# WilliamVenner/squad-mortar-helper

Measured on AMD Instinct MI355X. Metric: map frames/sec (1920x1080 full CV pipeline), whole job, higher is better.
Workload: dtype u8/f32

## Files before the change

### squad-mortar-helper_amd/batch.py

```python
import ctypes as C

import numpy as np

from . import _lib as L

STAGE_NAMES = ("button", "map_pass", "brq_pass", "lsd", "scale_ratio")


def make_anchors(per_frame):
    arr = (L.Anchors * len(per_frame))()
    for i, (start_y, scales) in enumerate(per_frame):
        arr[i].n = min(len(scales), L.MAX_SCALES)
        arr[i].scales_start_y = start_y
        for j, (m, x, y) in enumerate(scales[:L.MAX_SCALES]):
            arr[i].scales[j][0], arr[i].scales[j][1], arr[i].scales[j][2] = m, x, y
    return arr


def results_to_dicts(recs):
    out = []
    for r in recs:
        n = r.n_lines
        out.append(dict(
            map_open=int(r.map_open), n_lines=int(n),
# ... 93 lines not shown
            except L.VisionError as e:
                e.records = recs if rc == L.E_STATE else None
                raise
        return recs

    def set_firing(self, heightmap=None, fit_to_minimap=True, viewport=None):
        opt = L.firing_options(fit_to_minimap, viewport)
        L.check(self._lib.smhv_batch_set_firing(self._b, heightmap._hm if heightmap is not None else None, C.byref(opt)))

    def read_firing(self, first=0, n=None):
        n = self.max_frames - first if n is None else n
        out = (L.FiringResult * n)()
        L.check(self._lib.smhv_batch_read_firing(self._b, first, n, out))
        raw = np.frombuffer(out, np.uint8).reshape(n, C.sizeof(L.FiringResult))
        n_lines = raw[:, :4].copy().view(np.uint32).reshape(n)
        lines = raw[:, 8:].copy().view(L.firing_dtype()).reshape(n, L.MAX_LINES)
        return n_lines, lines

    def firing_ptr(self):
        d = C.c_void_p()
        L.check(self._lib.smhv_batch_firing_ptr(self._b, C.byref(d)))
        return d.value or 0

    def read_overlay(self, frame):
        return self.read_image(L.IMAGE_HEIGHTMAP_OVERLAY, frame)

    def overlay_ptr(self):
        d = C.c_void_p()
        L.check(self._lib.smhv_batch_overlay_ptr(self._b, C.byref(d)))
        return d.value or 0

    def render(self, viewport, out_w, out_h, first=0, n=None, heightmap=None, markers=False, fit_to_minimap=True, background=(0, 0, 0, 255),
               stream=None, options=None, layers=None):
        from .render import render_options
        n = self.max_frames - first if n is None else n
        opt = options if options is not None else render_options(viewport, out_w, out_h, heightmap is not None, markers, fit_to_minimap, background)
        if layers is not None:
            ly, keep = layers.struct()
            L.check(self._lib.smhv_batch_render_layers(self._b, first, n, heightmap._hm if heightmap is not None else None, C.byref(opt), C.byref(ly), stream))
            del keep
            return
        L.check(self._lib.smhv_batch_render(self._b, first, n, heightmap._hm if heightmap is not None else None, C.byref(opt), stream))

    def render_size(self):
        w, h = C.c_uint32(), C.c_uint32()
        L.check(self._lib.smhv_batch_render_size(self._b, C.byref(w), C.byref(h)))
        return int(w.value), int(h.value)

    def read_render(self, frame):
        w, h = self.render_size()
        out = np.empty((h, w, 4), np.uint8)
        L.check(self._lib.smhv_batch_read_render(self._b, frame, out.ctypes.data))
        return out

    def render_ptr(self):
        d, st = C.c_void_p(), C.c_uint64()
        L.check(self._lib.smhv_batch_render_ptr(self._b, C.byref(d), C.byref(st)))
        return d.value or 0, int(st.value)

    def render_labels(self, options, labels, first=0, n=None, heightmap=None, stream=None):
        n = self.max_frames - first if n is None else n
        lo, keep = labels.struct()
        L.check(self._lib.smhv_batch_render_labels(self._b, first, n, heightmap._hm if heightmap is not None else None, C.byref(options), C.byref(lo), stream))
        del keep

    def read_labels(self, first=0, n=None):
        n = self.max_frames - first if n is None else n
        out = (L.LabelResult * n)()
        L.check(self._lib.smhv_batch_read_labels(self._b, first, n, out))
        return out

    def labels_ptr(self):
        d = C.c_void_p()
        L.check(self._lib.smhv_batch_labels_ptr(self._b, C.byref(d)))
        return d.value or 0

    def feed(self, feed, first=0, n=None, snapshot=False, stream=0):
        n = self.max_frames - first if n is None else n
        L.check(self._lib.smhv_batch_feed(self._b, feed._f, first, n, L.FEED_SNAPSHOT if snapshot else 0, C.c_void_p(stream)))

    def read_image(self, which, frame):
        x, y, w, h = self.roi
        if which in (L.IMAGE_UI_MAP, L.IMAGE_HEIGHTMAP_OVERLAY):
            out = np.empty((h, w, 4), np.uint8)
        elif which == L.VIEW_LSD_INPUT:
            out = np.empty((h, w), np.uint8)
        else:
            out = np.empty((h // 2, w // 2), np.uint8)
        L.check(self._lib.smhv_batch_read_image(self._b, which, frame, out.ctypes.data))
        return out


class Pipeline:

    def __init__(self, vision, frame_w, frame_h, max_frames, depth=4, search=None, **options):
        self._lib = L.load()
        self._vision = vision
        p = C.c_void_p()
        opt = L.PipelineOptions()
        opt.size = C.sizeof(L.PipelineOptions)
        opt.search = {None: L.SEARCH_AUTO, "auto": L.SEARCH_AUTO, "batch": L.SEARCH_BATCH, "frame": L.SEARCH_FRAME}[search]
        for k, v in options.items():
            if k not in ("streams", "idle_close_us", "occupancy_policy", "late_helpers", "service_workgroups", "flags", "remote_after", "remote_tickets", "remote_last", "room_for_others"):
                raise TypeError("Pipeline: unknown option %r" % k)
            setattr(opt, k, int(v))
        L.check(self._lib.smhv_pipeline_create_ex(vision._ctx, frame_w, frame_h, max_frames, depth, C.byref(opt), C.byref(p)))
        self._p = p
        self.depth = depth
        self.slots = []
        for i in range(depth):
            b = C.c_void_p()
            L.check(self._lib.smhv_pipeline_slot(self._p, i, C.byref(b), None))
            self.slots.append(FrameBatch(vision, frame_w, frame_h, max_frames, _handle=b))

    def stream_of(self, slot):
        st = C.c_void_p()
        L.check(self._lib.smhv_pipeline_slot(self._p, slot, None, C.byref(st)))
        return st.value or 0

    def hold(self, slot, stream):
        L.check(self._lib.smhv_pipeline_hold(self._p, slot, C.c_void_p(stream)))

    def submit(self, frames_ptr, n, stages=L.STAGE_ALL, grayscale=True, max_gap=15, anchors=None, after_stream=0):
        if anchors is not None and len(anchors) < n:
            raise ValueError("anchors holds %d entries, the submission covers %d frames" % (len(anchors), n))
        a = C.cast(anchors, C.c_void_p) if anchors is not None else None
        slot = C.c_uint32(0)
        L.check(self._lib.smhv_pipeline_submit(self._p, C.c_void_p(frames_ptr), n, stages, int(bool(grayscale)), max_gap, a, C.c_void_p(after_stream), C.byref(slot)))
        return int(slot.value)

    def set_firing(self, heightmap=None, fit_to_minimap=True, viewport=None):
        opt = L.firing_options(fit_to_minimap, viewport)
        L.check(self._lib.smhv_pipeline_set_firing(self._p, heightmap._hm if heightmap is not None else None, C.byref(opt)))

    def search_stats(self):
        out = (C.c_uint64 * 32)()
        L.check(self._lib.smhv_debug_pipeline_stats(self._p, out))
        if not out[0]:
            return None
        keys = ("launches", "frames", "waves", "busy_cycles", "resident_cycles", "waves_per_launch", "submissions")
        d = dict(zip(keys, [int(v) for v in out[1:8]]))
        d["cycles_per_frame_by_phase"] = dict(zip(("acquire", "search", "record", "release"), [int(v) / max(d["frames"], 1) for v in out[8:12]]))
        d["help_cycles_per_frame"] = int(out[12]) / max(d["frames"], 1)
        d["remote_help"] = {"requests": int(out[16]), "helpers_attached": int(out[17]), "candidates_cast": int(out[18]), "tickets_left": int(out[19]) - (1 << 64) if int(out[19]) >= (1 << 63) else int(out[19])}
        d["cycles_per_frame"] = d["busy_cycles"] / max(d["frames"], 1)
        d["busy_fraction"] = d["busy_cycles"] / max(d["resident_cycles"], 1)
        d["remote_help"].update({"polls": int(out[23]), "polls_empty": int(out[24]), "claims_lost": int(out[25]), "exits_idle": int(out[26]), "exits_closed": int(out[27]),
                                 "cycles_attached_per_helper": int(out[28]) / max(int(out[17]), 1), "cast_fraction_of_attached": int(out[29]) / max(int(out[28]), 1)})
        d["timeline_ms"] = {"frame_wait": int(out[20]) / max(d["frames"], 1) / 1e5, "submission_search": int(out[21]) / max(d["submissions"], 1) / 1e5,
                            "last_frame_at_work": int(out[22]) / max(d["submissions"], 1) / 1e5}
        d["adaptive"] = bool(int(out[13]) & 2)
        d["settled"] = bool(int(out[13]) & 4) or not d["adaptive"]
        d["mode"] = "frame-granular" if int(out[13]) & 1 else "batch-granular"
        d["measured_frames_per_s"] = {"frame-granular": int(out[14]), "batch-granular": int(out[15])}
        return d

    def peek(self):
        out = (C.c_uint64 * 16)()
        L.check(self._lib.smhv_debug_pipeline_peek(self._p, out))
        keys = ("submissions", "alive_epoch", "launches", "last_seq", "avail", "head", "reserved", "closing_epoch", "completed", "busy")
        d = dict(zip(keys, [int(v) for v in out[:10]]))
        d["avail"] = d["avail"] - (1 << 64) if d["avail"] >= (1 << 63) else d["avail"]
        d["slots"] = [(int(v) >> 32, int(v) & 0xFFFFFFFF) for v in out[10:14]]
        d["service_workgroups"], d["waves_per_workgroup"] = int(out[14]) >> 32, int(out[14]) & 0xFFFFFFFF
        d["lds_words_per_wave"], d["lds_bytes_dynamic"] = int(out[15]) >> 32, int(out[15]) & 0xFFFFFFFF
        return d

    def wait(self, slot=None):
        if slot is None:
            L.check(self._lib.smhv_pipeline_wait_all(self._p))
        else:
            L.check(self._lib.smhv_pipeline_wait(self._p, slot))

    def close(self):
        if self._p:
            for b in self.slots:
                b.close()
            self._lib.smhv_pipeline_destroy(self._p)
            self._p = None

    def __del__(self):
        try:
            self.close()
        except Exception:
            pass
```

### squad-mortar-helper_amd/csrc/smh_kernels.h

```cpp
#pragma once
#include <hip/hip_runtime.h>
#include <stdint.h>

#include "../../include/smh_vision_hip.h"
#include "../../include/smh_vision_hip_debug.h"

namespace smh {

struct Geom {
	uint32_t W, H;
	uint32_t rx, ry, rw, rh;
	uint32_t bx, by, bw, bh;
	uint32_t qx, qy, qw, qh;
	uint32_t m_ax, m_xoff, m_quads, m_block;
	uint32_t q_ax, q_xoff, q_quads, q_block;
	uint64_t frame_bytes;
	uint64_t ui_pitch, ui_stride;
	uint64_t mask_pitch, mask_stride;
	uint32_t bits_pitch_w; uint64_t bits_stride_w;
	uint64_t ocr_pitch, ocr_stride;
};

struct FrameAux {
	uint32_t open;
	uint32_t red;
	uint32_t n_mask_px;
	uint32_t y_min, y_max, w_min, w_max;
	uint32_t tiles;
};

struct LsdCoop {
	uint32_t req_tail;
	uint32_t req_head;
	uint32_t done;
	uint32_t helpers;
	uint32_t remaining;
	uint32_t mode1;
	uint32_t stat_groups, stat_hits, stat_casts;
	uint32_t pad[7];
};
struct LsdCtl {
	uint32_t started[3];
	uint32_t finished[3];
	uint32_t pad[10];
};
struct LsdCacheEntry {
	unsigned long long tag;
	unsigned long long best;
	float ex, ey;
	uint32_t steps, pad;
};
#define SMH_LSD_REQ_CAP 64u
#define SMH_LSD_CACHE_SLOTS 512u
struct LsdCoopBufs {
	LsdCtl *ctl;
	LsdCoop *coop;
	uint32_t *req;
	LsdCacheEntry *cache;
	uint32_t epoch;
};

struct BatchError {
	uint32_t count;
	uint32_t frame, status;
	uint32_t info[8];
	uint32_t pad[5];
};

#define SMH_FARM_RING 4u
#define SMH_REC_ON 0x80000000u
#define SMH_LSD_LATE_HELP 1u
struct FarmEntry {
	unsigned long long post;
	unsigned long long best;
	unsigned long long end;
	unsigned long long start;
	unsigned long long done;
	unsigned long long pad[3];
};
struct FarmFrame {
	unsigned long long attached;
	unsigned long long owner_done;
	unsigned long long want;
	unsigned long long claimed;
	unsigned long long pad[4];
	FarmEntry ring[SMH_FARM_RING];
};

struct Buffers {
	BatchError *err;
	FarmFrame *farm;
	uint32_t rec_stages;
	uint32_t *rec_bars;
	uint32_t lsd_flags, lsd_late_kc;
	const uint8_t *frames;
	uint8_t *ui, *mask, *ocr, *scales;
	uint32_t *bits;
	uint32_t *tiled;
	uint8_t *occ;
	FrameAux *aux;
	smhv_frame_result *results;
	const smhv_anchors *anchors;
	const uint32_t *cull_tab;
	const float *ray_off;
	LsdCoopBufs co;
	const struct FiringRun *firing;
};
struct FiringRun {
	const uint16_t *hm;
	smhv_firing_result *out;
	uint32_t hm_w, hm_h;
	float b0x, b0y;
	double zscale;
	uint32_t flags;
	float sw, sh, tx, ty;
	uint32_t pad;
};
static_assert(sizeof(FiringRun) == 64, "one 64-byte block per run");
struct OverlayRun {
	const uint8_t *ui;
	uint8_t *out;
	const FrameAux *aux;
	const smhv_frame_result *res;
	const uint16_t *hm;
	const uint32_t *lut;
	uint32_t hm_w, hm_h;
	float b0x, b0y;
	uint32_t flags;
};
#define SMH_RND_MAX_LINES 256u
struct RenderRun {
	const uint8_t *ui;
	uint8_t *out;
	const FrameAux *aux;
	const smhv_frame_result *res;
	const smhv_line *lines;
	const uint16_t *hm;
	const uint32_t *lut;
	const uint16_t *lut16;
	uint64_t out_stride;
	uint32_t hm_w, hm_h;
	float b0x, b0y;
	uint32_t flags;
	uint32_t n_lines;
	uint32_t out_w, out_h;
	float ql, qt, qr, qb;
	float sw, sh, tx, ty;
	uint32_t bg;
	uint32_t lds_texels;
	uint32_t n_frames;
};
#define SMH_RND_MAX_ITEMS (SMH_RND_MAX_LINES + SMHV_RENDER_MAX_PRIMS + 1u)
#define SMH_RND_SRC_UI 0u
#define SMH_RND_SRC_GRAY 1u
#define SMH_RND_SRC_RGBA 2u
#define SMH_RND_SRC_PREPROCESS 3u
#define SMH_RND_SRC_CROPPED 4u
struct RenderLayersRun {
	const smhv_render_prim *prims;
	const uint8_t *src;
	uint64_t src_pitch, src_stride;
	uint32_t src_xoff;
	uint32_t src_mode;
	uint32_t src_w, src_h;
	uint32_t n_below, n_fg;
	uint32_t flags;
	uint32_t pad;
};
#define SMH_LBL_SLOTS (SMHV_LABEL_MAX_EXTRA + SMHV_MAX_LINES)
struct LabelCull { float mx, my, rad; uint32_t live; };
struct LabelRun {
	FiringRun fr;
	const FrameAux *aux;
	const smhv_frame_result *res;
	const smhv_label_line *extra;
	const smhv_line *lines;
	smhv_label_result *out;
	LabelCull *cull;
	uint8_t *img;
	uint64_t img_stride;
	double mpx;
	uint32_t out_w, out_h;
	uint32_t n_extra, n_lines;
	uint32_t detected;
	uint32_t scale;
	uint32_t per_call;
	uint32_t has_mpx;
};
__host__ __device__ inline uint32_t tiled_rows(const Geom &g) { return (g.rh + 7u) >> 3; }
__host__ __device__ inline uint64_t tiled_stride_w(const Geom &g) { return (uint64_t)tiled_rows(g) * g.bits_pitch_w * 8u; }
__host__ __device__ inline uint32_t occ_pitch(const Geom &g) { return ((g.m_block >> 6) + 3u) & ~3u; }
__host__ __device__ inline uint64_t occ_stride(const Geom &g) { return (uint64_t)tiled_rows(g) * occ_pitch(g); }

#define SMH_RAY_OFF_BATCHES 168u

#define SMH_SECTOR_R 52
#define SMH_SECTOR_DIM (2 * SMH_SECTOR_R + 1)
#define SMH_SECTOR_ENTRIES (SMH_SECTOR_DIM * SMH_SECTOR_DIM)
#define SMH_CULL_CELLS (SMH_SECTOR_DIM * 4)
#define SMH_CULL_TAB_WORDS (SMH_CULL_CELLS + (SMH_SECTOR_ENTRIES + 3) / 4)

#define SVC_MAX_SLOTS 32u
struct SvcSlot {
	Buffers b;
	uint32_t n;
	uint32_t seq;
	uint32_t done;
	uint32_t pad;
	unsigned long long t_pub;
};
#define SVC_REMOTE_RING 12u
#define SVC_REMOTE_OPEN 0x80000000ull
struct SvcRemoteEntry {
	unsigned long long post;
	unsigned long long claim;
	uint32_t res_a[4];
	uint32_t res_b[4];
	unsigned long long pad[2];
};
struct SvcRemote {
	unsigned long long state;
	unsigned long long info;
	unsigned long long pad[6];
	SvcRemoteEntry ring[SVC_REMOTE_RING];
};
#define SVC_HELP_RING 256u
struct SvcCtl {
	int32_t avail;
	uint32_t closing;
	int32_t help_avail;
	uint32_t help_head, help_reserve;
	uint32_t stat_remote;
	uint32_t head;
	uint32_t reserve;
	uint32_t completed;
	uint32_t busy;
	uint32_t stat_items, stat_waves;
	unsigned long long stat_busy, stat_life;
	unsigned long long stat_phase[4];
	unsigned long long stat_help;
	uint32_t stat_requests, stat_attached;
	unsigned long long stat_t_wait, stat_t_sub, stat_t_last;
	uint32_t stat_h_polls, stat_h_empty, stat_h_lost, stat_h_idle_exit, stat_h_closed_exit, stat_h_pad;
	unsigned long long stat_h_cycles, stat_h_cast_cycles;
	unsigned long long help_ring[SVC_HELP_RING];
};
struct SvcHost {
	unsigned long long state;
	uint32_t launches;
	uint32_t pad0;
	uint32_t done_seq[SVC_MAX_SLOTS];
	uint32_t pad[12];
};
struct SvcParams {
	SvcCtl *ctl;
	unsigned long long *ring;
	SvcSlot *slots;
	SvcHost *host;
	const uint32_t *cull_tab;
	const float *ray_off;
	float max_gap;
	uint32_t tile_cap, list_cap;
	uint32_t part_words;
	uint32_t ring_log2;
	uint32_t epoch;
	uint32_t idle_short, idle_long;
	uint32_t flags;
	SvcRemote *remote;
	uint32_t *remote_store;
	uint32_t remote_store_words;
	uint32_t remote_after;
	uint32_t remote_tickets;
	uint32_t remote_last_div;
	uint32_t compact;
};
uint32_t svc_waves_for(const Geom &g, uint32_t tile_limit, uint32_t *part_words, uint32_t *tile_cap, uint32_t *list_cap, uint32_t *lds_bytes, uint32_t *compact = nullptr);
uint32_t svc_store_words_for(const Geom &g, uint32_t tile_cap, uint32_t compact);
hipError_t svc_probe_host_atomics(SvcHost *h, SvcHost *d_h, bool *ok);
hipError_t launch_svc_publish(SvcCtl *ctl, unsigned long long *ring, SvcSlot *slots, uint32_t slot, const Buffers &b, uint32_t n, uint32_t seq, uint32_t ring_log2, hipStream_t s);
hipError_t launch_lsd_service(const Geom &g, const SvcParams &p, uint32_t workgroups, uint32_t waves, uint32_t lds_bytes, hipStream_t s);

enum : uint32_t { MAP_UI = 1u, MAP_MASK = 2u, MAP_PRIO = 0x100u, MAP_BAND_MAJOR = 0x200u };
enum : uint32_t { BRQ_OCR = 1u, BRQ_SCALES = 2u };

hipError_t launch_button(const Geom &g, const Buffers &b, uint32_t n, int force_open, hipStream_t s);
hipError_t launch_map_pass(const Geom &g, const Buffers &b, uint32_t n, uint32_t flags, int grayscale, hipStream_t s, bool tiles_wanted = false, bool overlapped = false);
struct LaunchTuning {
	uint32_t map_lds_total;
	uint32_t map_grid_cap;
	uint32_t lsd_tile_limit;
	uint32_t map_prio;
	uint32_t map_deep;
	uint32_t map_overlapped;
};
uint32_t map_brq_lds_bytes(const Geom &g);
uint32_t lsd_tile_lds_bytes(const Geom &g, uint32_t tile_limit);
hipError_t launch_map_brq_pass(const Geom &g, const Buffers &b, uint32_t n, uint32_t flags, uint32_t qflags, int grayscale, uint32_t fixed_start_y, int use_anchor_start, hipStream_t s,
                               const LaunchTuning *tune = nullptr);
hipError_t launch_pattern_copy(const Geom &g, const Buffers &b, uint32_t n, uint32_t rows_in_flight, hipStream_t s);
void map_band_rows(uint32_t rh, uint32_t n, int fused, uint32_t *rows, int *tiles);
hipError_t launch_brq_pass(const Geom &g, const Buffers &b, uint32_t n, uint32_t flags, uint32_t fixed_start_y, int use_anchor_start, hipStream_t s);
struct LsdFork { hipStream_t s1, s2; hipEvent_t fork, join1, join2; };
bool lsd_rows_only(const Geom &g);
hipError_t launch_lsd(const Geom &g, const Buffers &b, uint32_t n, float max_gap, int mode, float px, float py, hipStream_t s, const LsdFork *fk, uint32_t tile_bs = 0,
                      bool prefer_classic = false, uint32_t tile_limit = 0, bool *record_fused = nullptr);
size_t lsd_coop_ctl_bytes(uint32_t n);
hipError_t launch_scale_ratio(const Geom &g, const Buffers &b, uint32_t n, uint32_t *d_bars, hipStream_t s);
hipError_t launch_find_minimap(const Geom &g, const Buffers &b, uint32_t n, hipStream_t s);
hipError_t launch_finalize(const Geom &g, const Buffers &b, uint32_t n, uint32_t stages, hipStream_t s);
hipError_t launch_scales_finalize(const Geom &g, const Buffers &b, uint32_t n, uint32_t stages, uint32_t *d_bars, hipStream_t s);
hipError_t launch_firing_lines(const FiringRun &r, const smhv_line *lines, uint32_t n, uint32_t has_mpx, double mpx, uint32_t has_minimap,
                               const uint32_t minimap[4], smhv_firing *out, hipStream_t s);
hipError_t launch_heightmap_color_map(const uint16_t *hm, uint64_t n, uint32_t *mm, uint32_t *rgba, hipStream_t s);
#define SMH_HM_LUT_ENTRIES 65536u
hipError_t launch_heightmap_lut(const uint16_t *hm, uint64_t n, uint32_t *mm, uint32_t *lut, hipStream_t s);
hipError_t launch_hm_overlay(const Geom &g, const OverlayRun &r, uint32_t n, hipStream_t s);
hipError_t launch_render_map(const Geom &g, const RenderRun &r, uint32_t n, hipStream_t s);
hipError_t launch_render_map_layers(const Geom &g, const RenderRun &r, const RenderLayersRun &y, uint32_t n, hipStream_t s);
hipError_t launch_heightmap_lut16(const uint32_t *lut, uint16_t *lut16, uint32_t *vr, hipStream_t s);
#define SMH_HM_LUT_WORDS (SMH_HM_LUT_ENTRIES + 4u + SMH_HM_LUT_ENTRIES / 2u)
hipError_t launch_labels(const LabelRun &r, uint32_t n, hipStream_t s);
void render_set_form(uint32_t form);
uint32_t render_rule(const Geom &g, const RenderRun &r, uint32_t *texels, float *ratio);
float render_switch_ratio();
hipError_t launch_debug_view(const Geom &g, const Buffers &b, uint32_t frame, int which, int isolated, uint8_t *d_rgba, hipStream_t s);
hipError_t launch_marker_table(uint32_t *d_bits, hipStream_t s);
hipError_t launch_pack_rows(const void *d_src, uint32_t src_pitch_bytes, void *d_dst, uint32_t row_bytes, uint32_t rows, hipStream_t s);
hipError_t launch_side_probe(uint32_t *d_out, uint32_t workgroups, uint32_t spin, hipStream_t s);
hipError_t launch_build_sector_table(unsigned long long *d_tab, uint32_t T, hipStream_t s);
hipError_t launch_build_ray_offsets(float *d_off, hipStream_t s);
size_t lsd_lds_bytes();
void lsd_set_classic(bool on);
void lsd_set_tile_cap(uint32_t cap);
void lsd_set_threads(uint32_t threads);
void lsd_set_spin_limit(uint32_t polls);
hipError_t set_ray_table(const float *dx, const float *dy);
#define SMH_CRC_BS 1024
hipError_t launch_to_bgra(const void *d_src, void *d_bgra, uint64_t n_px, uint32_t layout, hipStream_t s);
hipError_t launch_unpack_rows(const void *d_pack, void *d_frame, uint32_t pitch_px, uint32_t roi_x, uint32_t roi_y, uint32_t roi_w, uint32_t roi_h, uint32_t btn_x,
                              uint32_t btn_y, uint32_t btn_w, uint32_t btn_h, hipStream_t s);
hipError_t launch_crc32(const void *d_msg, uint64_t n_dwords, uint32_t wgs, uint32_t rounds, uint32_t x_skip, const uint32_t *d_x_local,
                        const uint32_t *d_x_wg, uint32_t *d_acc, hipStream_t s);
uint32_t crc32_xpow(uint64_t n);
uint32_t crc32_mul(uint32_t a, uint32_t b);

struct FeedMap { uint64_t dst; uint32_t frame, pad; };
struct FeedRun {
	const uint8_t *ui;
	const smhv_frame_result *res;
	uint64_t ui_stride, ui_pitch;
	uint32_t w, h, xoff, quads;
	uint32_t n, first, flags;
	uint32_t len_term;
	uint32_t rows_per_wave;
	uint64_t capacity;
	uint32_t *raw;
	const uint32_t *tab;
	uint32_t *state;
	smhv_feed_header *header;
	smhv_feed_entry *entries;
	uint8_t *bytes;
	FeedMap *maps;
};
#define SMH_FEED_MAX_ROWS 16384u
hipError_t launch_feed_tables(uint32_t *d_tab, uint32_t w, uint32_t h, uint32_t xoff, uint32_t quads, hipStream_t s);
uint32_t feed_rows_per_wave(uint32_t h, uint32_t n);
void feed_set_rows(uint32_t rows);
hipError_t launch_feed(const FeedRun &r, hipStream_t s);

}
```

### squad-mortar-helper_amd/csrc/smh_lsd.hip

```cpp
#include <algorithm>
#include <atomic>
#include <cstdlib>
#include <cstring>

#include "smh_device.h"
#include "smh_proximity.h"
#include "smh_record.inc"

namespace smh {

struct RayDir { uint32_t dx, dy; };
__device__ RayDir g_ray_table[SMH_LSD_RAYS] = {
#include "ray_table.inc"
};

#ifndef LSD_BS
#define LSD_BS 1024
#endif
#define LSD_NW (LSD_BS / 64)
#ifndef LSD_C
#define LSD_C 8u
#endif
#ifndef LSD_C_RESET
#define LSD_C_RESET 2u
// ... 1126 lines not shown
				if (hit) m |= 1ull << u;
			}
		}
	}
	tab[i] = m;
}

size_t lsd_lds_bytes() { return LSD_DYN_LDS_BYTES; }

static std::atomic<bool> &lsd_classic_flag() {
	static std::atomic<bool> flag{false};
	return flag;
}
void lsd_set_classic(bool on) { lsd_classic_flag().store(on, std::memory_order_relaxed); }
static std::atomic<uint32_t> g_tile_cap_override{0};
void lsd_set_tile_cap(uint32_t cap) { g_tile_cap_override.store(cap, std::memory_order_relaxed); }
static std::atomic<uint32_t> g_bs_override{0};
void lsd_set_threads(uint32_t threads) { g_bs_override.store(threads, std::memory_order_relaxed); }
static std::atomic<uint32_t> g_spin_limit{W_SPIN_LIMIT_DEFAULT};
void lsd_set_spin_limit(uint32_t polls) { g_spin_limit.store(polls ? polls : W_SPIN_LIMIT_DEFAULT, std::memory_order_relaxed); }

bool lsd_rows_only(const Geom &g) { return (g.rh + 2u) * LSD_ROWS_PITCH(g.bits_pitch_w) + 4u <= LSD_WIN_WORDS_CAP; }

static uint32_t lsd_tile_static_lds() {
	static const uint32_t v = [] { hipFuncAttributes a; return hipFuncGetAttributes(&a, (const void *)k_lsd_tile) == hipSuccess ? (uint32_t)a.sharedSizeBytes : 17408u; }();
	return v;
}
static uint32_t lsd_tile_cap_of(const Geom &g, uint32_t tile_limit) {
	const uint32_t cap_o = g_tile_cap_override.load(std::memory_order_relaxed);
	uint32_t cap = tile_cap_for(g);
	if (tile_limit) cap = std::min(cap, tile_limit);
	if (cap_o) cap = std::min(cap_o, tile_cap_for(g));
	return cap;
}
uint32_t lsd_tile_lds_bytes(const Geom &g, uint32_t tile_limit) {
	return lsd_tile_static_lds() + (tile_mask_words(g.rw, g.rh, lsd_tile_cap_of(g, tile_limit)) + 2u * tile_list_cap_for(g) + W_NWIN * W_WIN_STRIDE) * 4u;
}

hipError_t launch_lsd(const Geom &g, const Buffers &b, uint32_t n, float max_gap, int mode, float px, float py, hipStream_t s, const LsdFork *fk, uint32_t tile_bs, bool prefer_classic,
                      uint32_t tile_limit, bool *record_fused) {
	if (record_fused) *record_fused = false;
	const unsigned lds_full = LSD_DYN_LDS_BYTES;
	static std::atomic<uint64_t> attr_devices{0};
	int dev = 0;
	hipError_t e0 = hipGetDevice(&dev);
	if (e0 != hipSuccess) return e0;
	if (dev >= 64 || !((attr_devices.load(std::memory_order_acquire) >> dev) & 1ull)) {
		hipError_t e = hipSuccess;
		const void *fns[] = {(const void *)k_lsd<LSD_MODE_ROWS, false>, (const void *)k_lsd<LSD_MODE_XWIN, false>, (const void *)k_lsd<LSD_MODE_GLOBAL, false>,
		                     (const void *)k_lsd<LSD_MODE_ROWS, true>, (const void *)k_lsd<LSD_MODE_XWIN, true>, (const void *)k_lsd<LSD_MODE_GLOBAL, true>};
		for (const void *fn : fns) if (e == hipSuccess) e = hipFuncSetAttribute(fn, hipFuncAttributeMaxDynamicSharedMemorySize, (int)lds_full);
		if (e == hipSuccess) e = hipFuncSetAttribute((const void *)k_lsd_tile, hipFuncAttributeMaxDynamicSharedMemorySize, (int)LSD_TILE_DYN_LDS_MAX);
		if (e != hipSuccess) return e;
		if (dev < 64) attr_devices.fetch_or(1ull << dev, std::memory_order_release);
	}
	const bool rows_only = mode == 0 && lsd_rows_only(g);
	const bool coop = mode == 0 && b.co.ctl != nullptr;
	if (mode == 0 && !coop && !prefer_classic && !lsd_classic_flag().load(std::memory_order_relaxed)) {
		const uint32_t bs_o = g_bs_override.load(std::memory_order_relaxed);
		const uint32_t bs = std::max<uint32_t>(128u, bs_o ? bs_o : (tile_bs ? std::min<uint32_t>(tile_bs, LSD_TILE_BS) : 512u));
		const uint32_t cap = lsd_tile_cap_of(g, tile_limit);
		const unsigned t_lds = std::min<unsigned>((tile_mask_words(g.rw, g.rh, cap) + 2u * tile_list_cap_for(g) + W_NWIN * W_WIN_STRIDE) * 4u, LSD_TILE_DYN_LDS_MAX);
		if (record_fused) *record_fused = (b.rec_stages & SMH_REC_ON) != 0u;
		hipLaunchKernelGGL(k_lsd_tile, dim3(n), dim3(bs), t_lds, s, g, b, max_gap, cap, g_spin_limit.load(std::memory_order_relaxed), tile_list_cap_for(g), n);
		return hipGetLastError();
	}
	if (coop) {
		hipError_t e = hipMemsetAsync(b.co.ctl, 0, lsd_coop_ctl_bytes(n), s);
		if (e != hipSuccess) return e;
	}
	uint32_t extra = 0;
	if (coop && rows_only) {
		static std::atomic<int> n_cus{0};
		int cus = n_cus.load(std::memory_order_relaxed);
		if (cus == 0) {
			if (hipDeviceGetAttribute(&cus, hipDeviceAttributeMultiprocessorCount, dev) != hipSuccess || cus <= 0) cus = 256;
			n_cus.store(cus, std::memory_order_relaxed);
		}
		if (n < (uint32_t)cus) extra = std::min((uint32_t)cus - n, 4u * n);
	}
	hipStream_t s1 = s, s2 = s;
	if (!rows_only && fk) {
		hipError_t e = hipEventRecord(fk->fork, s);
		if (e == hipSuccess) e = hipStreamWaitEvent(fk->s1, fk->fork, 0);
		if (e == hipSuccess) e = hipStreamWaitEvent(fk->s2, fk->fork, 0);
		if (e != hipSuccess) return e;
		s1 = fk->s1; s2 = fk->s2;
	}
	if (record_fused && mode == 0) *record_fused = (b.rec_stages & SMH_REC_ON) != 0u;
	if (coop) hipLaunchKernelGGL((k_lsd<LSD_MODE_ROWS, true>), dim3(n + extra), dim3(LSD_BS), lds_full, s, g, b, max_gap, mode, px, py, n);
	else hipLaunchKernelGGL((k_lsd<LSD_MODE_ROWS, false>), dim3(n), dim3(LSD_BS), lds_full, s, g, b, max_gap, mode, px, py, n);
	if (!rows_only) {
		if (coop) hipLaunchKernelGGL((k_lsd<LSD_MODE_XWIN, true>), dim3(n), dim3(LSD_BS), lds_full, s1, g, b, max_gap, mode, px, py, n);
		else hipLaunchKernelGGL((k_lsd<LSD_MODE_XWIN, false>), dim3(n), dim3(LSD_BS), lds_full, s1, g, b, max_gap, mode, px, py, n);
		if (coop) hipLaunchKernelGGL((k_lsd<LSD_MODE_GLOBAL, true>), dim3(n), dim3(LSD_BS), lds_full, s2, g, b, max_gap, mode, px, py, n);
		else hipLaunchKernelGGL((k_lsd<LSD_MODE_GLOBAL, false>), dim3(n), dim3(LSD_BS), lds_full, s2, g, b, max_gap, mode, px, py, n);
		if (fk) {
			hipError_t e = hipEventRecord(fk->join1, s1);
			if (e == hipSuccess) e = hipEventRecord(fk->join2, s2);
			if (e == hipSuccess) e = hipStreamWaitEvent(s, fk->join1, 0);
			if (e == hipSuccess) e = hipStreamWaitEvent(s, fk->join2, 0);
			if (e != hipSuccess) return e;
		}
	}
	return hipGetLastError();
}

static uint32_t lsd_service_static_lds() {
	static const uint32_t v = [] { hipFuncAttributes a; return hipFuncGetAttributes(&a, (const void *)k_lsd_service) == hipSuccess ? (uint32_t)a.sharedSizeBytes : SMH_CULL_TAB_WORDS * 4u; }();
	return v;
}
uint32_t svc_waves_for(const Geom &g, uint32_t tile_limit, uint32_t *part_words, uint32_t *tile_cap, uint32_t *list_cap, uint32_t *lds_bytes, uint32_t *compact) {
	const uint32_t cap = lsd_tile_cap_of(g, tile_limit);
	const uint32_t lds_cu = 160u * 1024u, beside = 2u * ((map_brq_lds_bytes(g) + 1023u) & ~1023u) + 1024u;
	uint32_t best_w = 0, best_part = 0, best_lc = 0, best_c = 0;
	for (uint32_t c = 0; c < 2u; ++c) {
		const uint32_t lc = c ? W_LIST_CAP_MAX / 2u : tile_list_cap_for(g);
		const uint32_t part = (SVC_WS_WORDS + (c ? tilec_mask_words(g.rw, g.rh, cap) : tile_mask_words(g.rw, g.rh, cap)) + 2u * lc + W_WIN_STRIDE + 3u) & ~3u;
		uint32_t w = SVC_MAX_WAVES;
		while (w > 0u && lsd_service_static_lds() + w * part * 4u + beside > lds_cu) --w;
		if (w > best_w) { best_w = w; best_part = part; best_lc = lc; best_c = c; }
	}
	if (part_words) *part_words = best_part;
	if (tile_cap) *tile_cap = cap;
	if (list_cap) *list_cap = best_lc;
	if (lds_bytes) *lds_bytes = best_w * best_part * 4u;
	if (compact) *compact = best_c;
	return best_w;
}

uint32_t svc_store_words_for(const Geom &g, uint32_t tile_cap, uint32_t compact) { return ((compact ? tilec_mask_words(g.rw, g.rh, tile_cap) : tile_mask_words(g.rw, g.rh, tile_cap)) + 7u) & ~3u; }

hipError_t svc_probe_host_atomics(SvcHost *h, SvcHost *d_h, bool *ok) {
	*ok = false;
	uint32_t *d_ok = nullptr;
	hipError_t e = hipMalloc((void **)&d_ok, sizeof(uint32_t));
	if (e != hipSuccess) return e;
	const unsigned long long expect = 0x0123456789ABCDEFull, desired = 0xFEDCBA9876543210ull;
	unsigned long long *w = (unsigned long long *)&h->pad[0];
	__atomic_store_n(w, expect, __ATOMIC_RELEASE);
	__atomic_store_n(&h->pad[2], 0u, __ATOMIC_RELEASE);
	e = hipMemset(d_ok, 0, sizeof(uint32_t));
	uint32_t dev_ok = 0;
	if (e == hipSuccess) { hipLaunchKernelGGL(k_svc_probe, dim3(1), dim3(1), 0, nullptr, d_h, expect, desired, d_ok); e = hipGetLastError(); }
	if (e == hipSuccess) e = hipMemcpy(&dev_ok, d_ok, sizeof dev_ok, hipMemcpyDeviceToHost);
	(void)hipFree(d_ok);
	if (e != hipSuccess) return e;
	*ok = dev_ok == 1u && __atomic_load_n(w, __ATOMIC_ACQUIRE) == desired && __atomic_load_n(&h->pad[2], __ATOMIC_ACQUIRE) == 0x600Du;
	__atomic_store_n(w, 0ull, __ATOMIC_RELEASE);
	__atomic_store_n(&h->pad[2], 0u, __ATOMIC_RELEASE);
	return hipSuccess;
}

hipError_t launch_svc_publish(SvcCtl *ctl, unsigned long long *ring, SvcSlot *slots, uint32_t slot, const Buffers &b, uint32_t n, uint32_t seq, uint32_t ring_log2, hipStream_t s) {
	hipLaunchKernelGGL(k_svc_publish, dim3(1), dim3(256), 0, s, ctl, ring, slots, slot, b, n, seq, ring_log2);
	return hipGetLastError();
}

hipError_t launch_lsd_service(const Geom &g, const SvcParams &p, uint32_t workgroups, uint32_t waves, uint32_t lds_bytes, hipStream_t s) {
	static std::atomic<uint64_t> attr_devices{0};
	int dev = 0;
	hipError_t e = hipGetDevice(&dev);
	if (e != hipSuccess) return e;
	if (dev >= 64 || !((attr_devices.load(std::memory_order_acquire) >> dev) & 1ull)) {
		e = hipFuncSetAttribute((const void *)k_lsd_service, hipFuncAttributeMaxDynamicSharedMemorySize, 160 * 1024 - (int)lsd_service_static_lds());
		if (e == hipSuccess) e = hipFuncSetAttribute((const void *)k_lsd_service_c, hipFuncAttributeMaxDynamicSharedMemorySize, 160 * 1024 - (int)lsd_service_static_lds());
		if (e != hipSuccess) return e;
		if (dev < 64) attr_devices.fetch_or(1ull << dev, std::memory_order_release);
	}
	if (p.compact) hipLaunchKernelGGL(k_lsd_service_c, dim3(workgroups), dim3(64u * waves), lds_bytes, s, g, p);
	else hipLaunchKernelGGL(k_lsd_service, dim3(workgroups), dim3(64u * waves), lds_bytes, s, g, p);
	return hipGetLastError();
}

size_t lsd_coop_ctl_bytes(uint32_t n) { return sizeof(LsdCtl) + sizeof(LsdCoop) * (size_t)n; }

hipError_t set_ray_table(const float *dx, const float *dy) {
	static RayDir host[SMH_LSD_RAYS];
	for (int i = 0; i < SMH_LSD_RAYS; ++i) { memcpy(&host[i].dx, &dx[i], 4); memcpy(&host[i].dy, &dy[i], 4); }
	return hipMemcpyToSymbol(HIP_SYMBOL(g_ray_table), host, sizeof host, 0, hipMemcpyHostToDevice);
}

__global__ void k_build_ray_offsets(float *off) {
	const uint32_t i = blockIdx.x * blockDim.x + threadIdx.x;
	if (i >= SMH_LSD_RAYS) return;
	const float dx = __uint_as_float(g_ray_table[i].dx), dy = __uint_as_float(g_ray_table[i].dy);
	float xo = 0.0f, yo = 0.0f;
	float2 *o = (float2 *)off + (size_t)i * (SMH_RAY_OFF_BATCHES + 1u);
	for (uint32_t j = 0; j <= SMH_RAY_OFF_BATCHES; ++j) {
		o[j] = make_float2(xo, yo);
		for (int k = 0; k < 32; ++k) { xo += dx; yo += dy; }
	}
}

hipError_t launch_build_ray_offsets(float *d_off, hipStream_t s) {
	hipLaunchKernelGGL(k_build_ray_offsets, dim3((SMH_LSD_RAYS + 63) / 64), dim3(64), 0, s, d_off);
	return hipGetLastError();
}

hipError_t launch_build_sector_table(unsigned long long *d_tab, uint32_t T, hipStream_t s) {
	static_assert(LSD_GROUPS == LSD_GROUPS_HOST && LSD_GROUPS <= 64, "sector masks are 64-bit");
	hipLaunchKernelGGL(k_build_sector_table, dim3((SMH_SECTOR_ENTRIES + 255) / 256), dim3(256), 0, s, d_tab, T);
	return hipGetLastError();
}

}
```

### squad-mortar-helper_amd/csrc/smh_lsd_seq.inc

```

template <int MODE>
__device__ __forceinline__ uint32_t seq_build_list(const Win &m, WShared &ws, uint32_t *list, uint32_t *survw, uint32_t list_cap, uint32_t wy0, uint32_t wrows, uint32_t wwords, uint32_t wi_min,
                                                   uint32_t WT, uint32_t *wi_next) {
	const uint32_t lane = threadIdx.x & 63u;
	uint32_t o = 0, next = WT;
	auto append = [&](uint32_t w, uint32_t wi) {
		const unsigned long long nz = __ballot(w != 0u);
		if (!nz) return;
		const uint32_t pos = o + (uint32_t)__popcll(nz & ((1ull << lane) - 1ull));
		if (w != 0u && pos < list_cap) { list[pos] = wi; survw[pos] = w; ws.stag[pos] = 0; }
		const uint32_t cnt = (uint32_t)__popcll(nz);
		if (o + cnt > list_cap) {
			unsigned long long rest = nz;
			for (uint32_t k = o; k < list_cap; ++k) rest &= rest - 1ull;
			next = (uint32_t)__builtin_amdgcn_readlane((int)wi, (int)__builtin_ctzll(rest));
			o = list_cap;
		} else o += cnt;
	};
	if constexpr (MODE == LSD_MODE_TILE || MODE == LSD_MODE_TILEC) {
		auto tile_at = [&](uint32_t ty, uint32_t c) -> uint32_t {
			if constexpr (MODE == LSD_MODE_TILEC) return tilec_number(m, (int)c, (int)ty);
			else return (uint32_t)m.t_idx[__mul24((int)ty, (int)m.t_pitch) + (int)c];
		};
		const bool two = wwords <= 32u;
// ... 296 lines not shown
		const uint32_t wi = list[e], r = wi / wwords, c = wi - r * wwords;
		fpy = (float)(wy0 + r); fpx0 = (float)(xorg + (int)(c * 32u));
		const uint32_t tag = ws.stag[e];
		if (w && tag < n_lines) {
			for (uint32_t l = tag; l < n_lines && w; ++l) {
				ProxLine L;
				L.x0 = ws.lines[l][0]; L.y0 = ws.lines[l][1]; L.x1 = ws.lines[l][2]; L.y1 = ws.lines[l][3];
				L.a = ws.prox_a[l]; L.dxl = ws.prox_d[l][0]; L.dyl = ws.prox_d[l][1];
				L.degenerate = L.dxl == 0.0 && L.dyl == 0.0;
				w = prox_filter_word(w, fpx0, fpy, L);
			}
			survw[e] = w;
			ws.stag[e] = (unsigned char)n_lines;
		}
	}
	return w;
}

__device__ __forceinline__ void desk_post_remote(WShared &ws, uint32_t slot, uint32_t qx, uint32_t qy, uint32_t &st, uint32_t &spx, uint32_t &spy) {
	const uint32_t k = uniform_u32(ws.rem_k) + 1u;
	if (opaque_lane() == slot) {
		ws.rob[slot].px = qx; ws.rob[slot].py = qy; ws.rob[slot].lines_seen = k; ws.rob[slot].state = H_RPOSTED;
		ws.rem_k = k;
		g_st64(&rem_of(ws)->ring[slot - SEQ_HELP_SLOTS].post, ((unsigned long long)k << 32) | ((qy & 0xFFFFu) << 16) | (qx & 0xFFFFu));
		st = H_RPOSTED; spx = qx; spy = qy;
	}
	RDBG(0, 1ull);
	wave_lds_sync();
}
__device__ __forceinline__ void desk_refresh(WShared &ws, const uint32_t *list, uint32_t *survw, uint32_t wy0, uint32_t wwords, int xorg, uint32_t cap_local, uint32_t cap_remote, uint32_t &post_seq,
                                             uint32_t &cur_e, int &cur_bit, uint32_t &ahead) {
	const uint32_t lane = opaque_lane();
	const uint32_t n_lines = W_LD(&ws.n_lines), end = ws.disp_end, first = W_LD(&ws.disp_e);
	const uint32_t want = 1u + cap_local + cap_remote;
	cur_e = end; cur_bit = -1;
	uint32_t mpx = 0xFFFFFFFFu, mpy = 0xFFFFFFFFu, np = 0;
	for (uint32_t e0 = first & ~63u; e0 < end && np < want; e0 += 64u) {
		float fpx0, fpy;
		const uint32_t w = disp_entry(ws, list, survw, e0 + lane, first, end, n_lines, wy0, wwords, xorg, fpx0, fpy);
		unsigned long long any = __ballot(w != 0u);
		while (any && np < want) {
			const uint32_t src = (uint32_t)__builtin_ctzll(any);
			any &= any - 1ull;
			uint32_t ww = (uint32_t)__builtin_amdgcn_readlane((int)w, (int)src);
			const int bx = (int)bcast_f(fpx0, src);
			const uint32_t by = (uint32_t)bcast_f(fpy, src);
			while (ww && np < want) {
				const uint32_t bit = (uint32_t)__builtin_ctz(ww);
				ww &= ww - 1u;
				if (lane == np) { mpx = (uint32_t)(bx + (int)bit); mpy = by; }
				++np;
				if (np == want) { cur_e = e0 + src; cur_bit = (int)bit; }
			}
		}
	}
	ahead = np;
	uint32_t st = H_FREE, spx = 0, spy = 0, sk = 0;
	if (lane < SEQ_DESK_ENTRIES) { st = W_LD_ACQ(&ws.rob[lane].state); spx = ws.rob[lane].px; spy = ws.rob[lane].py; sk = ws.rob[lane].lines_seen; }
	bool listed = false;
	for (uint32_t k = 0; k < np; ++k) {
		const uint32_t qx = (uint32_t)__builtin_amdgcn_readlane((int)mpx, (int)k), qy = (uint32_t)__builtin_amdgcn_readlane((int)mpy, (int)k);
		listed = listed || (spx == qx && spy == qy);
	}
	if (lane < SEQ_HELP_SLOTS && !listed) {
		if (st == (uint32_t)H_DONE) { W_ST(&ws.rob[lane].state, (uint32_t)H_FREE); st = H_FREE; }
		else if (st == (uint32_t)H_POSTED) {
			uint32_t expect = H_POSTED;
			if (__hip_atomic_compare_exchange_strong(&ws.rob[lane].state, &expect, (uint32_t)H_FREE, __ATOMIC_ACQ_REL, __ATOMIC_RELAXED, __HIP_MEMORY_SCOPE_WORKGROUP)) st = H_FREE;
			else st = H_TAKEN;
		}
	}
	if (lane >= SEQ_HELP_SLOTS && lane < SEQ_DESK_ENTRIES && !listed) {
		if (st == (uint32_t)H_DONE) { ws.rob[lane].state = H_FREE; st = H_FREE; }
		else if (st == (uint32_t)H_RPOSTED) {
			const unsigned long long old = __hip_atomic_fetch_max(&rem_of(ws)->ring[lane - SEQ_HELP_SLOTS].claim, (unsigned long long)sk, __ATOMIC_RELAXED, __HIP_MEMORY_SCOPE_AGENT);
			st = (uint32_t)old < sk ? (uint32_t)H_FREE : (uint32_t)H_RZOMBIE;
			ws.rob[lane].state = st;
#ifdef SMH_LSD_WDEBUG
			atomicAdd(&ws.rdbg[st == (uint32_t)H_FREE ? 1 : 2], 1ull);
#endif
		}
	}
	wave_lds_sync();
	for (uint32_t k = 1; k < np; ++k) {
		const uint32_t qx = (uint32_t)__builtin_amdgcn_readlane((int)mpx, (int)k), qy = (uint32_t)__builtin_amdgcn_readlane((int)mpy, (int)k);
		const bool live = lane < SEQ_DESK_ENTRIES && st != (uint32_t)H_FREE && st != (uint32_t)H_RZOMBIE;
		if (__ballot(live && spx == qx && spy == qy) != 0ull) continue;
		const unsigned long long free_l = __ballot(lane < SEQ_HELP_SLOTS && st == (uint32_t)H_FREE);
		const unsigned long long free_r = __ballot(lane >= SEQ_HELP_SLOTS && lane < SEQ_DESK_ENTRIES && st == (uint32_t)H_FREE);
		const uint32_t busy_l = SEQ_HELP_SLOTS - (uint32_t)__popcll(free_l);
		const uint32_t busy_r = (uint32_t)__popcll(__ballot(lane >= SEQ_HELP_SLOTS && live));
		if (busy_l < cap_local && free_l) {
			const uint32_t slot = (uint32_t)__builtin_ctzll(free_l);
			if (lane == slot) {
				ws.rob[slot].px = qx; ws.rob[slot].py = qy; ws.rob[slot].lines_seen = post_seq;
				W_ST_REL(&ws.rob[slot].state, (uint32_t)H_POSTED);
				st = H_POSTED; spx = qx; spy = qy;
			}
			++post_seq;
		} else if (busy_r < cap_remote && free_r) desk_post_remote(ws, (uint32_t)__builtin_ctzll(free_r), qx, qy, st, spx, spy);
		else break;
	}
}

__device__ __forceinline__ void desk_post_more(WShared &ws, const uint32_t *list, uint32_t *survw, uint32_t wy0, uint32_t wwords, int xorg, uint32_t cap_local, uint32_t cap_remote, uint32_t &post_seq,
                                               uint32_t &cur_e, int &cur_bit, uint32_t &ahead) {
	const uint32_t lane = opaque_lane();
	uint32_t st = H_DONE;
	if (lane < SEQ_DESK_ENTRIES) st = W_LD_ACQ(&ws.rob[lane].state);
	unsigned long long free_l = __ballot(lane < SEQ_HELP_SLOTS && st == (uint32_t)H_FREE);
	unsigned long long free_r = __ballot(lane >= SEQ_HELP_SLOTS && lane < SEQ_DESK_ENTRIES && st == (uint32_t)H_FREE);
	uint32_t busy_l = SEQ_HELP_SLOTS - (uint32_t)__popcll(free_l);
	uint32_t busy_r = (uint32_t)__popcll(__ballot(lane >= SEQ_HELP_SLOTS && lane < SEQ_DESK_ENTRIES && (st == (uint32_t)H_RPOSTED || st == (uint32_t)H_DONE)));
	if (cap_remote && busy_r < cap_remote && !free_r && __ballot(lane >= SEQ_HELP_SLOTS && lane < SEQ_DESK_ENTRIES && st == (uint32_t)H_RZOMBIE)) {
		remote_harvest(ws);
		if (lane < SEQ_DESK_ENTRIES) st = W_LD_ACQ(&ws.rob[lane].state);
		free_r = __ballot(lane >= SEQ_HELP_SLOTS && lane < SEQ_DESK_ENTRIES && st == (uint32_t)H_FREE);
	}
	bool room_l = busy_l < cap_local && free_l, room_r = busy_r < cap_remote && free_r;
	if (!room_l && !room_r) return;
	const uint32_t n_lines = W_LD(&ws.n_lines), end = ws.disp_end, first = W_LD(&ws.disp_e);
	while ((room_l || room_r) && cur_e < end) {
		const uint32_t e0 = cur_e & ~63u;
		float fpx0, fpy;
		uint32_t w = disp_entry(ws, list, survw, e0 + lane, first, end, n_lines, wy0, wwords, xorg, fpx0, fpy);
		if (e0 + lane < cur_e) w = 0u;
		else if (e0 + lane == cur_e && cur_bit >= 0) w = cur_bit >= 31 ? 0u : (w & ~((2u << (uint32_t)cur_bit) - 1u));
		const unsigned long long any = __ballot(w != 0u);
		if (!any) { cur_e = e0 + 64u; cur_bit = -1; continue; }
		const uint32_t src = (uint32_t)__builtin_ctzll(any);
		const uint32_t ww = (uint32_t)__builtin_amdgcn_readlane((int)w, (int)src);
		const uint32_t bit = (uint32_t)__builtin_ctz(ww);
		const uint32_t ppx = (uint32_t)((int)bcast_f(fpx0, src) + (int)bit), ppy = (uint32_t)bcast_f(fpy, src);
		cur_e = e0 + src; cur_bit = (int)bit;
		if (ahead++ == 0u) continue;
		if (room_l) {
			const uint32_t slot = (uint32_t)__builtin_ctzll(free_l);
			free_l &= free_l - 1ull;
			if (lane == slot) {
				ws.rob[slot].px = ppx; ws.rob[slot].py = ppy; ws.rob[slot].lines_seen = post_seq;
				W_ST_REL(&ws.rob[slot].state, (uint32_t)H_POSTED);
			}
			++post_seq; ++busy_l;
		} else {
			uint32_t d0 = 0, d1 = 0, d2 = 0;
			desk_post_remote(ws, (uint32_t)__builtin_ctzll(free_r), ppx, ppy, d0, d1, d2);
			free_r &= free_r - 1ull;
			++busy_r;
		}
		room_l = busy_l < cap_local && free_l; room_r = busy_r < cap_remote && free_r;
	}
}

template <int MODE, bool WAVE = false, bool TEAM = false>
__device__ void lsd_frame_seq(const Geom &g, const Buffers &b, uint32_t f, float max_gap, const FrameAux &aux, uint32_t *smem, WShared &ws, const uint32_t *cull_tab, const RayDir *dirs,
                              uint32_t win_cap, uint32_t list_cap, const FrameView *tile_view = nullptr) {
	static_assert(!TEAM || (WAVE && (MODE == LSD_MODE_TILE || MODE == LSD_MODE_TILEC)), "helpers read the owner's tile store in LDS");
	const uint32_t lane = threadIdx.x & 63u;
	FrameView v;
	if constexpr (MODE == LSD_MODE_TILE || MODE == LSD_MODE_TILEC) v = *tile_view;
	else frame_setup<MODE, WAVE>(g, b, f, aux, smem, v);
	const Win &m = v.m;
	uint32_t *list = smem + win_cap, *survw = list + list_cap, *wwin = survw + list_cap;
	const uint32_t wy0 = v.wy0, wrows = v.wrows, wwords = v.wwords;
	const int xorg = v.xorg;
	const uint32_t WT = wrows * wwords;
	const bool cull = b.cull_tab != nullptr && max_gap > 0.0f && max_gap <= 49.0f;
	if (lane == 0) { ws.n_lines = 0u; ws.rounds = 0u; ws.steps = 0ull; }
	if (TEAM && lane < SEQ_DESK_ENTRIES) ws.rob[lane].state = H_FREE;
	if (TEAM && lane == 0) { ws.rem_open = 0u; ws.rem_nr = 0u; }
#ifdef SMH_LSD_WDEBUG
	if (lane < 8u) ws.dbg[lane] = 0u;
	if (lane < 10u) ws.rdbg[lane] = 0ull;
	if (lane == 0) ws.prof[0] = 0ull;
#endif
	const bool remote_ok = TEAM && ws.rem_r != 0ull;
	bool rem_open = false;
	uint32_t rem_nr = 0, rem_asked = 0;
	uint32_t rounds = 0, n_lines = 0, post_seq = 0;
	uint32_t seg_start = 0, cur_e = 0, ahead = 0;
	int cur_bit = -1;
	bool done = false, want = false, desk_valid = false;
#ifdef SMH_LSD_WDEBUG
	unsigned long long sprof[8] = {0, 0, 0, 0, 0, 0, 0, 0}, slast = __builtin_amdgcn_s_memtime(), uprof[12] = {0, 0, 0, 0, 0, 0, 0, 0, 0, 0, 0, 0};
	uint32_t n_units = 0, n_taken = 0;
#define SPROF(i) do { const unsigned long long _n = __builtin_amdgcn_s_memtime(); sprof[i] += _n - slast; slast = _n; } while (0)
#else
#define SPROF(i)
#endif
	while (!done) {
		uint32_t segnext;
		const uint32_t n_list = seq_build_list<MODE>(m, ws, list, survw, list_cap, wy0, wrows, wwords, seg_start, WT, &segnext);
		if (lane == 0) { ws.disp_e = 0u; ws.disp_end = n_list; }
		desk_valid = false;
		__builtin_amdgcn_fence(__ATOMIC_RELEASE, "workgroup");
		__builtin_amdgcn_wave_barrier();
		__builtin_amdgcn_fence(__ATOMIC_ACQUIRE, "workgroup");
		SPROF(0);
		while (true) {
			uint32_t px = 0, py = 0;
			if (!wave_dispatch(ws, list, survw, wy0, wwords, xorg, px, py)) break;
			__builtin_amdgcn_fence(__ATOMIC_RELEASE, "workgroup");
			__builtin_amdgcn_wave_barrier();
			SPROF(1);
			float xs = 0.0f, ys = 0.0f, ex0 = 0.0f, ey0 = 0.0f;
			unsigned long long wkey = 0ull;
			uint32_t st_sum = 0u;
			++rounds;
			if (ahead) --ahead;
			bool have = false;
#ifdef SMH_LSD_WDEBUG
			const unsigned long long t_tk = __builtin_amdgcn_s_memtime();
#endif
			if (TEAM && want) have = desk_take(ws, px, py, xs, ys, wkey, ex0, ey0, st_sum);
#ifdef SMH_LSD_WDEBUG
			if (rem_open) RDBG(7, __builtin_amdgcn_s_memtime() - t_tk);
#endif
#ifdef SMH_LSD_WDEBUG
			if (have) ++n_taken;
			if (!have) seq_cast_candidate<MODE>(m, wwin, cull_tab, cull, dirs, b.ray_off, max_gap, px, py, xs, ys, wkey, ex0, ey0, st_sum, sprof, slast, uprof, n_units);
#else
			if (!have) seq_cast_candidate<MODE>(m, wwin, cull_tab, cull, dirs, b.ray_off, max_gap, px, py, xs, ys, wkey, ex0, ey0, st_sum);
#endif
			if (lane == 0) ws.steps += st_sum;
			if (wkey != 0ull && __uint_as_float((uint32_t)(wkey >> 32)) > SMH_LSD_ACCEPT_LEN_SQ) {
				float ex, ey;
				get_centre(m, ex0, ey0, ex, ey);
				if (lane == 0) {
					ws.lines[n_lines][0] = xs; ws.lines[n_lines][1] = ys; ws.lines[n_lines][2] = ex; ws.lines[n_lines][3] = ey;
					const ProxLine pl = prox_line(xs, ys, ex, ey);
					ws.prox_a[n_lines] = pl.a; ws.prox_d[n_lines][0] = pl.dxl; ws.prox_d[n_lines][1] = pl.dyl;
					W_ST_REL(&ws.n_lines, n_lines + 1u);
				}
				++n_lines;
				desk_valid = false;
				__builtin_amdgcn_fence(__ATOMIC_RELEASE, "workgroup");
				__builtin_amdgcn_wave_barrier();
				__builtin_amdgcn_fence(__ATOMIC_ACQUIRE, "workgroup");
				if (n_lines == SMH_LSD_MAX_LINES) { done = true; break; }
			}
			if (TEAM) {
				if (!want && rounds >= SEQ_HELP_AFTER) {
					want = true;
					if (lane == 0) W_ST_REL(&ws.want_set, 1u);
				}
				if (want) {
					if (remote_ok && (rounds & (rem_open ? 7u : 1u)) == 0u) {
						if (rem_open) {
							rem_nr = remote_helpers(ws);
							const uint32_t want_h = uniform_u32(ws.rem_tickets);
							if (rem_nr * 2u < want_h && rounds - rem_asked >= 8u) {
								if ((ws.rem_flags & 1u) || (int32_t)uniform_u32((uint32_t)__hip_atomic_load(&rem_ctl_of(ws)->avail, __ATOMIC_RELAXED, __HIP_MEMORY_SCOPE_AGENT)) <= 0)
									(void)remote_issue_tickets(ws, rem_ctl_of(ws), uniform_u32(ws.rem_gen), want_h - rem_nr);
								rem_asked = rounds;
							}
						}
						else if (rounds >= uniform_u32(ws.rem_after) && ws.disp_end - min(W_LD(&ws.disp_e), ws.disp_end) >= SEQ_REMOTE_MIN_LEFT) {
							const uint32_t *dp = (const uint32_t *)(uintptr_t)(((unsigned long long)uniform_u32((uint32_t)(ws.rem_done >> 32)) << 32) | uniform_u32((uint32_t)ws.rem_done));
							const uint32_t n_sub = uniform_u32(ws.rem_n), fin = uniform_u32(__hip_atomic_load(dp, __ATOMIC_RELAXED, __HIP_MEMORY_SCOPE_AGENT));
							const bool free_waves = (ws.rem_flags & 1u) || (int32_t)uniform_u32((uint32_t)__hip_atomic_load(&rem_ctl_of(ws)->avail, __ATOMIC_RELAXED, __HIP_MEMORY_SCOPE_AGENT)) <= 0;
							if (free_waves && (n_sub - min(fin, n_sub)) * uniform_u32(ws.rem_last_div) <= n_sub) rem_asked = rounds;
#ifdef SMH_LSD_WDEBUG
							if (rem_asked == rounds && lane == 0) { ws.dbg[3] += 1u; if (ws.dbg[4] == 0u) ws.dbg[4] = rounds; }
#endif
							if (rem_asked == rounds)
								rem_open = remote_open<MODE == LSD_MODE_TILEC>((uint32_t)(uintptr_t)(const LdsByte *)&ws, (uint32_t)(uintptr_t)(const LdsByte *)smem, MODE == LSD_MODE_TILEC ? tilec_idx_words(g.rw, g.rh) : tile_idx_words(g.rw, g.rh));
						}
					}
					const uint32_t nh = uniform_u32(W_LD(&ws.late));
					const uint32_t cap_l = min(nh, SEQ_HELP_SLOTS - 1u), cap_r = rem_open ? min(2u + 2u * rem_nr, SVC_REMOTE_RING) : 0u;
					if (!cap_l && !cap_r) desk_valid = false;
					else if (!desk_valid) {
#ifdef SMH_LSD_WDEBUG
						const unsigned long long t_r = __builtin_amdgcn_s_memtime();
#endif
						desk_refresh(ws, list, survw, wy0, wwords, xorg, cap_l, cap_r, post_seq, cur_e, cur_bit, ahead);
						desk_valid = true;
#ifdef SMH_LSD_WDEBUG
						if (rem_open) { RDBG(3, 1ull); RDBG(5, __builtin_amdgcn_s_memtime() - t_r); }
#endif
					} else {
#ifdef SMH_LSD_WDEBUG
						const unsigned long long t_r = __builtin_amdgcn_s_memtime();
#endif
						desk_post_more(ws, list, survw, wy0, wwords, xorg, cap_l, cap_r, post_seq, cur_e, cur_bit, ahead);
#ifdef SMH_LSD_WDEBUG
						if (rem_open) RDBG(6, __builtin_amdgcn_s_memtime() - t_r);
#endif
					}
#ifdef SMH_LSD_WDEBUG
					if (rem_open) { RDBG(8, 1ull); if (lane == 0 && ws.rdbg[9] == 0ull) ws.rdbg[9] = __builtin_amdgcn_s_memtime(); }
#endif
				}
			}
			SPROF(4);
		}
		if (segnext >= WT) break;
		seg_start = segnext;
	}
	if (TEAM) {
		if (lane == 0) W_ST_REL(&ws.want_set, 0u);
		if (rem_open) remote_close(ws);
		while (uniform_u32(W_LD_ACQ(&ws.late)) != 0u) __builtin_amdgcn_s_sleep(2);
	}
	smhv_frame_result *res = &b.results[f];
	if (lane < n_lines) {
		res->lines[lane].x0 = ws.lines[lane][0]; res->lines[lane].y0 = ws.lines[lane][1];
		res->lines[lane].x1 = ws.lines[lane][2]; res->lines[lane].y1 = ws.lines[lane][3];
	}
	if (lane == 0) { res->n_lines = n_lines; res->rounds = rounds; res->ray_steps = ws.steps; res->status = SMHV_FRAME_OK; }
#ifdef SMH_LSD_WDEBUG
	if (lane == 0) {
		for (int k = 0; k < 5; ++k) res->meters[20 + k] = (double)sprof[k];
		for (int k = 0; k < 3; ++k) res->meters[25 + k] = (double)uprof[8 + k];
		res->meters[30] = (double)uprof[0]; res->meters[31] = (double)uprof[1];
		res->meters[28] = (double)n_units;
		res->meters[29] = (double)n_taken;
		res->length_px[22] = (double)ws.dbg[0]; res->length_px[23] = (double)ws.dbg[1]; res->length_px[24] = (double)ws.dbg[2]; res->length_px[25] = (double)ws.prof[0];
		res->length_px[26] = (double)ws.dbg[3]; res->length_px[27] = (double)ws.dbg[4];
		for (int k = 0; k < 9; ++k) res->angle[16 + k] = (float)ws.rdbg[k];
		res->angle[25] = ws.rdbg[9] ? (float)(__builtin_amdgcn_s_memtime() - ws.rdbg[9]) : 0.0f;
	}
#endif
}
```

### squad-mortar-helper_amd/csrc/smh_lsd_wave.inc

```

#ifndef W_WAVES_PER_EU
#define W_WAVES_PER_EU 4
#endif
#ifndef W_A_BATCHES
#define W_A_BATCHES LSD_A_BATCHES
#endif
#ifndef W_NWIN
#define W_NWIN 4u
#endif
#define W_ROB 16u
#define W_LIST_CAP_MAX 1024u
#define W_WIN_R 67
#define W_WIN_ROWS (2 * W_WIN_R + 1)
#define W_WIN_STRIDE (W_WIN_ROWS * LSD_W2_PITCH + 2u)
#ifndef W_SPEC_MAX
#define W_SPEC_MAX 8u
#endif
static_assert(W_SPEC_MAX + SMH_FARM_RING <= W_ROB && W_NWIN <= W_SPEC_MAX && W_NWIN + SMH_FARM_RING <= W_ROB && (W_ROB & (W_ROB - 1u)) == 0u && W_NWIN <= 32u, "reorder buffer: every local (one window each) and remote (one ring entry each) candidate in flight has a slot");
static_assert(2 * W_WIN_R + 1 + 31 <= 32 * LSD_W2_PITCH, "a window row holds the neighbourhood from a word boundary on");
static_assert(W_WIN_R >= 32 * (int)W_A_BATCHES + 3 && W_WIN_R >= SMH_SECTOR_R + 3, "the window covers the first batches and the culling annulus");
#ifndef W_SPEC_MIN
#define W_SPEC_MIN 2u
#endif
#ifndef W_SPEC_GROW
#define W_SPEC_GROW(s) ((s) * 2u)
#endif
#define W_SPIN_LIMIT_DEFAULT 4000000u

struct WSlot {
	uint32_t px, py;
	uint32_t lines_seen;
	uint32_t state;
	float ptx, pty;
	unsigned long long todo;
	unsigned long long live;
	unsigned long long best;
	float ex, ey;
	uint32_t block;
	uint32_t pending;
	uint32_t steps;
	uint32_t win;
	unsigned long long tag;
#ifdef SMH_LSD_WDEBUG
	unsigned long long t_disp, t_setup, t_done;
#endif
};
enum { W_FREE = 0, W_SETUP = 1, W_CASTING = 2, W_DONE = 3, W_REMOTE = 4 };

struct WShared {
	WSlot rob[W_ROB];
	uint32_t lock;
	uint32_t head, tail;
	uint32_t spec;
	uint32_t disp_e, disp_end;
	uint32_t n_lines, rounds, frame_done;
	unsigned long long steps;
	float lines[SMH_LSD_MAX_LINES][4];
	float prox_a[SMH_LSD_MAX_LINES];
	double prox_d[SMH_LSD_MAX_LINES][2];
	unsigned char stag[W_LIST_CAP_MAX];
	uint32_t scan[LSD_NW];
	uint32_t segnext;
	uint32_t ntiles;
	uint32_t stuck;
	uint32_t win_free;
	uint32_t farm_on, farm_posted, farm_retired, pad0;
	uint32_t late, want_set, want_tick, pick;
	unsigned long long t0, late_cycles;
	unsigned long long rem_r, rem_store, rem_ctl;
	uint32_t rem_after, rem_tickets, rem_owner, rem_cap;
	uint32_t rem_open, rem_gen, rem_k, rem_nr;
	unsigned long long rem_done;
	uint32_t rem_n, rem_last_div;
	uint32_t rem_flags, rem_pad;
#ifdef SMH_LSD_WDEBUG
	uint32_t dbg[8];
	unsigned long long rdbg[10];
	uint32_t why[4];
	unsigned long long prof[12];
	unsigned long long lat[8];
#endif
};
#ifdef SMH_LSD_WDEBUG
#define WDBG(i, v) do { if ((threadIdx.x & 63u) == 0) atomicAdd(&ws.dbg[i], (v)); } while (0)
#define WPROF(i) do { const unsigned long long _n = __builtin_amdgcn_s_memtime(); wprof[i] += _n - wlast; wlast = _n; } while (0)
#else
#define WDBG(i, v)
#define WPROF(i)
#endif

#define W_LD(p) __hip_atomic_load((p), __ATOMIC_RELAXED, __HIP_MEMORY_SCOPE_WORKGROUP)
#define W_LD_ACQ(p) __hip_atomic_load((p), __ATOMIC_ACQUIRE, __HIP_MEMORY_SCOPE_WORKGROUP)
#define W_ST(p, v) __hip_atomic_store((p), (v), __ATOMIC_RELAXED, __HIP_MEMORY_SCOPE_WORKGROUP)
#define W_ST_REL(p, v) __hip_atomic_store((p), (v), __ATOMIC_RELEASE, __HIP_MEMORY_SCOPE_WORKGROUP)

__device__ __forceinline__ float bcast_f(float v, uint32_t src) { return __uint_as_float((uint32_t)__builtin_amdgcn_readlane((int)__float_as_uint(v), (int)src)); }
__device__ __forceinline__ uint32_t uniform_u32(uint32_t v) { return (uint32_t)__builtin_amdgcn_readfirstlane((int)v); }

__device__ __forceinline__ const LdsByte *window_base(const uint32_t *wwin, uint32_t px, uint32_t py) {
	const int x0 = ((int)px - W_WIN_R) & ~31, y0 = (int)py - W_WIN_R;
	return (const LdsByte *)(const LdsWord *)wwin - (__mul24(y0, (int)(4u * LSD_W2_PITCH)) + ((x0 >> 5) << 2));
}
__device__ __forceinline__ uint32_t opaque_lane() { uint32_t l = threadIdx.x & 63u; asm volatile("" : "+v"(l)); return l; }
template <bool COMPACT = false>
__device__ __forceinline__ void cand_setup(const Win &m, uint32_t *wwin, const uint32_t *cull_tab, bool cull, uint32_t px, uint32_t py, float &xs, float &ys, unsigned long long &live
#ifdef SMH_LSD_WDEBUG
                                           , unsigned long long *cprof = nullptr
#endif
                                           ) {
	const uint32_t lane = opaque_lane();
#ifdef SMH_LSD_WDEBUG
	const unsigned long long c_t0 = __builtin_amdgcn_s_memtime();
#endif
	{
		const int wq0 = (((int)px - W_WIN_R) & ~31) >> 5, y0 = (int)py - W_WIN_R;
		constexpr uint32_t NIT = (W_WIN_ROWS * LSD_W2_PITCH + 63u) / 64u;
		if (m.tiled) {
#pragma unroll
			for (uint32_t k = 0; k < NIT; ++k) {
				const uint32_t i = lane + 64u * k;
				if (i < W_WIN_ROWS * LSD_W2_PITCH) wwin[i] = 0u;
			}
			const int ty0 = y0 >> 3, ty1 = (y0 + (int)W_WIN_ROWS - 1) >> 3;
			const uint32_t nslots = (uint32_t)(ty1 - ty0 + 1) * LSD_W2_PITCH;
			static_assert(((W_WIN_ROWS + 14u) / 8u + 1u) * LSD_W2_PITCH <= 128u, "two tile slots per lane cover the window");
			uint32_t tv[2];
#pragma unroll
			for (uint32_t rnd = 0; rnd < 2u; ++rnd) {
				const uint32_t sidx = lane + 64u * rnd, tr = sidx / LSD_W2_PITCH, tc = sidx - tr * LSD_W2_PITCH;
				const int ty = ty0 + (int)tr, wq = wq0 + (int)tc;
				const bool ok = sidx < nslots && ty >= 0 && (uint32_t)(ty << 3) < m.h && (uint32_t)(wq + 2) < m.t_pitch;
				if constexpr (COMPACT) tv[rnd] = ok ? tilec_number(m, wq, ty) : 0u;
				else tv[rnd] = ok ? (uint32_t)m.t_idx[__mul24(ty, (int)m.t_pitch) + wq] : 0u;
			}
			const uint32_t grp = lane >> 3, row = lane & 7u;
#pragma unroll
			for (uint32_t rnd = 0; rnd < 2u; ++rnd) {
				unsigned long long todo = __ballot(tv[rnd] != 0u);
				while (todo) {
					uint32_t src = 64u;
#pragma unroll
					for (uint32_t k = 0; k < 8u; ++k) {
						const uint32_t p = todo ? (uint32_t)__builtin_ctzll(todo) : 64u;
						todo &= todo - 1ull;
						if (grp == k) src = p;
					}
					const uint32_t tt = (uint32_t)__shfl((int)tv[rnd], (int)(src & 63u));
					const uint32_t sidx = src + 64u * rnd, tr = sidx / LSD_W2_PITCH, tc = sidx - tr * LSD_W2_PITCH;
					const int rr = ((ty0 + (int)tr) << 3) + (int)row - y0;
					if (src < 64u && rr >= 0 && rr < (int)W_WIN_ROWS) wwin[(uint32_t)rr * LSD_W2_PITCH + tc] = (uint32_t)m.t_tiles[(tt << 3) + row];
				}
			}
		} else {
#pragma unroll 1
			for (uint32_t i = lane; i < W_WIN_ROWS * LSD_W2_PITCH; i += 64u) {
				const uint32_t r = i / LSD_W2_PITCH, c = i - r * LSD_W2_PITCH;
				const int b0 = ((wq0 + (int)c) << 5) + m.xbias;
				wwin[i] = __builtin_amdgcn_alignbit(win_word(m, (b0 >> 5) + 1, y0 + (int)r), win_word(m, b0 >> 5, y0 + (int)r), (uint32_t)b0 & 31u);
			}
		}
		if (lane < 2u) wwin[W_WIN_ROWS * LSD_W2_PITCH + lane] = 0u;
		__builtin_amdgcn_fence(__ATOMIC_RELEASE, "workgroup");
		__builtin_amdgcn_wave_barrier();
	}
#ifdef SMH_LSD_WDEBUG
	if (cprof) cprof[0] += __builtin_amdgcn_s_memtime() - c_t0;
#endif
	Win mw = m;
	mw.w2 = window_base(wwin, px, py);
	{
		const uint32_t l = lane & 31u, dir = l >> 3, k = l & 7u;
		const float cx = (float)px, cy = (float)py, fk = (float)k;
		bool cond = k < 5u;
		if (dir == 0u) cond = cond && (cx - fk > 0.0f);
		else if (dir == 1u) cond = cond && (cx + fk < (float)(m.w - 1u));
		else if (dir == 2u) cond = cond && (cy - fk > 0.0f);
		else cond = cond && (cy + fk < (float)(m.h - 1u));
		if (cond) {
			const int k_ = (int)k;
			const int xi = (int)px + (dir == 0u ? -k_ : (dir == 1u ? k_ : 0)), yi = (int)py + (dir == 2u ? -k_ : (dir == 3u ? k_ : 0));
			cond = win2_bit(mw, xi, yi) != 0u;
		}
		const uint32_t bits = (uint32_t)__ballot(cond);
		const float nl = (float)__builtin_ctz(~(bits & 0xFFu)), nr = (float)__builtin_ctz(~((bits >> 8) & 0xFFu));
		const float nu = (float)__builtin_ctz(~((bits >> 16) & 0xFFu)), nd = (float)__builtin_ctz(~((bits >> 24) & 0xFFu));
		xs = ((cx - nl) + (cx + nr)) / 2.0f;
		ys = ((cy - nu) + (cy + nd)) / 2.0f;
	}
	live = (1ull << LSD_GROUPS) - 1ull;
#ifdef SMH_LSD_WDEBUG
	const unsigned long long c_t1 = __builtin_amdgcn_s_memtime();
	struct CullTimer { unsigned long long *p, t; __device__ ~CullTimer() { if (p) p[1] += __builtin_amdgcn_s_memtime() - t; } } c_timer{cprof, c_t1};
#endif
	if (cull) {
		unsigned long long acc = 0ull;
		const int fx = (int)floorf(xs), fy = (int)floorf(ys);
		constexpr int ROUNDS = (SMH_CULL_CELLS + 63) / 64;
		uint32_t hits[ROUNDS];
#pragma unroll
		for (int it = 0; it < ROUNDS; ++it) {
			const uint32_t cell = lane + 64u * (uint32_t)it;
			const int yi = fy + (int)(cell >> 2) - SMH_SECTOR_R;
			uint32_t hit = 0;
			if (cell < SMH_CULL_CELLS) {
				const int b0 = fx - SMH_SECTOR_R + (int)((cell & 3u) << 5);
				const uint32_t lo = win2_word(mw, b0 >> 5, yi), hi = win2_word(mw, (b0 >> 5) + 1, yi);
				hit = __builtin_amdgcn_alignbit(hi, lo, (uint32_t)b0 & 31u) & cull_tab[cell];
			}
			hits[it] = hit;
		}
#pragma unroll
		for (int it = 0; it < ROUNDS; ++it) {
			uint32_t hit = hits[it];
			if (hit) {
				const uint32_t cell = lane + 64u * (uint32_t)it;
				const uint8_t *codes = (const uint8_t *)(cull_tab + SMH_CULL_CELLS) + (cell >> 2) * SMH_SECTOR_DIM + ((cell & 3u) << 5);
				while (hit) {
					const uint32_t code = codes[__builtin_ctz(hit)];
					hit &= hit - 1u;
					acc |= code == 0xFFu ? ~0ull : ((2ull << (code >> 6)) - 1ull) << (code & 63u);
				}
			}
		}
		acc = wave_or64(acc);
		live = (acc | (acc >> LSD_GROUPS)) & ((1ull << LSD_GROUPS) - 1ull);
	}
}
// ... 1239 lines not shown
```

### squad-mortar-helper_amd/csrc/smh_record.inc

```
#pragma once
#include "smh_device.h"
#include "smh_firing.h"

namespace smh {

__device__ inline bool find_scale_width(const uint8_t *img, size_t pitch, uint32_t w, uint32_t h, uint32_t meters, uint32_t x, uint32_t y, double *ratio,
                                 uint32_t bar[3]) {
	const uint32_t lane = threadIdx.x & 63u;
	if (y < SMH_MIN_SCALE_VERTICAL_BAR_HEIGHT || x >= w) return false;
	const double t = (20.0 / 640.0) * (double)w;
	const uint32_t max_off = (uint32_t)floor(t + 0.5);
	const uint32_t y_end = min(h, y + max_off);
	auto first_tick = [&](uint32_t yy, uint32_t count, auto col) -> uint32_t {
		for (uint32_t base = 0; base < count; base += 256u) {
			uint8_t v[4][SMH_MIN_SCALE_VERTICAL_BAR_HEIGHT];
#pragma unroll
			for (uint32_t c = 0; c < 4u; ++c) {
				const uint32_t i = base + c * 64u + lane, xx = col(min(i, count - 1u));
#pragma unroll
				for (uint32_t k = 0; k < SMH_MIN_SCALE_VERTICAL_BAR_HEIGHT; ++k) v[c][k] = img[(size_t)min(yy + k, h - 1u) * pitch + xx];
			}
#pragma unroll
			for (uint32_t c = 0; c < 4u; ++c) {
				const uint32_t i = base + c * 64u + lane;
				uint32_t bad = 0;
#pragma unroll
				for (uint32_t k = 0; k < SMH_MIN_SCALE_VERTICAL_BAR_HEIGHT; ++k) bad |= (yy + k >= h || v[c][k] != 0) ? 1u : 0u;
				const uint64_t hit = __ballot(i < count && bad == 0u);
				if (hit) return base + c * 64u + (uint32_t)__builtin_ctzll(hit);
			}
		}
		return count;
	};
	for (uint32_t y0 = y; y0 < y_end; y0 += 64u) {
		const uint32_t yl = y0 + lane;
		uint64_t rows = __ballot(yl < y_end && img[(size_t)min(yl, h - 1u) * pitch + x] == 0);
		while (rows) {
			const uint32_t yy = y0 + (uint32_t)__builtin_ctzll(rows);
			rows &= rows - 1ull;
			const uint32_t ri = first_tick(yy, w - x, [&](uint32_t i) { return x + i; });
			uint32_t right = ri < w - x ? x + ri : 0u;
			if (right == 0) continue;
			right -= 1;
			const uint32_t li = x ? first_tick(yy, x, [&](uint32_t i) { return x - 1u - i; }) : 0u;
			uint32_t left = li < x ? x - 1u - li : 0u;
			if (left == 0) continue;
			left += 1;
			const uint32_t width = right - left;
			if (width < SMH_MIN_SCALE_WIDTH) continue;
			bar[0] = left; bar[1] = yy; bar[2] = right;
			*ratio = (double)meters / (double)width;
			return true;
		}
	}
	return false;
}

__device__ __forceinline__ void scale_ratio_body(const Geom &g, const Buffers &b, uint32_t f, uint32_t *bars) {
	const uint32_t wave = threadIdx.x >> 6, lane = threadIdx.x & 63u, nwaves = blockDim.x >> 6;
	__shared__ double s_ratio[SMHV_MAX_SCALES];
	__shared__ uint32_t s_ok[SMHV_MAX_SCALES];
	smhv_frame_result *res = &b.results[f];
	const bool open = b.aux[f].open != 0;
	const smhv_anchors an = b.anchors[f];
	const uint32_t n = open ? min(an.n, (uint32_t)SMHV_MAX_SCALES) : 0u;
	const bool valid = an.scales_start_y <= g.qh;
	for (uint32_t k = wave; k < SMHV_MAX_SCALES; k += nwaves) {
		double r = 0.0;
		uint32_t bar[3] = {0, 0, 0};
		bool ok = false;
		if (k < n && valid) {
			const uint8_t *img = b.scales + (size_t)f * g.ocr_stride + g.q_xoff;
			ok = find_scale_width(img, g.ocr_pitch, g.qw, g.qh, an.scales[k][0], an.scales[k][1], an.scales[k][2], &r, bar);
		}
		if (lane == 0) {
			s_ratio[k] = r; s_ok[k] = ok ? 1u : 0u;
			if (bars) {
				uint32_t *o = bars + ((size_t)f * SMHV_MAX_SCALES + k) * 4;
				o[0] = bar[0]; o[1] = bar[1]; o[2] = bar[2]; o[3] = ok ? 1u : 0u;
			}
		}
	}
	__syncthreads();
	if (threadIdx.x == 0) {
		double sum = 0.0; uint32_t k = 0;
		for (uint32_t i = 0; i < SMHV_MAX_SCALES; ++i)
			if (s_ok[i]) { sum = k ? sum + s_ratio[i] : s_ratio[i]; ++k; }
		res->has_mpx = k ? 1u : 0u;
		res->mpx = k == 0 ? 0.0 : (k == 1 ? sum : sum / (double)k);
	}
}

__device__ __forceinline__ void finalize_body(const Geom &g, const Buffers &b, uint32_t f, uint32_t stages, uint32_t l) {
	smhv_frame_result *res = &b.results[f];
	const FrameAux aux = b.aux[f];
	const bool open = aux.open != 0;
	const bool markers = (stages & SMHV_STAGE_MARKERS) != 0;
	const uint32_t n = (open && markers) ? res->n_lines : 0u;
	const bool has_mpx = open && (stages & SMHV_STAGE_SCALES) && res->has_mpx;
	const double mpx = has_mpx ? res->mpx : 0.0;
	if (l < SMHV_MAX_LINES) {
		double len = 0.0, met = 0.0;
		float ang = 0.0f;
		smhv_line ln = {0.0f, 0.0f, 0.0f, 0.0f};
		if (l < n) {
			ln = res->lines[l];
			const double ax = (double)ln.x0 - (double)ln.x1, ay = (double)ln.y0 - (double)ln.y1;
			len = sqrt(ax * ax + ay * ay);
			met = has_mpx ? len * mpx : 0.0;
			ang = atan2f(ln.y0 - ln.y1, ln.x0 - ln.x1);
		}
		res->lines[l] = ln;
#ifdef SMH_LSD_PROFILE
		if (l < 20)
#endif
		res->length_px[l] = len;
#ifdef SMH_LSD_PROFILE
		if (l < 16)
#endif
		res->angle[l] = ang;
#ifdef SMH_LSD_PROFILE
		if (l < 20)
#endif
		res->meters[l] = met;
	}
	if (l == 0) {
		res->map_open = open ? 1u : 0u;
		res->n_lines = n;
		res->mpx = mpx; res->has_mpx = has_mpx ? 1u : 0u;
		res->n_mask_px = (open && markers) ? aux.n_mask_px : 0u;
		res->red_pixels = aux.red;
		if (!(open && markers)) { res->rounds = 0; res->ray_steps = 0; }
		if (!(stages & SMHV_STAGE_MINIMAP)) { res->has_minimap = 0; res->minimap[0] = 0; res->minimap[1] = 0; res->minimap[2] = 0; res->minimap[3] = 0; }
		if (!(open && markers)) res->status = SMHV_FRAME_OK;
	}
}

__device__ __forceinline__ void finalize_body(const Geom &g, const Buffers &b, uint32_t f, uint32_t stages) { finalize_body(g, b, f, stages, threadIdx.x); }

__device__ __forceinline__ void firing_after_finalize(const Buffers *bp, uint32_t f, uint32_t lane) {
	__builtin_amdgcn_fence(__ATOMIC_RELEASE, "workgroup");
	__builtin_amdgcn_wave_barrier();
	__builtin_amdgcn_fence(__ATOMIC_ACQUIRE, "workgroup");
	firing_frame_tail(bp, f, lane);
}

__device__ __attribute__((noinline)) void frame_record_tail(const Geom *gp, const Buffers *bp, uint32_t f) {
	const Geom &g = *gp;
	const Buffers &b = *bp;
	const uint32_t stages = b.rec_stages & ~SMH_REC_ON;
	if (stages & SMHV_STAGE_SCALES) {
		scale_ratio_body(g, b, f, b.rec_bars);
		__syncthreads();
	}
	if (threadIdx.x < 64) {
		finalize_body(g, b, f, stages);
		if (stages & SMHV_STAGE_FIRING) firing_after_finalize(bp, f, threadIdx.x);
	}
}

__device__ __attribute__((noinline)) void frame_record_tail_wave(const Geom *gp, const Buffers *bp, uint32_t f) {
	const Geom &g = *gp;
	const Buffers &b = *bp;
	const uint32_t stages = b.rec_stages & ~SMH_REC_ON;
	const uint32_t lane = threadIdx.x & 63u;
	smhv_frame_result *res = &b.results[f];
	if (stages & SMHV_STAGE_SCALES) {
		const bool open = b.aux[f].open != 0;
		const smhv_anchors an = b.anchors[f];
		const uint32_t n = open ? min(an.n, (uint32_t)SMHV_MAX_SCALES) : 0u;
		const bool valid = an.scales_start_y <= g.qh;
		double sum = 0.0;
		uint32_t cnt = 0;
		for (uint32_t k = 0; k < SMHV_MAX_SCALES; ++k) {
			double r = 0.0;
			uint32_t bar[3] = {0, 0, 0};
			bool ok = false;
			if (k < n && valid) {
				const uint8_t *img = b.scales + (size_t)f * g.ocr_stride + g.q_xoff;
				ok = find_scale_width(img, g.ocr_pitch, g.qw, g.qh, an.scales[k][0], an.scales[k][1], an.scales[k][2], &r, bar);
			}
			if (lane == 0 && b.rec_bars) {
				uint32_t *o = b.rec_bars + ((size_t)f * SMHV_MAX_SCALES + k) * 4;
				o[0] = bar[0]; o[1] = bar[1]; o[2] = bar[2]; o[3] = ok ? 1u : 0u;
			}
			if (ok) { sum = cnt ? sum + r : r; ++cnt; }
		}
		if (lane == 0) {
			res->has_mpx = cnt ? 1u : 0u;
			res->mpx = cnt == 0 ? 0.0 : (cnt == 1 ? sum : sum / (double)cnt);
		}
	}
	__builtin_amdgcn_fence(__ATOMIC_RELEASE, "workgroup");
	__builtin_amdgcn_wave_barrier();
	__builtin_amdgcn_fence(__ATOMIC_ACQUIRE, "workgroup");
	finalize_body(g, b, f, stages, lane);
	if (stages & SMHV_STAGE_FIRING) firing_after_finalize(bp, f, lane);
}

}
```

### squad-mortar-helper_amd/csrc/smh_runtime.cpp

```cpp
#include <hip/hip_runtime.h>

#include <atomic>
#include <condition_variable>
#include <deque>
#include <thread>
#include <cmath>
#include <cstdarg>
#include <cstdio>
#include <cstdlib>
#include <cstring>
#include <ctime>
#include <sched.h>
#include <pthread.h>
#include <cctype>
#include <mutex>
#include <vector>
#include <new>
#include <string>

#include "smh_consts.h"
#include "smh_kernels.h"

using namespace smh;

// ... 599 lines not shown
	o->ocr_pitch = g.ocr_pitch; o->ocr_stride = g.ocr_stride; o->ocr_offset = g.q_xoff;
	o->scales_pitch = g.ocr_pitch; o->scales_stride = g.ocr_stride; o->scales_offset = g.q_xoff;
	o->bits_pitch_words = g.bits_pitch_w; o->bits_stride = g.bits_stride_w * 4; o->bits_xoff = g.m_xoff;
	return SMHV_OK;
}

extern "C" SMHV_API int smhv_batch_enable_timing(smhv_batch *b, int enable) {
	if (!b) return fail(SMHV_E_INVALID, "null batch");
	if (enable && !b->ev) {
		HIPCHK(hipSetDevice(b->ctx->device));
		b->ev = new hipEvent_t[smhv_batch::TIMING_RING][smhv_batch::TIMING_EVENTS]();
		for (int r = 0; r < smhv_batch::TIMING_RING; ++r)
			for (int i = 0; i < smhv_batch::TIMING_EVENTS; ++i) HIPCHK(hipEventCreate(&b->ev[r][i]));
	}
	b->timing = enable != 0;
	b->timed_runs = 0;
	return SMHV_OK;
}

static void hm_release(smhv_heightmap *hm) {
	if (!hm || hm->refs.fetch_sub(1, std::memory_order_acq_rel) != 1) return;
	(void)hipSetDevice(hm->ctx->device);
	(void)hipDeviceSynchronize();
	if (hm->d) (void)hipFree(hm->d);
	if (uint32_t *l = hm->d_lut.load(std::memory_order_acquire)) (void)hipFree(l);
	ctx_release(hm->ctx);
	delete hm;
}

static smhv_firing_options firing_opts(const smhv_firing_options *opt) {
	smhv_firing_options o{};
	o.size = sizeof o;
	if (opt) { o.flags = opt->flags; o.viewport_scale[0] = opt->viewport_scale[0]; o.viewport_scale[1] = opt->viewport_scale[1];
	           o.viewport_top_left[0] = opt->viewport_top_left[0]; o.viewport_top_left[1] = opt->viewport_top_left[1]; }
	if (o.viewport_scale[0] == 0.0f) o.viewport_scale[0] = 1.0f;
	if (o.viewport_scale[1] == 0.0f) o.viewport_scale[1] = 1.0f;
	return o;
}

static void firing_run_params(const smhv_heightmap *hm, const smhv_firing_options *o, FiringRun *r) {
	memset(r, 0, sizeof *r);
	if (hm) {
		r->hm = hm->d; r->hm_w = hm->w; r->hm_h = hm->h;
		r->b0x = (float)hm->bounds[0]; r->b0y = (float)hm->bounds[1];
		r->zscale = (double)hm->scale[2] / 0.1953125;
	}
	r->flags = o->flags;
	r->sw = o->viewport_scale[0] == 0.0f ? 1.0f : o->viewport_scale[0];
	r->sh = o->viewport_scale[1] == 0.0f ? 1.0f : o->viewport_scale[1];
	r->tx = o->viewport_top_left[0]; r->ty = o->viewport_top_left[1];
}

static void firing_bind(smhv_batch *b, smhv_heightmap *hm, const smhv_firing_options *opt) {
	b->fire_opt = firing_opts(opt);
	if (b->fire_hm == hm) return;
	hm_retain(hm);
	smhv_heightmap *old = b->fire_hm;
	b->fire_hm = hm;
	hm_release(old);
}

static int check_firing_options(const smhv_firing_options *opt) {
	if (opt && opt->size != 0u && opt->size < sizeof(smhv_firing_options)) return fail(SMHV_E_INVALID, "smhv_firing_options.size %u < %zu", opt->size, sizeof(smhv_firing_options));
	if (opt && (opt->flags & ~SMHV_FIRING_BOUNDS_OFFSET)) return fail(SMHV_E_INVALID, "unknown firing flags 0x%x", opt->flags);
	return SMHV_OK;
}

static int firing_upload(smhv_batch *b, hipStream_t sb) {
	if (!b->d_firing) {
		hipError_t e = hipMalloc((void **)&b->d_firing, sizeof(smhv_firing_result) * (size_t)b->max_frames);
		if (e == hipSuccess) e = hipMalloc((void **)&b->d_fire_run, sizeof(FiringRun));
		if (e == hipSuccess) e = hipMemset(b->d_firing, 0, sizeof(smhv_firing_result) * (size_t)b->max_frames);
		if (e != hipSuccess) {
			if (b->d_firing) (void)hipFree(b->d_firing);
			if (b->d_fire_run) (void)hipFree(b->d_fire_run);
			b->d_firing = nullptr; b->d_fire_run = nullptr;
			return fail(SMHV_E_HIP, "firing slab: %s", hipGetErrorString(e));
		}
	}
	smhv_batch::FireStage *st = nullptr;
	for (auto &a : b->fire_stage)
		if (hipEventQuery(a.done) == hipSuccess) { st = &a; break; }
	if (!st) {
		smhv_batch::FireStage a;
		hipError_t e = hipHostMalloc((void **)&a.h, sizeof(FiringRun));
		if (e == hipSuccess) e = hipEventCreateWithFlags(&a.done, hipEventDisableTiming);
		if (e != hipSuccess) { if (a.h) (void)hipHostFree(a.h); return fail(SMHV_E_HIP, "firing staging: %s", hipGetErrorString(e)); }
		b->fire_stage.push_back(a);
		st = &b->fire_stage.back();
	}
	firing_run_params(b->fire_hm, &b->fire_opt, st->h);
	st->h->out = b->d_firing;
	HIPCHK(hipMemcpyAsync(b->d_fire_run, st->h, sizeof(FiringRun), hipMemcpyHostToDevice, sb));
	HIPCHK(hipEventRecord(st->done, sb));
	return SMHV_OK;
}

static int hm_lut(const smhv_heightmap *hm, const uint32_t **lut) {
	uint32_t *l = hm->d_lut.load(std::memory_order_acquire);
	if (!l) {
		std::lock_guard<std::mutex> lk(hm->lut_mu);
		l = hm->d_lut.load(std::memory_order_relaxed);
		if (!l) {
			HIPCHK(hipSetDevice(hm->ctx->device));
			hipStream_t s = nullptr;
			hipError_t e = hipMalloc((void **)&l, sizeof(uint32_t) * SMH_HM_LUT_WORDS);
			if (e == hipSuccess) e = hipStreamCreateWithFlags(&s, hipStreamNonBlocking);
			if (e == hipSuccess) e = launch_heightmap_lut(hm->d, (uint64_t)hm->w * hm->h, l + SMH_HM_LUT_ENTRIES, l, s);
			if (e == hipSuccess) e = launch_heightmap_lut16(l, (uint16_t *)(l + SMH_HM_LUT_ENTRIES + 4u), l + SMH_HM_LUT_ENTRIES + 2u, s);
			if (e == hipSuccess) e = hipStreamSynchronize(s);
			if (s) (void)hipStreamDestroy(s);
			if (e != hipSuccess) {
				if (l) (void)hipFree(l);
				return fail(SMHV_E_HIP, "heightmap overlay colour table: %s", hipGetErrorString(e));
			}
			hm->d_lut.store(l, std::memory_order_release);
		}
	}
	*lut = l;
	return SMHV_OK;
}

static int overlay_prepare(smhv_batch *b, const smhv_heightmap *hm, uint32_t flags, const smhv_frame_result *res, hipStream_t s, OverlayRun *r) {
	const uint32_t *lut = nullptr;
	int rc = hm_lut(hm, &lut);
	if (rc) return rc;
	if (!b->d_overlay) {
		const size_t bytes = b->g.ui_stride * (size_t)b->max_frames;
		hipError_t e = hipMalloc((void **)&b->d_overlay, bytes);
		if (e == hipSuccess) e = hipMemsetAsync(b->d_overlay, 0, bytes, s);
		if (e != hipSuccess) {
			if (b->d_overlay) (void)hipFree(b->d_overlay);
			b->d_overlay = nullptr;
			return fail(SMHV_E_HIP, "overlay slab: %s", hipGetErrorString(e));
		}
	}
	memset(r, 0, sizeof *r);
	r->ui = b->d_ui; r->out = b->d_overlay; r->aux = b->d_aux; r->res = res;
	r->hm = hm->d; r->lut = lut; r->hm_w = hm->w; r->hm_h = hm->h;
	r->b0x = (float)hm->bounds[0]; r->b0y = (float)hm->bounds[1];
	r->flags = flags;
	return SMHV_OK;
}

static int check_overlay_stages(uint32_t stages, const smhv_heightmap *hm) {
	if (!(stages & SMHV_STAGE_HEIGHTMAP_OVERLAY)) return SMHV_OK;
	if ((stages & (SMHV_STAGE_UI_MAP | SMHV_STAGE_MINIMAP)) != (SMHV_STAGE_UI_MAP | SMHV_STAGE_MINIMAP))
		return fail(SMHV_E_INVALID, "SMHV_STAGE_HEIGHTMAP_OVERLAY needs SMHV_STAGE_UI_MAP and SMHV_STAGE_MINIMAP");
	if (!hm) return fail(SMHV_E_INVALID, "SMHV_STAGE_HEIGHTMAP_OVERLAY needs a heightmap (smhv_batch_set_firing / smhv_pipeline_set_firing)");
	return SMHV_OK;
}

struct SvcPublish { SvcCtl *ctl; unsigned long long *ring; SvcSlot *slots; uint32_t slot, seq, ring_log2; const uint32_t *cull_tab; bool have_cull; hipStream_t s_pro; hipEvent_t ev_pro;
                    bool *published; };
static int batch_run_impl(smhv_batch *b, const void *d_frames, uint32_t n, uint32_t stages, int grayscale, uint32_t max_gap,
                          const smhv_anchors *anchors, hipStream_t s, hipStream_t sl, const SvcPublish *svc = nullptr) {
	if (!b || !d_frames || n == 0 || n > b->max_frames) return fail(SMHV_E_INVALID, "bad arguments (n=%u, capacity %u)", n, b ? b->max_frames : 0);
	CTX_OPEN(b->ctx);
	if ((stages & (SMHV_STAGE_ALL | SMHV_STAGE_MINIMAP)) == 0) return fail(SMHV_E_INVALID, "no stage selected");
	if ((stages & SMHV_STAGE_FIRING) && !(stages & SMHV_STAGE_MARKERS)) return fail(SMHV_E_INVALID, "SMHV_STAGE_FIRING needs SMHV_STAGE_MARKERS");
	{ int rc = check_overlay_stages(stages, b->fire_hm); if (rc) return rc; }
	stages &= SMHV_STAGE_ALL | SMHV_STAGE_MINIMAP | SMHV_STAGE_EXACT_STATS | SMHV_STAGE_LSD_HELPERS | SMHV_STAGE_FIRING | SMHV_STAGE_HEIGHTMAP_OVERLAY;
	HIPCHK(hipSetDevice(b->ctx->device));
	const Geom &g = b->g;
	Buffers bf = make_buffers(b, (const uint8_t *)d_frames, 0);
	OverlayRun orun{};
	if (stages & SMHV_STAGE_HEIGHTMAP_OVERLAY) {
		int rc = overlay_prepare(b, b->fire_hm, b->fire_opt.flags, bf.results, s, &orun);
		if (rc) return rc;
	}
	if ((bf.co.epoch & 0xFFFFu) == 0u && b->d_farm) HIPCHK(hipMemsetAsync(b->d_farm, 0, sizeof(FarmFrame) * (size_t)b->max_frames, s));
	if (stages & SMHV_STAGE_LSD_HELPERS) bf.co.ctl = (LsdCtl *)b->d_lsd_ctl;
	if (svc && svc->have_cull) bf.cull_tab = svc->cull_tab;
	else if ((stages & SMHV_STAGE_MARKERS) && !(stages & SMHV_STAGE_EXACT_STATS)) {
		int rc = sector_table_for(b->ctx, max_gap, s, &bf);
		if (rc) return rc;
	}
	const bool scales = (stages & SMHV_STAGE_SCALES) && anchors;
	const hipStream_t sb = (svc && svc->s_pro) ? svc->s_pro : s;
	if (scales) {
		smhv_batch::AnchorStage *st = nullptr;
		for (auto &a : b->anchor_stage)
			if (hipEventQuery(a.done) == hipSuccess) { st = &a; break; }
		if (!st) {
			smhv_batch::AnchorStage a;
			hipError_t e = hipHostMalloc((void **)&a.h, sizeof(smhv_anchors) * b->max_frames);
			if (e == hipSuccess) e = hipEventCreateWithFlags(&a.done, hipEventDisableTiming);
			if (e != hipSuccess) { if (a.h) (void)hipHostFree(a.h); return fail(SMHV_E_HIP, "anchor staging: %s", hipGetErrorString(e)); }
			b->anchor_stage.push_back(a);
			st = &b->anchor_stage.back();
		}
		memcpy(st->h, anchors, sizeof(smhv_anchors) * n);
		HIPCHK(hipMemcpyAsync(b->d_anchors, st->h, sizeof(smhv_anchors) * n, hipMemcpyHostToDevice, sb));
		HIPCHK(hipEventRecord(st->done, sb));
	}
	if (stages & SMHV_STAGE_FIRING) {
		int rc = firing_upload(b, sb);
		if (rc) return rc;
		bf.firing = b->d_fire_run;
	}
	const bool t = b->timing;
	hipEvent_t *ev = t ? b->ev[b->timed_runs % smhv_batch::TIMING_RING] : nullptr;
#define STAGE_BEGIN(i, st) do { if (t) HIPCHK(hipEventRecord(ev[2 * (i)], (st))); } while (0)
#define STAGE_END(i, st) do { if (t) HIPCHK(hipEventRecord(ev[2 * (i) + 1], (st))); } while (0)
	STAGE_BEGIN(0, sb);
	HIPCHK(launch_button(g, bf, n, 0, sb));
	STAGE_END(0, sb);
	if (sb != s) {
		HIPCHK(hipEventRecord(svc->ev_pro, sb));
		HIPCHK(hipStreamWaitEvent(s, svc->ev_pro, 0));
	}
	uint32_t mflags = 0, qflags = 0;
	if (stages & SMHV_STAGE_MARKERS) mflags |= MAP_MASK;
	if (stages & SMHV_STAGE_UI_MAP) mflags |= MAP_UI;
	if (stages & SMHV_STAGE_OCR) qflags |= BRQ_OCR;
	if (scales) qflags |= BRQ_SCALES;
	if (b->probe) HIPCHK(hipEventRecord(b->ev_probe[0], s));
	STAGE_BEGIN(1, s);
	if (mflags && qflags) HIPCHK(launch_map_brq_pass(g, bf, n, mflags, qflags, grayscale, 0, 1, s, &b->tune));
	else if (mflags) HIPCHK(launch_map_pass(g, bf, n, mflags, grayscale, s, true, b->tune.map_overlapped != 0u));
	STAGE_END(1, s);
	if (mflags & MAP_UI) { b->ui_written = true; b->ui_gray = grayscale != 0; }
	if (mflags & MAP_MASK) b->mask_written = true;
	if (qflags & BRQ_OCR) b->ocr_written = true;
	if (qflags & BRQ_SCALES) b->scales_written = true;
	STAGE_BEGIN(2, s);
	if (qflags && !mflags) HIPCHK(launch_brq_pass(g, bf, n, qflags, 0, 1, s));
	STAGE_END(2, s);
	if (!svc) HIPCHK(hipEventRecord(b->ev_map_done, s));
	if (b->probe) HIPCHK(hipEventRecord(b->ev_probe[1], s));
	if (sl != s) HIPCHK(hipStreamWaitEvent(sl, b->ev_map_done, 0));
	const bool skip_lsd = g_skip_lsd.load(std::memory_order_relaxed);
	if (svc) {
		if (stages & SMHV_STAGE_MINIMAP) HIPCHK(launch_find_minimap(g, bf, n, s));
		if (stages & SMHV_STAGE_HEIGHTMAP_OVERLAY) HIPCHK(launch_hm_overlay(g, orun, n, s));
		bf.rec_stages = SMH_REC_ON | (scales ? stages : (stages & ~SMHV_STAGE_SCALES));
		bf.rec_bars = b->d_bars;
		STAGE_BEGIN(3, s);
		HIPCHK(launch_svc_publish(svc->ctl, svc->ring, svc->slots, svc->slot, bf, n, svc->seq, svc->ring_log2, s));
		if (svc->published) *svc->published = true;
		STAGE_END(3, s);
		STAGE_BEGIN(4, s);
		STAGE_END(4, s);
		if (t) b->timed_runs++;
		return SMHV_OK;
	}
	STAGE_BEGIN(3, sl);
	const uint32_t late_kc = b->lsd_late_kc;
	if (late_kc > 0u) { bf.lsd_flags |= SMH_LSD_LATE_HELP; bf.lsd_late_kc = late_kc; }
	bool record_fused = false;
	if (!(stages & SMHV_STAGE_MINIMAP)) {
		bf.rec_stages = SMH_REC_ON | (scales ? stages : (stages & ~SMHV_STAGE_SCALES));
		bf.rec_bars = b->d_bars;
	}
	if ((stages & SMHV_STAGE_MARKERS) && !skip_lsd) HIPCHK(launch_lsd(g, bf, n, (float)max_gap, 0, 0.0f, 0.0f, sl, b->lsd_fork.s1 ? &b->lsd_fork : nullptr, b->lsd_bs, b->lsd_prefer_classic,
	                                                      (mflags && qflags) ? b->tune.lsd_tile_limit : 0u,
	                                                      &record_fused));
	STAGE_END(3, sl);
	if (b->probe) { HIPCHK(hipEventRecord(b->ev_probe[2], sl)); b->probe_valid = (stages & SMHV_STAGE_MARKERS) && mflags; }
	if (stages & SMHV_STAGE_MINIMAP) HIPCHK(launch_find_minimap(g, bf, n, sl));
	if (stages & SMHV_STAGE_HEIGHTMAP_OVERLAY) HIPCHK(launch_hm_overlay(g, orun, n, sl));
	STAGE_BEGIN(4, sl);
	if (record_fused) {  }
	else if (scales) HIPCHK(launch_scales_finalize(g, bf, n, stages, b->d_bars, sl));
	else HIPCHK(launch_finalize(g, bf, n, stages & ~SMHV_STAGE_SCALES, sl));
	STAGE_END(4, sl);
#undef STAGE_BEGIN
#undef STAGE_END
	if (t) b->timed_runs++;
	return SMHV_OK;
}

extern "C" SMHV_API int smhv_batch_run(smhv_batch *b, const void *d_frames, uint32_t n, uint32_t stages, int grayscale, uint32_t max_gap,
                                       const smhv_anchors *anchors, void *stream) {
	return batch_run_impl(b, d_frames, n, stages, grayscale, max_gap, anchors, (hipStream_t)stream, (hipStream_t)stream);
}

extern "C" SMHV_API int smhv_debug_pattern_copy(smhv_batch *b, const void *d_frames, uint32_t n, uint32_t rows_in_flight, void *stream) {
	if (!b || !d_frames || n == 0 || n > b->max_frames || (rows_in_flight != 0u && rows_in_flight != 4u && rows_in_flight != 8u && rows_in_flight != 12u))
		return fail(SMHV_E_INVALID, "bad arguments (rows in flight: 0 = 4, 4, 8, 12)");
	CTX_OPEN(b->ctx);
	HIPCHK(hipSetDevice(b->ctx->device));
	const Buffers bf = make_buffers(b, (const uint8_t *)d_frames, 0);
	HIPCHK(launch_pattern_copy(b->g, bf, n, rows_in_flight, (hipStream_t)stream));
	return SMHV_OK;
}

extern "C" SMHV_API int smhv_batch_wait_map_pass(smhv_batch *b, void *stream) {
	if (!b) return fail(SMHV_E_INVALID, "null batch");
	HIPCHK(hipSetDevice(b->ctx->device));
	HIPCHK(hipStreamWaitEvent((hipStream_t)stream, b->ev_map_done, 0));
	return SMHV_OK;
}

extern "C" SMHV_API int smhv_batch_set_scales_stream(smhv_batch *b, void *stream) {
	if (!b) return fail(SMHV_E_INVALID, "null batch");
	(void)stream;
	return SMHV_OK;
}

extern "C" SMHV_API int smhv_batch_stage_ms(smhv_batch *b, float ms[5]) {
	if (!b || !ms) return fail(SMHV_E_INVALID, "bad arguments");
	if (!b->ev || b->timed_runs == 0) return fail(SMHV_E_STATE, "no timed smhv_batch_run since timing was enabled");
	const uint64_t runs = b->timed_runs < (uint64_t)smhv_batch::TIMING_RING ? b->timed_runs : (uint64_t)smhv_batch::TIMING_RING;
	double acc[5] = {0, 0, 0, 0, 0};
	for (uint64_t r = 0; r < runs; ++r) {
		hipEvent_t *ev = b->ev[(b->timed_runs - 1 - r) % smhv_batch::TIMING_RING];
		for (int i = 0; i < 5; ++i) {
			float m = 0;
			HIPCHK(hipEventSynchronize(ev[2 * i + 1]));
			HIPCHK(hipEventElapsedTime(&m, ev[2 * i], ev[2 * i + 1]));
			acc[i] += m;
		}
	}
	for (int i = 0; i < 5; ++i) ms[i] = (float)(acc[i] / (double)runs);
	b->timed_runs = 0;
	return SMHV_OK;
}

extern "C" SMHV_API int smhv_batch_lsd_coop_stats(smhv_batch *b, uint32_t first, uint32_t n, uint32_t *out) {
	if (!b || !out || (uint64_t)first + n > b->max_frames) return fail(SMHV_E_INVALID, "bad arguments");
	HIPCHK(hipSetDevice(b->ctx->device));
	HIPCHK(hipDeviceSynchronize());
	std::vector<LsdCoop> h(n);
	HIPCHK(hipMemcpy(h.data(), b->d_lsd_ctl + sizeof(LsdCtl) + sizeof(LsdCoop) * (size_t)first, sizeof(LsdCoop) * n, hipMemcpyDeviceToHost));
	for (uint32_t i = 0; i < n; ++i) { out[4 * i] = h[i].stat_groups; out[4 * i + 1] = h[i].stat_hits; out[4 * i + 2] = h[i].stat_casts; out[4 * i + 3] = h[i].req_tail; }
	return SMHV_OK;
}

extern "C" SMHV_API int smhv_batch_device_ptrs(smhv_batch *b, void **r, void **ui, void **mask, void **ocr, void **scales, void **bits) {
	if (!b) return fail(SMHV_E_INVALID, "null batch");
	if (r) *r = b->d_results;
	if (ui) *ui = b->d_ui;
	if (mask) *mask = b->d_mask;
	if (ocr) *ocr = b->d_ocr;
	if (scales) *scales = b->d_scales;
	if (bits) *bits = b->d_bits;
	return SMHV_OK;
}

extern "C" SMHV_API int smhv_batch_tile_mask(smhv_batch *b, void **d_tiled, void **d_occ, uint32_t geometry[4]) {
	if (!b) return fail(SMHV_E_INVALID, "null batch");
	if (d_tiled) *d_tiled = b->d_tiled;
	if (d_occ) *d_occ = b->d_occ;
	if (geometry) { geometry[0] = tiled_rows(b->g); geometry[1] = b->g.bits_pitch_w; geometry[2] = occ_pitch(b->g); geometry[3] = b->g.m_xoff; }
	return SMHV_OK;
}

extern "C" SMHV_API int smhv_batch_read_tile_mask(smhv_batch *b, uint32_t frame, uint32_t *tiled, uint8_t *occ, uint32_t *bits, int *written) {
	if (!b || frame >= b->max_frames) return fail(SMHV_E_INVALID, "bad arguments");
	HIPCHK(hipSetDevice(b->ctx->device));
	HIPCHK(hipDeviceSynchronize());
	const Geom &g = b->g;
	if (tiled) HIPCHK(hipMemcpy(tiled, b->d_tiled + (size_t)frame * tiled_stride_w(g), tiled_stride_w(g) * 4, hipMemcpyDeviceToHost));
	if (occ) HIPCHK(hipMemcpy(occ, b->d_occ + (size_t)frame * occ_stride(g), occ_stride(g), hipMemcpyDeviceToHost));
	if (bits) HIPCHK(hipMemcpy(bits, b->d_bits + (size_t)frame * g.bits_stride_w, g.bits_stride_w * 4, hipMemcpyDeviceToHost));
	if (written) {
		FrameAux a;
		HIPCHK(hipMemcpy(&a, b->d_aux + frame, sizeof a, hipMemcpyDeviceToHost));
		*written = a.tiles ? 1 : 0;
	}
	return SMHV_OK;
}

extern "C" SMHV_API int smhv_batch_read_results(smhv_batch *b, uint32_t first, uint32_t n, smhv_frame_result *out) {
	if (!b || !out || (uint64_t)first + n > b->max_frames) return fail(SMHV_E_INVALID, "bad arguments");
	HIPCHK(hipSetDevice(b->ctx->device));
	HIPCHK(hipDeviceSynchronize());
	HIPCHK(hipMemcpy(out, b->d_results + first, sizeof(smhv_frame_result) * n, hipMemcpyDeviceToHost));
	return batch_check_errors(b, "batch_read_results");
}

static int copy_image_d2h(smhv_ctx *c, int slot, uint8_t *dst, const uint8_t *d_rows, size_t pitch, size_t xoff, size_t width, size_t rows, hipStream_t s) {
	const size_t bytes = pitch * rows;
	if (c->h_stage_cap[slot] < bytes) {
		if (c->h_stage[slot]) { (void)hipHostFree(c->h_stage[slot]); c->h_stage[slot] = nullptr; c->h_stage_cap[slot] = 0; }
		HIPCHK(hipHostMalloc((void **)&c->h_stage[slot], bytes, hipHostMallocDefault));
		c->h_stage_cap[slot] = bytes;
	}
	HIPCHK(hipMemcpyAsync(c->h_stage[slot], d_rows, bytes, hipMemcpyDeviceToHost, s));
	HIPCHK(wait_stream(s));
	for (size_t r = 0; r < rows; ++r) memcpy(dst + r * width, c->h_stage[slot] + r * pitch + xoff, width);
	return SMHV_OK;
}

extern "C" SMHV_API int smhv_batch_read_image(smhv_batch *b, int which, uint32_t frame, uint8_t *out) {
	if (!b || !out || frame >= b->max_frames) return fail(SMHV_E_INVALID, "bad arguments");
	CTX_OPEN(b->ctx);
	const Geom &g = b->g;
	HIPCHK(hipSetDevice(b->ctx->device));
	HIPCHK(hipDeviceSynchronize());
	if (which == SMHV_IMAGE_HEIGHTMAP_OVERLAY && !b->d_overlay) return fail(SMHV_E_STATE, "batch_read_image: no run of this batch had SMHV_STAGE_HEIGHTMAP_OVERLAY");
// ... 228 lines not shown
		if (e == hipSuccess) e = hipMalloc((void **)&p->d_svc_ctl, sizeof(SvcCtl));
		if (e == hipSuccess) e = hipMemset(p->d_svc_ctl, 0, sizeof(SvcCtl));
		if (e == hipSuccess) e = hipMalloc((void **)&p->d_svc_ring, sizeof(unsigned long long) << lg);
		if (e == hipSuccess) e = hipMemset(p->d_svc_ring, 0, sizeof(unsigned long long) << lg);
		if (e == hipSuccess) e = hipMalloc((void **)&p->d_svc_slots, sizeof(SvcSlot) * depth);
		if (e == hipSuccess) e = hipMemset(p->d_svc_slots, 0, sizeof(SvcSlot) * depth);
		if (!(opt.flags & (SMHV_PIPE_NO_REMOTE_HELP | SMHV_PIPE_NO_TEAM_HELP)) && (uint64_t)p->svc_wgs * p->svc_waves <= 0xFFFFu) {
			const size_t owners = (size_t)p->svc_wgs * p->svc_waves;
			p->svc_store_words = svc_store_words_for(g0, p->svc_tile_cap, p->svc_compact);
			if (e == hipSuccess) e = hipMalloc((void **)&p->d_svc_remote, sizeof(SvcRemote) * owners);
			if (e == hipSuccess) e = hipMemset(p->d_svc_remote, 0, sizeof(SvcRemote) * owners);
			if (e == hipSuccess) e = hipMalloc((void **)&p->d_svc_store, sizeof(uint32_t) * owners * p->svc_store_words);
		}
	}
	if (e != hipSuccess) { smhv_pipeline_destroy(p); return fail(SMHV_E_HIP, "pipeline streams / events: %s", hipGetErrorString(e)); }
	for (uint32_t i = 0; i < depth; ++i) {
		int rc = smhv_batch_create(c, W, H, max_frames, &p->batch[i]);
		if (rc) { smhv_pipeline_destroy(p); return rc; }
		p->batch[i]->lsd_bs = depth >= 2 ? 512u : 1024u;
		p->batch[i]->lsd_prefer_classic = depth == 2 && lsd_rows_only(p->batch[i]->g);
		if (p->svc && !p->adaptive) {
			p->batch[i]->tune.map_prio = (opt.flags & SMHV_PIPE_NO_STREAM_PRIORITY) ? 0u : 1u;
			p->batch[i]->tune.map_deep = (opt.flags & SMHV_PIPE_THREE_LOAD_SETS) ? 1u : 0u;
			p->batch[i]->tune.map_overlapped = 1u;
		} else if (depth >= 3) {
			if (opt.occupancy_policy != 2u) p->tuning = pipeline_tuning(p->batch[i]->g);
			p->batch[i]->tune = p->tuning;
			p->batch[i]->tune.map_overlapped = 1u;
			if (opt.late_helpers == 1u) p->batch[i]->lsd_late_kc = 20u;
			if (opt.occupancy_policy == 0u) {
				p->adapt = true;
				hipError_t e2 = hipSuccess;
				for (int k = 0; k < 3 && e2 == hipSuccess; ++k) e2 = hipEventCreate(&p->batch[i]->ev_probe[k]);
				if (e2 != hipSuccess) { smhv_pipeline_destroy(p); return fail(SMHV_E_HIP, "pipeline probe events: %s", hipGetErrorString(e2)); }
				p->batch[i]->probe = true;
			}
		}
	}
	*out = p;
	return SMHV_OK;
}

extern "C" SMHV_API int smhv_pipeline_create(smhv_ctx *c, uint32_t W, uint32_t H, uint32_t max_frames, uint32_t depth, smhv_pipeline **out) {
	return pipeline_create_impl(c, W, H, max_frames, depth, nullptr, out);
}

extern "C" SMHV_API int smhv_pipeline_create_ex(smhv_ctx *c, uint32_t W, uint32_t H, uint32_t max_frames, uint32_t depth, const smhv_pipeline_options *opt, smhv_pipeline **out) {
	return pipeline_create_impl(c, W, H, max_frames, depth, opt, out);
}

static inline bool svc_alive(smhv_pipeline *p) { return (uint32_t)__atomic_load_n(&p->h_svc->state, __ATOMIC_ACQUIRE) != 0u; }

static int svc_launch(smhv_pipeline *p, uint32_t slot) {
	SvcParams sp;
	sp.ctl = p->d_svc_ctl; sp.ring = p->d_svc_ring; sp.slots = p->d_svc_slots; sp.host = p->d_svc_host;
	sp.cull_tab = p->svc_cull; sp.ray_off = p->ctx->d_ray_off; sp.max_gap = (float)p->svc_max_gap;
	sp.tile_cap = p->svc_tile_cap; sp.list_cap = p->svc_list_cap; sp.part_words = p->svc_part_words; sp.ring_log2 = p->svc_ring_log2;
	sp.epoch = ++p->svc_epoch;
	if (sp.epoch == 0u) sp.epoch = ++p->svc_epoch;
	sp.idle_short = p->opt.idle_close_us ? p->opt.idle_close_us * 2u : 100u;
	sp.flags = (p->opt.flags & SMHV_PIPE_NO_TEAM_HELP) ? 8u : 0u;
	sp.idle_long = 50000u;
	if (p->opt.flags & SMHV_PIPE_HELP_FIRST) sp.flags |= 16u;
	if (p->opt.flags & SMHV_PIPE_WALK_BIT_ROWS) sp.flags |= 32u;

	sp.remote = p->d_svc_remote; sp.remote_store = p->d_svc_store; sp.remote_store_words = p->svc_store_words;
	sp.remote_after = p->opt.remote_after ? p->opt.remote_after : 24u;
	sp.remote_tickets = std::min<uint32_t>(p->opt.remote_tickets ? p->opt.remote_tickets : 3u, 16u);
	sp.remote_last_div = p->opt.remote_last ? p->opt.remote_last : 6u;
	sp.compact = p->svc_compact;
	__atomic_fetch_or(&p->h_svc->state, (unsigned long long)sp.epoch, __ATOMIC_ACQ_REL);
	hipError_t e = hipStreamWaitEvent(p->s_search, p->ev_pub[slot], 0);
	if (e == hipSuccess) e = launch_lsd_service(p->batch[slot]->g, sp, p->svc_wgs, p->svc_waves, p->svc_lds, p->s_search);
	if (e != hipSuccess) {
		__atomic_fetch_and(&p->h_svc->state, 0xFFFFFFFF00000000ull, __ATOMIC_ACQ_REL);
		return fail(SMHV_E_HIP, "launching the line-search service: %s", hipGetErrorString(e));
	}
	p->h_svc->launches++;
	return SMHV_OK;
}

static int svc_wait_slot(smhv_pipeline *p, uint32_t slot) {
	const uint32_t target = p->seq[slot];
	if (target == 0u) return SMHV_OK;
	volatile uint32_t *flag = &p->h_svc->done_seq[slot];
	uint64_t spins = 0;
	struct timespec t0;
	clock_gettime(CLOCK_MONOTONIC, &t0);
	auto reached = [flag, target]() { return (int32_t)(__atomic_load_n(flag, __ATOMIC_ACQUIRE) - target) >= 0; };
	while (!reached()) {
		if (!svc_alive(p)) {
			if (reached()) break;
			int rc = svc_launch(p, slot);
			if (rc) return rc;
		}
		if (++spins < 4000u) { __builtin_ia32_pause(); continue; }
		struct timespec ts = {0, 20000};
		nanosleep(&ts, nullptr);
		if ((spins & 1023u) == 0u) {
			struct timespec t1;
			clock_gettime(CLOCK_MONOTONIC, &t1);
			if (t1.tv_sec - t0.tv_sec > 60) {
				const unsigned long long st = __atomic_load_n(&p->h_svc->state, __ATOMIC_ACQUIRE);
				return fail(SMHV_E_STATE, "pipeline_wait: slot %u (sequence %u, last completed %u) did not complete within 60 s: line-search service stalled "
				            "(submissions %u, launch alive %u, launches %u)", slot, target, *flag, (uint32_t)(st >> 32), (uint32_t)st, p->h_svc->launches);
			}
		}
	}
	return SMHV_OK;
}

static int svc_submit(smhv_pipeline *p, uint32_t slot, const void *d_frames, uint32_t n, uint32_t stages, int grayscale, uint32_t max_gap,
                      const smhv_anchors *anchors, void *after_stream, uint32_t *slot_out) {
	smhv_batch *b = p->batch[slot];
	if (!d_frames || n == 0 || n > b->max_frames) return fail(SMHV_E_INVALID, "bad arguments (n=%u, capacity %u)", n, b->max_frames);
	int rc = slot_wait(p, slot);
	if (rc) return rc;
	if (batch_check_errors(b, "pipeline_submit (the slot's previous submission, never waited for)") != SMHV_OK) logf(p->ctx, 2, "%s", t_last_error.c_str());
	hipStream_t st = p->svc_stream[p->submitted % p->svc_streams];
	if (p->adaptive) { b->tune = LaunchTuning{0u, 0u, 0u, (p->opt.flags & SMHV_PIPE_NO_STREAM_PRIORITY) ? 0u : 1u, (p->opt.flags & SMHV_PIPE_THREE_LOAD_SETS) ? 1u : 0u, 1u}; b->probe = false; b->lsd_late_kc = 0u; }
	Buffers probe{};
	const bool want_cull = (stages & SMHV_STAGE_MARKERS) && !(stages & SMHV_STAGE_EXACT_STATS);
	if (want_cull) { rc = sector_table_for(p->ctx, max_gap, st, &probe); if (rc) return rc; }
	if (!p->svc_key_valid || p->svc_cull != probe.cull_tab || p->svc_max_gap != max_gap) {
		for (uint32_t i = 0; i < p->depth; ++i) { rc = svc_wait_slot(p, i); if (rc) return rc; }
		struct timespec td0;
		clock_gettime(CLOCK_MONOTONIC, &td0);
		for (uint64_t spins = 0; svc_alive(p); ++spins) {
			struct timespec ts = {0, 20000}, td1;
			nanosleep(&ts, nullptr);
			if ((spins & 1023u) == 1023u) {
				clock_gettime(CLOCK_MONOTONIC, &td1);
				if (td1.tv_sec - td0.tv_sec > 60) {
					const unsigned long long stw = __atomic_load_n(&p->h_svc->state, __ATOMIC_ACQUIRE);
					return fail(SMHV_E_STATE, "pipeline_submit: the line-search service did not close within 60 s of its last submission (another gap threshold needs a new launch; "
					            "submissions %u, launch alive %u, launches %u)", (uint32_t)(stw >> 32), (uint32_t)stw, p->h_svc->launches);
				}
			}
		}
		p->svc_key_valid = true; p->svc_cull = probe.cull_tab; p->svc_max_gap = max_gap;
	}
	const hipStream_t s_first = p->s_pro ? p->s_pro : st;
	if (after_stream) {
		HIPCHK(hipEventRecord(p->ev_after, (hipStream_t)after_stream));
		HIPCHK(hipStreamWaitEvent(s_first, p->ev_after, 0));
	}
	if (p->held[slot]) {
		HIPCHK(hipStreamWaitEvent(s_first, p->hold[slot], 0));
		p->held[slot] = 0;
	}
	uint32_t seq = ++p->seq_counter;
	if (seq == 0u) seq = ++p->seq_counter;
	bool published = false;
	SvcPublish pub{p->d_svc_ctl, p->d_svc_ring, p->d_svc_slots, slot, seq, p->svc_ring_log2, probe.cull_tab, true, p->s_pro, p->ev_pro[slot], &published};
	__atomic_fetch_add(&p->h_svc->state, 1ull << 32, __ATOMIC_ACQ_REL);
	rc = batch_run_impl(b, d_frames, n, stages, grayscale, max_gap, anchors, st, st, &pub);
	if (rc && !published) {
		__atomic_fetch_sub(&p->h_svc->state, 1ull << 32, __ATOMIC_ACQ_REL);
		return rc;
	}
	const int rc_late = rc;
	p->seq[slot] = seq;
	p->slot_st[slot] = st;
	p->last_sl[slot] = st;
	p->slot_frame[slot] = 1;
	if (!svc_alive(p)) {
		HIPCHK(hipEventRecord(p->ev_pub[slot], st));
		rc = svc_launch(p, slot);
		if (rc) return rc;
	}
	p->submitted++;
	if (slot_out) *slot_out = slot;
	return rc_late;
}


#define SMH_MODE_RECHECK 16384u
static inline bool same_shape(uint32_t n_a, uint32_t st_a, uint32_t gap_a, uint32_t n_b, uint32_t st_b, uint32_t gap_b) {
	if (st_a != st_b || gap_a != gap_b) return false;
	const uint64_t lo = std::min(n_a, n_b), hi = std::max(n_a, n_b);
	return hi * 4u <= lo * 5u;
}
#define SMH_MODE_REMEASURE_CAP 4u
static int mode_control(smhv_pipeline *p, uint32_t n, uint32_t stages, uint32_t max_gap) {
	smhv_pipeline::ModeCtl &m = p->mc;
	const uint32_t W = 8u * p->depth;
	auto begin = [&m]() { m.count = 0; m.frames = 0; m.window_mixed = false; clock_gettime(CLOCK_MONOTONIC, &m.t0); };
	auto rate = [&m]() {
		struct timespec t1;
		clock_gettime(CLOCK_MONOTONIC, &t1);
		const double dt = (double)(t1.tv_sec - m.t0.tv_sec) + 1e-9 * (double)(t1.tv_nsec - m.t0.tv_nsec);
		return dt > 0.0 ? (double)m.frames / dt : 0.0;
	};
	const bool same = m.key_n == 0u || same_shape(n, stages, max_gap, m.key_n, m.key_stages, m.key_gap);
	if (m.key_n == 0u) { m.key_n = n; m.key_stages = stages; m.key_gap = max_gap; }
	if (m.phase == 4) {
		if (same) m.cand_count = 0;
		else {
			if (m.cand_count && same_shape(n, stages, max_gap, m.cand_n, m.cand_stages, m.cand_gap)) m.cand_count++;
			else { m.cand_n = n; m.cand_stages = stages; m.cand_gap = max_gap; m.cand_count = 1; }
			if (m.cand_count >= p->depth && m.remeasured < SMH_MODE_REMEASURE_CAP) {
				m.key_n = m.cand_n; m.key_stages = m.cand_stages; m.key_gap = m.cand_gap;
				m.cand_count = 0; m.remeasured++;
				m.phase = 0; m.count = 0;
			}
		}
	} else if (!same) m.window_mixed = true;
	int rc = SMHV_OK;
	switch (m.phase) {
	case 0:
		if (m.count >= 2u * p->depth) { m.phase = 1; begin(); }
		break;
	case 1:
		if (m.count >= W) {
			if (m.window_mixed) { m.key_n = n; m.key_stages = stages; m.key_gap = max_gap; begin(); break; }
			m.rate[p->mode_frame ? 1 : 0] = rate(); p->mode_frame = !p->mode_frame; m.phase = 2; m.count = 0;
		}
		break;
	case 2:
		if (m.count >= 6u * p->depth) { m.phase = 3; begin(); }
		break;
	case 3:
		if (m.count >= W) {
			if (m.window_mixed) { m.key_n = n; m.key_stages = stages; m.key_gap = max_gap; begin(); break; }
			m.rate[p->mode_frame ? 1 : 0] = rate();
			p->mode_frame = !(m.rate[0] > 1.03 * m.rate[1]);
			m.decisions++;
			m.phase = 4; m.count = 0; m.settle = SMH_MODE_RECHECK;
			logf(p->ctx, 3, "pipeline: frame-granular search %.0f frames/s, batch-granular %.0f -> %s", m.rate[1], m.rate[0], p->mode_frame ? "frame-granular" : "batch-granular");
		}
		break;
	default:
		if (m.count >= m.settle) { m.phase = 1; m.remeasured = 0; begin(); }
		break;
	}
	return rc;
}

extern "C" SMHV_API int smhv_pipeline_submit(smhv_pipeline *p, const void *d_frames, uint32_t n, uint32_t stages, int grayscale, uint32_t max_gap,
                                             const smhv_anchors *anchors, void *after_stream, uint32_t *slot_out) {
	if (!p) return fail(SMHV_E_INVALID, "null pipeline");
	CTX_OPEN(p->ctx);
	HIPCHK(hipSetDevice(p->ctx->device));
	const uint32_t slot = (uint32_t)(p->submitted % p->depth);
	if (stages & SMHV_STAGE_HEIGHTMAP_OVERLAY) {
		int rc = check_overlay_stages(stages, p->fire_hm);
		const uint32_t *lut = nullptr;
		if (!rc) rc = hm_lut(p->fire_hm, &lut);
		if (rc) return rc;
	}
	if (stages & (SMHV_STAGE_FIRING | SMHV_STAGE_HEIGHTMAP_OVERLAY)) firing_bind(p->batch[slot], p->fire_hm, &p->fire_opt);
	if (p->adaptive) { int rc = mode_control(p, n, stages, max_gap); if (rc) return rc; }
	if (p->svc && p->mode_frame) {
		int rc = svc_submit(p, slot, d_frames, n, stages, grayscale, max_gap, anchors, after_stream, slot_out);
		if (!rc && p->adaptive) { p->mc.count++; p->mc.frames += n; }
		return rc;
	}
	{ int rc = slot_wait(p, slot); if (rc) return rc; }
	if (batch_check_errors(p->batch[slot], "pipeline_submit (the slot's previous submission, never waited for)") != SMHV_OK)
		logf(p->ctx, 2, "%s", t_last_error.c_str());
	if (p->adapt) {
		smhv_batch *bb = p->batch[slot];
		if (bb->probe_valid) {
			float map_ms = 0.0f, lsd_ms = 0.0f;
			if (hipEventElapsedTime(&map_ms, bb->ev_probe[0], bb->ev_probe[1]) == hipSuccess &&
			    hipEventElapsedTime(&lsd_ms, bb->ev_probe[1], bb->ev_probe[2]) == hipSuccess && map_ms > 0.0f) {
				const float ratio = lsd_ms / map_ms;
				p->ratio_ema = p->ratio_ema == 0.0f ? ratio : 0.75f * p->ratio_ema + 0.25f * ratio;
				if (p->tune_on && p->ratio_ema > SMH_ADAPT_OFF) p->tune_on = false;
				else if (!p->tune_on && p->ratio_ema < SMH_ADAPT_ON) p->tune_on = true;
			}
			bb->probe_valid = false;
		}
		bb->tune = p->tune_on ? p->tuning : LaunchTuning{0u, 0u, 0u, 0u, 0u, 0u};
		bb->tune.map_overlapped = 1u;
		bb->lsd_late_kc = p->opt.late_helpers == 2u ? 0u : (p->opt.late_helpers == 1u ? 20u : (p->tune_on ? 0u : SMH_LATE_KC_SEARCH_BOUND));
		bb->probe = (p->submitted / p->depth) % 4u == 0u || (p->adaptive && p->mc.phase != 4u);
	}
	if (p->adaptive && !p->adapt) {
		p->batch[slot]->tune = p->tuning;
		p->batch[slot]->tune.map_overlapped = 1u;
		p->batch[slot]->lsd_late_kc = p->opt.late_helpers == 1u ? 20u : 0u;
	}
	hipStream_t st, sl;
	{
		st = sl = p->stream[slot];
		bool idle = true;
		for (uint32_t i = 0; i < p->depth && idle; ++i) idle = hipEventQuery(p->done[i]) == hipSuccess;
		if (idle) p->round_start = p->submitted;
		const uint64_t k = p->submitted - p->round_start;
		if (k > 0 && k < p->depth) {
			const uint32_t prev = (uint32_t)((p->submitted - 1) % p->depth);
			HIPCHK(hipStreamWaitEvent(st, p->batch[prev]->ev_map_done, 0));
		}
	}
	if (after_stream) {
		HIPCHK(hipEventRecord(p->ev_after, (hipStream_t)after_stream));
		HIPCHK(hipStreamWaitEvent(st, p->ev_after, 0));
	}
	if (p->held[slot]) {
		HIPCHK(hipStreamWaitEvent(st, p->hold[slot], 0));
		p->held[slot] = 0;
	}
	if (p->depth == 1 && lsd_rows_only(p->batch[slot]->g)) stages |= SMHV_STAGE_LSD_HELPERS;
	int rc = batch_run_impl(p->batch[slot], d_frames, n, stages, grayscale, max_gap, anchors, st, sl);
	if (rc) return rc;
	HIPCHK(hipEventRecord(p->done[slot], sl));
	p->last_sl[slot] = sl;
	p->slot_frame[slot] = 0;
	p->submitted++;
	if (p->adaptive) { p->mc.count++; p->mc.frames += n; }
	if (slot_out) *slot_out = slot;
	return SMHV_OK;
}

extern "C" SMHV_API int smhv_pipeline_wait(smhv_pipeline *p, uint32_t slot) {
	if (!p || slot >= p->depth) return fail(SMHV_E_INVALID, "pipeline_wait: bad arguments");
	HIPCHK(hipSetDevice(p->ctx->device));
	{ int rc = slot_wait(p, slot); if (rc) return rc; }
	return batch_check_errors(p->batch[slot], "pipeline_wait");
}

extern "C" SMHV_API int smhv_pipeline_wait_all(smhv_pipeline *p) {
	if (!p) return fail(SMHV_E_INVALID, "null pipeline");
	HIPCHK(hipSetDevice(p->ctx->device));
	for (uint32_t i = 0; i < p->depth; ++i) { int r = slot_wait(p, i); if (r) return r; }
	int rc = SMHV_OK;
	for (uint32_t i = 0; i < p->depth; ++i) {
		std::string keep = t_last_error;
		const int r = batch_check_errors(p->batch[i], "pipeline_wait_all");
		if (r && !rc) rc = r;
		else if (r) t_last_error = keep;
	}
	return rc;
}

extern "C" SMHV_API int smhv_debug_pipeline_stats(smhv_pipeline *p, uint64_t out[32]) {
	if (!p || !out) return fail(SMHV_E_INVALID, "bad arguments");
	memset(out, 0, sizeof(uint64_t) * 32);
	if (!p->svc) return SMHV_OK;
	HIPCHK(hipSetDevice(p->ctx->device));
	HIPCHK(hipDeviceSynchronize());
	SvcCtl c;
	HIPCHK(hipMemcpy(&c, p->d_svc_ctl, sizeof c, hipMemcpyDeviceToHost));
	out[0] = 1u; out[1] = p->h_svc->launches; out[2] = c.stat_items; out[3] = c.stat_waves; out[4] = c.stat_busy; out[5] = c.stat_life;
	out[6] = (uint64_t)p->svc_wgs * p->svc_waves; out[7] = c.completed;
	for (int k = 0; k < 4; ++k) out[8 + k] = c.stat_phase[k];
	out[12] = c.stat_help;
	out[16] = c.stat_requests; out[17] = c.stat_attached; out[18] = c.stat_remote; out[19] = (uint64_t)(int64_t)c.help_avail;
	out[20] = c.stat_t_wait; out[21] = c.stat_t_sub; out[22] = c.stat_t_last;
	out[23] = c.stat_h_polls; out[24] = c.stat_h_empty; out[25] = c.stat_h_lost; out[26] = c.stat_h_idle_exit; out[27] = c.stat_h_closed_exit; out[28] = c.stat_h_cycles; out[29] = c.stat_h_cast_cycles;
	out[13] = (p->adaptive ? 2u : 0u) | (p->mode_frame ? 1u : 0u) | (p->mc.phase == 4u ? 4u : 0u); out[14] = (uint64_t)p->mc.rate[1]; out[15] = (uint64_t)p->mc.rate[0];
	return SMHV_OK;
}

extern "C" SMHV_API int smhv_debug_pipeline_peek(smhv_pipeline *p, uint64_t out[16]) {
	if (!p || !out) return fail(SMHV_E_INVALID, "bad arguments");
	memset(out, 0, sizeof(uint64_t) * 16);
	if (!p->svc) return SMHV_OK;
	HIPCHK(hipSetDevice(p->ctx->device));
	const unsigned long long st = __atomic_load_n(&p->h_svc->state, __ATOMIC_ACQUIRE);
	out[0] = st >> 32; out[1] = (uint32_t)st; out[2] = p->h_svc->launches; out[3] = p->seq_counter;
	out[14] = ((uint64_t)p->svc_wgs << 32) | p->svc_waves; out[15] = ((uint64_t)p->svc_part_words << 32) | p->svc_lds;
	std::lock_guard<std::mutex> lk(p->peek_mu);
	if (!p->s_peek) HIPCHK(hipStreamCreateWithFlags(&p->s_peek, hipStreamNonBlocking));
	if (!p->h_peek) HIPCHK(hipHostMalloc((void **)&p->h_peek, sizeof(SvcCtl)));
	SvcCtl *h_ctl = p->h_peek;
	HIPCHK(hipMemcpyAsync(h_ctl, p->d_svc_ctl, sizeof(SvcCtl), hipMemcpyDeviceToHost, p->s_peek));
	HIPCHK(hipStreamSynchronize(p->s_peek));
	out[4] = (uint64_t)(int64_t)h_ctl->avail; out[5] = h_ctl->head; out[6] = h_ctl->reserve; out[7] = h_ctl->closing; out[8] = h_ctl->completed; out[9] = h_ctl->busy;
	for (uint32_t i = 0; i < 4 && i < p->depth; ++i) out[10 + i] = ((uint64_t)p->seq[i] << 32) | __atomic_load_n(&p->h_svc->done_seq[i], __ATOMIC_ACQUIRE);
	return SMHV_OK;
}

extern "C" SMHV_API int smhv_pipeline_hold(smhv_pipeline *p, uint32_t slot, void *stream) {
	if (!p || slot >= p->depth) return fail(SMHV_E_INVALID, "pipeline_hold: bad arguments");
	HIPCHK(hipSetDevice(p->ctx->device));
	HIPCHK(hipEventRecord(p->hold[slot], (hipStream_t)stream));
	p->held[slot] = 1;
	return SMHV_OK;
}

extern "C" SMHV_API int smhv_pipeline_slot(smhv_pipeline *p, uint32_t slot, smhv_batch **batch, void **stream) {
	if (!p || slot >= p->depth) return fail(SMHV_E_INVALID, "pipeline_slot: bad arguments");
	if (batch) *batch = p->batch[slot];
	if (stream && p->svc && (p->slot_frame[slot] || p->stream.empty())) {
		HIPCHK(hipSetDevice(p->ctx->device));
		int rc = svc_wait_slot(p, slot);
		if (rc) return rc;
		*stream = (void *)(p->slot_st[slot] ? p->slot_st[slot] : p->svc_stream[0]);
		return SMHV_OK;
	}
	if (stream) *stream = (void *)(p->last_sl[slot] ? p->last_sl[slot] : p->stream[slot]);
	return SMHV_OK;
}

static int ensure_frame_buffers(smhv_ctx *c, uint32_t w, uint32_t h) {
	if (c->fb && c->W == w && c->H == h) return SMHV_OK;
	std::lock_guard<std::mutex> lk(c->mu);
	Geom g;
	int rc = compute_geom(w, h, &g);
	if (rc) return rc;
	HIPCHK(hipDeviceSynchronize());
	if (c->fb) { smhv_batch_destroy(c->fb); c->fb = nullptr; }
	if (c->h_ocr) { (void)hipHostFree(c->h_ocr); c->h_ocr = nullptr; }
	if (c->h_scales) { (void)hipHostFree(c->h_scales); c->h_scales = nullptr; }
	rc = smhv_batch_create(c, w, h, 1, &c->fb);
	if (rc) return rc;
	HIPCHK(hipHostMalloc((void **)&c->h_ocr, (size_t)g.qw * g.qh));
	HIPCHK(hipHostMalloc((void **)&c->h_scales, (size_t)g.qw * g.qh));
	memset(c->h_scales, 0, (size_t)g.qw * g.qh);
	memset(c->h_ocr, 0, (size_t)g.qw * g.qh);
	c->W = w; c->H = h;
	logf(c, 3, "allocated buffers for %ux%u frames (map ROI %u,%u %ux%u)", w, h, g.rx, g.ry, g.rw, g.rh);
	return SMHV_OK;
}

struct TraitTimer {
	smhv_ctx *c; int idx; struct timespec t0;
	TraitTimer(smhv_ctx *c_, int idx_) : c(c_), idx(idx_) { clock_gettime(CLOCK_MONOTONIC, &t0); }
	~TraitTimer() {
		if (!c) return;
		struct timespec t1;
		clock_gettime(CLOCK_MONOTONIC, &t1);
		c->tt_ns[idx].fetch_add((uint64_t)((t1.tv_sec - t0.tv_sec) * 1000000000ll + (t1.tv_nsec - t0.tv_nsec)), std::memory_order_relaxed);
		c->tt_calls[idx].fetch_add(1u, std::memory_order_relaxed);
	}
};
extern "C" SMHV_API int smhv_trait_times(smhv_ctx *c, uint64_t ns[SMHV_TRAIT_CALLS], uint64_t calls[SMHV_TRAIT_CALLS], int reset) {
	if (!c) return fail(SMHV_E_INVALID, "null context");
	for (int i = 0; i < SMHV_TRAIT_CALLS; ++i) {
		if (ns) ns[i] = c->tt_ns[i].load(std::memory_order_relaxed);
		if (calls) calls[i] = c->tt_calls[i].load(std::memory_order_relaxed);
		if (reset) { c->tt_ns[i].store(0, std::memory_order_relaxed); c->tt_calls[i].store(0, std::memory_order_relaxed); }
	}
	return SMHV_OK;
}

static void reset_frame_state(smhv_ctx *c) {
	c->have_frame = true; c->cropped = false; c->map_open = false; c->isolated = false; c->mask_valid = false; c->minimap_cached = false;
}

extern "C" SMHV_API int smhv_load_frame(smhv_ctx *c, const uint8_t *bgra, uint32_t w, uint32_t h) {
	TraitTimer tt_(c, SMHV_T_LOAD_FRAME);
	if (!c || !bgra || w == 0 || h == 0) return fail(SMHV_E_INVALID, "bad arguments");
	CTX_OPEN(c);
	HIPCHK(hipSetDevice(c->device));
	int rc = ensure_frame_buffers(c, w, h);
	if (rc) return rc;
	const size_t bytes = (size_t)w * h * 4;
	if (c->d_frame_cap < bytes) {
		HIPCHK(hipDeviceSynchronize());
		if (c->d_frame) (void)hipFree(c->d_frame);
		c->d_frame = nullptr; c->d_frame_cap = 0;
		HIPCHK(hipMalloc((void **)&c->d_frame, bytes));
		c->d_frame_cap = bytes;
	}
	const Geom &g = c->fb->g;
	const uint32_t y0 = g.ry < g.by ? g.ry : g.by;
	const uint32_t y1 = (g.ry + g.rh > g.by + g.bh) ? g.ry + g.rh : g.by + g.bh;
	const size_t off = (size_t)y0 * w * 4, len = (size_t)(y1 - y0) * w * 4;
	HIPCHK(hipMemcpyAsync(c->d_frame + off, bgra + off, len, hipMemcpyHostToDevice, c->s_main));
	HIPCHK(wait_stream(c->s_main));
	c->frame_ptr = c->d_frame;
	reset_frame_state(c);
	return SMHV_OK;
}

extern "C" SMHV_API int smhv_load_frame_view(smhv_ctx *c, const uint8_t *parent_bgra, uint32_t parent_w, uint32_t parent_h,
                                              uint32_t x, uint32_t y, uint32_t w, uint32_t h) {
	if (!c || !parent_bgra || w == 0 || h == 0) return fail(SMHV_E_INVALID, "bad arguments");
	if ((uint64_t)x + w > parent_w || (uint64_t)y + h > parent_h)
		return fail(SMHV_E_INVALID, "load_frame_view: the view %ux%u+%u+%u does not lie inside its %ux%u parent", w, h, x, y, parent_w, parent_h);
	if (x == 0 && w == parent_w) return smhv_load_frame(c, parent_bgra + (size_t)y * parent_w * 4, w, h);
	CTX_OPEN(c);
	HIPCHK(hipSetDevice(c->device));
	int rc = ensure_frame_buffers(c, w, h);
	if (rc) return rc;
	const size_t bytes = (size_t)w * h * 4;
	if (c->d_frame_cap < bytes) {
		HIPCHK(hipDeviceSynchronize());
		if (c->d_frame) (void)hipFree(c->d_frame);
		c->d_frame = nullptr; c->d_frame_cap = 0;
		HIPCHK(hipMalloc((void **)&c->d_frame, bytes));
		c->d_frame_cap = bytes;
	}
	const Geom &g = c->fb->g;
	const uint32_t y0 = g.ry < g.by ? g.ry : g.by;
	const uint32_t y1 = (g.ry + g.rh > g.by + g.bh) ? g.ry + g.rh : g.by + g.bh;
	const uint8_t *src = parent_bgra + ((size_t)(y + y0) * parent_w + x) * 4;
	HIPCHK(hipMemcpy2DAsync(c->d_frame + (size_t)y0 * w * 4, (size_t)w * 4, src, (size_t)parent_w * 4, (size_t)w * 4, y1 - y0, hipMemcpyHostToDevice, c->s_main));
	HIPCHK(wait_stream(c->s_main));
	c->frame_ptr = c->d_frame;
	reset_frame_state(c);
	return SMHV_OK;
}

extern "C" SMHV_API int smhv_load_frame_device(smhv_ctx *c, const void *d_bgra, uint32_t w, uint32_t h) {
	TraitTimer tt_(c, SMHV_T_LOAD_FRAME);
	if (!c || !d_bgra || w == 0 || h == 0) return fail(SMHV_E_INVALID, "bad arguments");
	CTX_OPEN(c);
	HIPCHK(hipSetDevice(c->device));
	int rc = ensure_frame_buffers(c, w, h);
	if (rc) return rc;
// ... 1330 lines not shown
```

### squad-mortar-helper_amd/csrc/smh_service.inc

```
#pragma once

struct SvcKernelArgs { Geom g; SvcParams p; };
#ifdef __HIP_DEVICE_COMPILE__
typedef const __attribute__((address_space(4))) SvcSlot *SvcSlotPtr;
typedef const __attribute__((address_space(4))) SvcKernelArgs *SvcKernelArgsPtr;
#else
typedef const SvcSlot *SvcSlotPtr;
typedef const SvcKernelArgs *SvcKernelArgsPtr;
#endif
__device__ __forceinline__ SvcKernelArgsPtr svc_args(const void *ka) {
	const unsigned long long v = (unsigned long long)(uintptr_t)ka;
	const uint32_t lo = (uint32_t)__builtin_amdgcn_readfirstlane((int)(uint32_t)v), hi = (uint32_t)__builtin_amdgcn_readfirstlane((int)(uint32_t)(v >> 32));
	return (SvcKernelArgsPtr)(uintptr_t)(((unsigned long long)hi << 32) | lo);
}

#define SVC_WS_WORDS ((uint32_t)((sizeof(WShared) + 15u) / 16u * 4u))
#define SVC_POLL_SLEEP 64

__device__ __forceinline__ uint32_t svc_ld(const uint32_t *p) { return __hip_atomic_load(p, __ATOMIC_RELAXED, __HIP_MEMORY_SCOPE_AGENT); }

__device__ __forceinline__ uint32_t *lds_ptr(uint32_t byte_off) { return (uint32_t *)(LdsWord *)(uintptr_t)uniform_u32(byte_off); }
__device__ __forceinline__ uint32_t lds_off(const void *p) { return (uint32_t)(uintptr_t)(const LdsByte *)p; }

template <bool COMPACT>
__device__ __attribute__((noinline)) void svc_frame_global(const void *kargs, uint32_t slot, uint32_t f, uint32_t part_off, uint32_t cull_off, uint32_t dirs_off) {
	SvcKernelArgsPtr ka = svc_args(kargs);
	slot = uniform_u32(slot); f = uniform_u32(f);
	uint32_t *part = lds_ptr(part_off);
	const Geom g = ka->g;
	const Buffers b = ((SvcSlotPtr)(ka->p.slots + slot))->b;
	const FrameAux aux = b.aux[f];
	lsd_frame_seq<LSD_MODE_GLOBAL, true>(g, b, f, ka->p.max_gap, aux, part + SVC_WS_WORDS, *(WShared *)part, lds_ptr(cull_off), (const RayDir *)lds_ptr(dirs_off), 0u, ka->p.list_cap);
}

template <bool COMPACT>
__device__ __attribute__((noinline)) unsigned long long svc_frame(const void *kargs, uint32_t slot, uint32_t f, uint32_t part_off, uint32_t cull_off, uint32_t dirs_off) {
	SvcKernelArgsPtr ka = svc_args(kargs);
	slot = uniform_u32(slot); f = uniform_u32(f);
	uint32_t *part = lds_ptr(part_off);
	const Geom g = ka->g;
	const Buffers b = ((SvcSlotPtr)(ka->p.slots + slot))->b;
	const FrameAux aux = b.aux[f];
	WShared &ws = *(WShared *)part;
	uint32_t *smem = part + SVC_WS_WORDS;
	if (!aux.open || aux.n_mask_px == 0) {
		if ((threadIdx.x & 63u) == 0) { b.results[f].n_lines = 0; b.results[f].rounds = 0; b.results[f].ray_steps = 0; b.results[f].status = SMHV_FRAME_OK; }
	} else {
		const uint32_t tile_cap = ka->p.tile_cap;
		if ((threadIdx.x & 63u) == 0) {
			SvcSlot *sl = ka->p.slots + slot;
			ws.rem_done = (unsigned long long)(uintptr_t)&sl->done;
			ws.rem_n = __hip_atomic_load(&sl->n, __ATOMIC_RELAXED, __HIP_MEMORY_SCOPE_AGENT);
		}
		FrameView v;
		bool fits;
		if constexpr (COMPACT) {
			uint32_t rc = 2u;
			if (b.tiled && aux.tiles && !(ka->p.flags & 32u)) rc = frame_setup_tilec_occ(g, b, f, aux, smem, tile_cap, &ws.ntiles, v, smem + tilec_mask_words(g.rw, g.rh, tile_cap), 2u * ka->p.list_cap + W_WIN_STRIDE);
			fits = rc == 2u ? frame_setup_tilec(g, b, f, aux, smem, tile_cap, &ws.ntiles, v) : rc == 0u;
		} else {
			uint32_t rc = 2u;
			if (b.tiled && aux.tiles && !(ka->p.flags & 32u)) rc = frame_setup_tile_occ(g, b, f, aux, smem, tile_cap, &ws.ntiles, v, smem + tile_mask_words(g.rw, g.rh, tile_cap), 2u * ka->p.list_cap + W_WIN_STRIDE);
			fits = rc == 2u ? frame_setup_tile<true>(g, b, f, aux, smem, tile_cap, &ws.ntiles, v) : rc == 0u;
		}
		if (fits) {
			if constexpr (COMPACT) lsd_frame_seq<LSD_MODE_TILEC, true, true>(g, b, f, ka->p.max_gap, aux, smem, ws, lds_ptr(cull_off), (const RayDir *)lds_ptr(dirs_off), tilec_mask_words(g.rw, g.rh, tile_cap), ka->p.list_cap, &v);
			else lsd_frame_seq<LSD_MODE_TILE, true, true>(g, b, f, ka->p.max_gap, aux, smem, ws, lds_ptr(cull_off), (const RayDir *)lds_ptr(dirs_off), tile_mask_words(g.rw, g.rh, tile_cap), ka->p.list_cap, &v);
		} else svc_frame_global<COMPACT>(kargs, slot, f, part_off, cull_off, dirs_off);
	}
	const unsigned long long t_search_end = __builtin_amdgcn_s_memtime();
	if (b.rec_stages & SMH_REC_ON) frame_record_tail_wave(&((const SvcKernelArgs *)kargs)->g, &((const SvcSlot *)(ka->p.slots + slot))->b, f);
	return t_search_end;
}

#define SVC_HELP_IDLE_POLLS 160u
template <bool COMPACT>
__device__ __attribute__((noinline)) void svc_help(const void *kargs, uint32_t owner_off, uint32_t my_off, uint32_t cull_off, uint32_t dirs_off) {
	SvcKernelArgsPtr ka = svc_args(kargs);
	uint32_t *opart = lds_ptr(owner_off), *mpart = lds_ptr(my_off);
	WShared &wo = *(WShared *)opart;
	const uint32_t lane = threadIdx.x & 63u;
	uint32_t ok = 0;
	if (lane == 0 && W_LD_ACQ(&wo.want_set) && W_LD(&wo.late) < SEQ_MAX_HELPERS) {
		const uint32_t prev = __hip_atomic_fetch_add(&wo.late, 1u, __ATOMIC_ACQ_REL, __HIP_MEMORY_SCOPE_WORKGROUP);
		if (prev < SEQ_MAX_HELPERS && W_LD_ACQ(&wo.want_set)) ok = 1u;
		else __hip_atomic_fetch_sub(&wo.late, 1u, __ATOMIC_RELEASE, __HIP_MEMORY_SCOPE_WORKGROUP);
	}
	if (!uniform_u32(ok)) return;
	const uint32_t rw = ka->g.rw, rh = ka->g.rh, tile_cap = ka->p.tile_cap, list_cap = ka->p.list_cap;
	const float max_gap = ka->p.max_gap;
	const bool cull = ka->p.cull_tab != nullptr && max_gap > 0.0f && max_gap <= 49.0f;
	const float *ray_off = ka->p.ray_off;
	Win m;
	if constexpr (COMPACT) tilec_win(m, rw, rh, opart + SVC_WS_WORDS, tile_cap); else tile_win(m, rw, rh, opart + SVC_WS_WORDS, tile_cap);
	uint32_t *wwin = mpart + SVC_WS_WORDS + (COMPACT ? tilec_mask_words(rw, rh, tile_cap) : tile_mask_words(rw, rh, tile_cap)) + 2u * list_cap;
	const uint32_t *cull_tab = lds_ptr(cull_off);
	const RayDir *dirs = (const RayDir *)lds_ptr(dirs_off);
	uint32_t idle = 0;
	while (uniform_u32(W_LD_ACQ(&wo.want_set))) {
		uint32_t key = 0u;
		if (lane < SEQ_HELP_SLOTS && W_LD_ACQ(&wo.rob[lane].state) == (uint32_t)H_POSTED) key = ~((wo.rob[lane].lines_seen << 2) | lane);
		key = wave_max32_dpp(key);
		if (!key) {
			if (++idle > SVC_HELP_IDLE_POLLS) break;
			__builtin_amdgcn_s_sleep(8);
			continue;
		}
		WSlot &sl = wo.rob[~key & 3u];
		uint32_t got = 0;
		if (lane == 0) { uint32_t expect = H_POSTED; got = __hip_atomic_compare_exchange_strong(&sl.state, &expect, (uint32_t)H_TAKEN, __ATOMIC_ACQ_REL, __ATOMIC_RELAXED, __HIP_MEMORY_SCOPE_WORKGROUP) ? 1u : 0u; }
		if (!uniform_u32(got)) continue;
		idle = 0;
		const uint32_t px = uniform_u32(sl.px), py = uniform_u32(sl.py);
		float xs, ys, ex0, ey0;
		unsigned long long wkey;
		uint32_t st_sum;
#ifdef SMH_LSD_WDEBUG
		unsigned long long sprof[8] = {0, 0, 0, 0, 0, 0, 0, 0}, slast = __builtin_amdgcn_s_memtime(), uprof[12] = {0, 0, 0, 0, 0, 0, 0, 0, 0, 0, 0, 0};
		uint32_t n_units = 0;
		seq_cast_candidate<COMPACT ? LSD_MODE_TILEC : LSD_MODE_TILE>(m, wwin, cull_tab, cull, dirs, ray_off, max_gap, px, py, xs, ys, wkey, ex0, ey0, st_sum, sprof, slast, uprof, n_units);
#else
		seq_cast_candidate<COMPACT ? LSD_MODE_TILEC : LSD_MODE_TILE>(m, wwin, cull_tab, cull, dirs, ray_off, max_gap, px, py, xs, ys, wkey, ex0, ey0, st_sum);
#endif
		if (lane == 0) {
			sl.ptx = xs; sl.pty = ys; sl.best = wkey; sl.ex = ex0; sl.ey = ey0; sl.steps = st_sum;
			W_ST_REL(&sl.state, (uint32_t)H_DONE);
		}
	}
	if (lane == 0) __hip_atomic_fetch_sub(&wo.late, 1u, __ATOMIC_RELEASE, __HIP_MEMORY_SCOPE_WORKGROUP);
}

#define SVC_REMOTE_IDLE_POLLS 12u
#define SVC_REMOTE_IDLE_POLLS_FREE 600u
#define SVC_REMOTE_MAX_HELPERS 12u
template <bool COMPACT>
__device__ __attribute__((noinline)) void svc_help_remote(const void *kargs, uint32_t ticket, uint32_t my_off, uint32_t cull_off, uint32_t dirs_off) {
	SvcKernelArgsPtr ka = svc_args(kargs);
	ticket = uniform_u32(ticket);
	const uint32_t owner = ticket & 0xFFFFu, gen16 = ticket >> 16;
	SvcRemote *r = ka->p.remote + owner;
	const uint32_t lane = threadIdx.x & 63u;
	uint32_t ok = 0, gen = 0;
	if (lane == 0) {
		unsigned long long st = g_ld64(&r->state);
		while ((st & SVC_REMOTE_OPEN) && ((uint32_t)(st >> 32) & 0xFFFFu) == gen16 && ((uint32_t)st & 0x7FFFFFFFu) < SVC_REMOTE_MAX_HELPERS) {
			if (__hip_atomic_compare_exchange_strong(&r->state, &st, st + 1ull, __ATOMIC_ACQ_REL, __ATOMIC_RELAXED, __HIP_MEMORY_SCOPE_AGENT)) { ok = 1u; gen = (uint32_t)(st >> 32); break; }
		}
	}
	if (!uniform_u32(ok)) return;
	gen = uniform_u32(gen);
	if (lane == 0) __hip_atomic_fetch_add(&ka->p.ctl->stat_attached, 1u, __ATOMIC_RELAXED, __HIP_MEMORY_SCOPE_AGENT);
	__builtin_amdgcn_fence(__ATOMIC_ACQUIRE, "agent");
	const uint32_t rw = ka->g.rw, rh = ka->g.rh, tile_cap = ka->p.tile_cap, list_cap = ka->p.list_cap;
	const uint32_t ntiles = min(uniform_u32((uint32_t)g_ld64(&r->info)), tile_cap);
	uint32_t *mpart = lds_ptr(my_off), *store = mpart + SVC_WS_WORDS;
	{
		const uint4 *src = (const uint4 *)(ka->p.remote_store + (size_t)owner * ka->p.remote_store_words);
		uint4 *dst = (uint4 *)store;
		for (uint32_t i = lane; i < (ntiles + 1u) * 2u; i += 64u) dst[i] = src[i];
		const uint32_t q0 = (tile_cap + 1u) * 2u, nq = ((COMPACT ? tilec_idx_words(rw, rh) : tile_idx_words(rw, rh)) + 3u) / 4u;
		for (uint32_t i = lane; i < nq; i += 64u) dst[q0 + i] = src[q0 + i];
	}
	wave_lds_sync();
	const float max_gap = ka->p.max_gap;
	const bool cull = ka->p.cull_tab != nullptr && max_gap > 0.0f && max_gap <= 49.0f;
	const float *ray_off = ka->p.ray_off;
	Win m;
	if constexpr (COMPACT) tilec_win(m, rw, rh, store, tile_cap); else tile_win(m, rw, rh, store, tile_cap);
	uint32_t *wwin = store + (COMPACT ? tilec_mask_words(rw, rh, tile_cap) : tile_mask_words(rw, rh, tile_cap)) + 2u * list_cap;
	const uint32_t *cull_tab = lds_ptr(cull_off);
	const RayDir *dirs = (const RayDir *)lds_ptr(dirs_off);
	uint32_t idle = 0, n_cast = 0, n_polls = 0, n_empty = 0, n_lost = 0, exit_idle = 0;
	unsigned long long t_cast = 0ull;
	const unsigned long long t_att = __builtin_amdgcn_s_memtime();
	while (true) {
		++n_polls;
		const unsigned long long st = g_ld64(&r->state);
		unsigned long long pw = 0ull, cw = 0ull;
		if (lane < SVC_REMOTE_RING) { pw = g_ld64(&r->ring[lane].post); cw = g_ld64(&r->ring[lane].claim); }
		if (!(uniform_u32((uint32_t)st) & (uint32_t)SVC_REMOTE_OPEN) || uniform_u32((uint32_t)(st >> 32)) != gen) break;
		const uint32_t pk = (uint32_t)(pw >> 32);
		const bool open_post = lane < SVC_REMOTE_RING && pk != 0u && (unsigned long long)pk > cw;
		const uint32_t key = wave_max32_dpp(open_post ? ~pk : 0u);
		if (!key) {
			const int32_t waiting = (int32_t)uniform_u32((uint32_t)__hip_atomic_load(&ka->p.ctl->avail, __ATOMIC_RELAXED, __HIP_MEMORY_SCOPE_AGENT));
			++n_empty;
			if (++idle > (waiting > 0 ? SVC_REMOTE_IDLE_POLLS : SVC_REMOTE_IDLE_POLLS_FREE)) { exit_idle = 1u; break; }
			if (idle < 4u) __builtin_amdgcn_s_sleep(24); else __builtin_amdgcn_s_sleep(72);
			continue;
		}
		const uint32_t k = ~key;
		const uint32_t e = (uint32_t)__builtin_ctzll(__ballot(open_post && pk == k));
		uint32_t mine = 0;
		if (lane == 0) mine = __hip_atomic_fetch_max(&r->ring[e].claim, (unsigned long long)k, __ATOMIC_RELAXED, __HIP_MEMORY_SCOPE_AGENT) < (unsigned long long)k ? 1u : 0u;
		if (!uniform_u32(mine)) { ++n_lost; continue; }
		idle = 0;
		const unsigned long long t_c0 = __builtin_amdgcn_s_memtime();
		const uint32_t pxy = (uint32_t)__builtin_amdgcn_readlane((int)(uint32_t)pw, (int)e);
		const uint32_t px = pxy & 0xFFFFu, py = pxy >> 16;
		float xs, ys, ex0, ey0;
		unsigned long long wkey;
		uint32_t st_sum;
#ifdef SMH_LSD_WDEBUG
		unsigned long long sprof[8] = {0, 0, 0, 0, 0, 0, 0, 0}, slast = __builtin_amdgcn_s_memtime(), uprof[12] = {0, 0, 0, 0, 0, 0, 0, 0, 0, 0, 0, 0};
		uint32_t n_units = 0;
		seq_cast_candidate<COMPACT ? LSD_MODE_TILEC : LSD_MODE_TILE>(m, wwin, cull_tab, cull, dirs, ray_off, max_gap, px, py, xs, ys, wkey, ex0, ey0, st_sum, sprof, slast, uprof, n_units);
#else
		seq_cast_candidate<COMPACT ? LSD_MODE_TILEC : LSD_MODE_TILE>(m, wwin, cull_tab, cull, dirs, ray_off, max_gap, px, py, xs, ys, wkey, ex0, ey0, st_sum);
#endif
		++n_cast;
		t_cast += __builtin_amdgcn_s_memtime() - t_c0;
		if (lane == 0) {
			SvcRemoteEntry *en = &r->ring[e];
			const rem_u32x4 a = {k, st_sum, (uint32_t)(wkey >> 32), (uint32_t)wkey};
			const rem_u32x4 b = {k, __float_as_uint(ex0), __float_as_uint(ey0), ((uint32_t)(ys * 2.0f) << 16) | ((uint32_t)(xs * 2.0f) & 0xFFFFu)};
			g_st128(en->res_a, a);
			g_st128(en->res_b, b);
		}
	}
	asm volatile("s_waitcnt vmcnt(0)" ::: "memory");
	if (lane == 0) {
		__hip_atomic_fetch_sub(&r->state, 1ull, __ATOMIC_RELEASE, __HIP_MEMORY_SCOPE_AGENT);
		SvcCtl *ctl = ka->p.ctl;
		__hip_atomic_fetch_add(&ctl->stat_remote, n_cast, __ATOMIC_RELAXED, __HIP_MEMORY_SCOPE_AGENT);
// ... 42 lines not shown
			}
		}
		uint32_t got = 0, ticket = 0;
		if ((int32_t)(uint32_t)look > 0 && lane == 0) {
			if (__hip_atomic_fetch_sub(&ctl->avail, 1, __ATOMIC_ACQUIRE, __HIP_MEMORY_SCOPE_AGENT) > 0) {
				ticket = __hip_atomic_fetch_add(&ctl->head, 1u, __ATOMIC_RELAXED, __HIP_MEMORY_SCOPE_AGENT);
				got = 1u;
			} else __hip_atomic_fetch_add(&ctl->avail, 1, __ATOMIC_RELAXED, __HIP_MEMORY_SCOPE_AGENT);
		}
		got = uniform_u32(got);
		if (got) {
			ticket = uniform_u32(ticket);
			const unsigned long long *e = p.ring + (ticket & ((1u << p.ring_log2) - 1u));
			const uint32_t gen = (ticket >> p.ring_log2) + 1u;
			unsigned long long w;
			while ((uint32_t)((w = __hip_atomic_load(e, __ATOMIC_RELAXED, __HIP_MEMORY_SCOPE_AGENT)) >> 32) != gen) __builtin_amdgcn_s_sleep(2);
			if (lane == 0) __hip_atomic_fetch_add(&ctl->busy, 1u, __ATOMIC_RELAXED, __HIP_MEMORY_SCOPE_AGENT);
			return uniform_u32((uint32_t)w);
		}
		const uint32_t naps = polls < 8u ? 1u : (polls < 32u ? 4u : 16u);
		for (uint32_t k = 0; k < naps; ++k) {
			if (team_smem && svc_sibling_in_need(team_smem, p.part_words, nw, me) != 0xFFFFFFFFu) return 0xFFFFFFFEu;
			if (polls < 8u) __builtin_amdgcn_s_sleep(SVC_POLL_SLEEP); else __builtin_amdgcn_s_sleep(127);
		}
		++polls;
		if (checker && polls >= 8u && (polls & 3u) == 0u) {
			const unsigned long long idle = (__builtin_amdgcn_s_memtime() - t_idle0) >> 10;
			if (idle >= p.idle_short) {
				uint32_t leave = 0;
				if (lane == 0) {
					unsigned long long st = __hip_atomic_load(&p.host->state, __ATOMIC_RELAXED, __HIP_MEMORY_SCOPE_SYSTEM);
					if ((uint32_t)st != p.epoch) {
						__hip_atomic_store(&ctl->closing, p.epoch, __ATOMIC_RELEASE, __HIP_MEMORY_SCOPE_AGENT);
						leave = 1u;
					} else {
						const uint32_t comp = __hip_atomic_load(&ctl->completed, __ATOMIC_RELAXED, __HIP_MEMORY_SCOPE_AGENT);
						const bool quiet = svc_ld(&ctl->busy) == 0u && __hip_atomic_load(&ctl->avail, __ATOMIC_RELAXED, __HIP_MEMORY_SCOPE_AGENT) <= 0;
						const bool drained = quiet && (int32_t)(comp - (uint32_t)(st >> 32)) >= 0;
						const bool stalled = quiet && idle >= p.idle_long;
						if ((drained || stalled) &&
						    __hip_atomic_compare_exchange_strong(&p.host->state, &st, st & 0xFFFFFFFF00000000ull, __ATOMIC_ACQ_REL, __ATOMIC_RELAXED, __HIP_MEMORY_SCOPE_SYSTEM)) {
							__hip_atomic_store(&ctl->closing, p.epoch, __ATOMIC_RELEASE, __HIP_MEMORY_SCOPE_AGENT);
							leave = 1u;
						}
					}
				}
				if (uniform_u32(leave)) return 0xFFFFFFFFu;
			}
		}
	}
}

#define SVC_MAX_WAVES 4
#pragma clang diagnostic push
#pragma clang diagnostic ignored "-Wpass-failed"
template <bool COMPACT>
__device__ __forceinline__ void svc_kernel_body(const Geom &g, const SvcParams &p) {
	extern __shared__ __attribute__((aligned(16))) uint32_t smem[];
	__shared__ uint32_t cull_tab[SMH_CULL_TAB_WORDS];
	__shared__ RayDir s_dirs[SMH_LSD_RAYS];
	const uint32_t lane = threadIdx.x & 63u, wave = threadIdx.x >> 6;
	if (p.cull_tab) for (uint32_t i = threadIdx.x; i < SMH_CULL_TAB_WORDS; i += blockDim.x) cull_tab[i] = p.cull_tab[i];
	for (uint32_t i = threadIdx.x; i < SMH_LSD_RAYS; i += blockDim.x) s_dirs[i] = g_ray_table[i];
	if (lane == 0) {
		WShared &w0 = *(WShared *)(smem + wave * p.part_words);
		w0.want_set = 0u; w0.late = 0u;
		const uint32_t owner = blockIdx.x * (blockDim.x >> 6) + wave;
		const bool rem = p.remote != nullptr && !(p.flags & 8u) && owner < 0x10000u;
		w0.rem_r = rem ? (unsigned long long)(uintptr_t)(p.remote + owner) : 0ull;
		w0.rem_store = (unsigned long long)(uintptr_t)(p.remote_store + (size_t)owner * p.remote_store_words);
		w0.rem_ctl = (unsigned long long)(uintptr_t)p.ctl;
		w0.rem_after = p.remote_after; w0.rem_tickets = p.remote_tickets; w0.rem_owner = owner; w0.rem_cap = p.tile_cap;
		w0.rem_open = 0u; w0.rem_gen = 0u; w0.rem_k = 0u; w0.rem_nr = 0u;
		w0.rem_last_div = p.remote_last_div; w0.rem_flags = (p.flags & 16u) ? 1u : 0u;
	}
	__syncthreads();
	uint32_t *part = smem + wave * p.part_words;
	const uint32_t nw = blockDim.x >> 6;
	const bool team = nw > 1u && !(p.flags & 8u);
	if (p.flags & 4u) __builtin_amdgcn_s_setprio(3);
	const unsigned long long t_start = __builtin_amdgcn_s_memtime();
	unsigned long long t_busy = 0ull, t_help = 0ull, t_phase[4] = {0ull, 0ull, 0ull, 0ull}, rt_wait = 0ull;
	uint32_t n_items = 0u;
	while (true) {
		if (team) {
			const uint32_t sib = svc_sibling_in_need(smem, p.part_words, nw, uniform_u32(wave));
			if (sib != 0xFFFFFFFFu) {
				const unsigned long long t_h = __builtin_amdgcn_s_memtime();
				svc_help<COMPACT>((const void *)__builtin_amdgcn_kernarg_segment_ptr(), sib, lds_off(part), lds_off(cull_tab), lds_off(s_dirs));
				t_help += __builtin_amdgcn_s_memtime() - t_h;
				continue;
			}
		}
		uint32_t help_ticket = 0;
		const uint32_t item = svc_pop(p, team ? smem : nullptr, nw, uniform_u32(wave), blockIdx.x == 0u && uniform_u32(wave) == 0u, &help_ticket);
		if (item == 0xFFFFFFFEu) continue;
		if (item == 0xFFFFFFFDu) {
			const unsigned long long t_h = __builtin_amdgcn_s_memtime();
			svc_help_remote<COMPACT>((const void *)__builtin_amdgcn_kernarg_segment_ptr(), help_ticket, lds_off(part), lds_off(cull_tab), lds_off(s_dirs));
			t_help += __builtin_amdgcn_s_memtime() - t_h;
			continue;
		}
		if (item == 0xFFFFFFFFu) break;
		const unsigned long long t_item = __builtin_amdgcn_s_memtime(), rt_item = __builtin_amdgcn_s_memrealtime();
		const uint32_t slot = item >> 24, f = item & 0xFFFFFFu;
		if (!(p.flags & 1u)) {
			__builtin_amdgcn_fence(__ATOMIC_ACQUIRE, "agent");
			__builtin_amdgcn_s_dcache_inv();
		}
		const unsigned long long t_acq = __builtin_amdgcn_s_memtime();
		const unsigned long long t_srch = svc_frame<COMPACT>((const void *)__builtin_amdgcn_kernarg_segment_ptr(), slot, f, lds_off(part), lds_off(cull_tab), lds_off(s_dirs));
		const unsigned long long t_rec = __builtin_amdgcn_s_memtime();
		if (!(p.flags & 2u)) __builtin_amdgcn_fence(__ATOMIC_RELEASE, "agent");
		if (lane == 0) {
			SvcSlot *sl = p.slots + slot;
			const uint32_t n = __hip_atomic_load(&sl->n, __ATOMIC_RELAXED, __HIP_MEMORY_SCOPE_AGENT), seq = __hip_atomic_load(&sl->seq, __ATOMIC_RELAXED, __HIP_MEMORY_SCOPE_AGENT);
			const unsigned long long t_pub = __hip_atomic_load(&sl->t_pub, __ATOMIC_RELAXED, __HIP_MEMORY_SCOPE_AGENT), rt_now = __builtin_amdgcn_s_memrealtime();
			rt_wait += rt_item - t_pub;
			__hip_atomic_fetch_sub(&p.ctl->busy, 1u, __ATOMIC_RELAXED, __HIP_MEMORY_SCOPE_AGENT);
			if (__hip_atomic_fetch_add(&sl->done, 1u, __ATOMIC_ACQ_REL, __HIP_MEMORY_SCOPE_AGENT) + 1u == n) {
				__hip_atomic_store(&p.host->done_seq[slot], seq, __ATOMIC_RELEASE, __HIP_MEMORY_SCOPE_SYSTEM);
				__hip_atomic_fetch_add(&p.ctl->stat_t_sub, rt_now - t_pub, __ATOMIC_RELAXED, __HIP_MEMORY_SCOPE_AGENT);
				__hip_atomic_fetch_add(&p.ctl->stat_t_last, rt_now - rt_item, __ATOMIC_RELAXED, __HIP_MEMORY_SCOPE_AGENT);
				__hip_atomic_fetch_add(&p.ctl->completed, 1u, __ATOMIC_RELEASE, __HIP_MEMORY_SCOPE_AGENT);
			}
		}
		const unsigned long long t_end = __builtin_amdgcn_s_memtime();
		t_busy += t_end - t_item;
		t_phase[0] += t_acq - t_item; t_phase[1] += t_srch - t_acq; t_phase[2] += t_rec - t_srch; t_phase[3] += t_end - t_rec;
		++n_items;
	}
	if (lane == 0) {
		__hip_atomic_fetch_add(&p.ctl->stat_items, n_items, __ATOMIC_RELAXED, __HIP_MEMORY_SCOPE_AGENT);
		__hip_atomic_fetch_add(&p.ctl->stat_waves, 1u, __ATOMIC_RELAXED, __HIP_MEMORY_SCOPE_AGENT);
		__hip_atomic_fetch_add(&p.ctl->stat_busy, t_busy, __ATOMIC_RELAXED, __HIP_MEMORY_SCOPE_AGENT);
		__hip_atomic_fetch_add(&p.ctl->stat_life, __builtin_amdgcn_s_memtime() - t_start, __ATOMIC_RELAXED, __HIP_MEMORY_SCOPE_AGENT);
		for (int k = 0; k < 4; ++k) __hip_atomic_fetch_add(&p.ctl->stat_phase[k], t_phase[k], __ATOMIC_RELAXED, __HIP_MEMORY_SCOPE_AGENT);
		__hip_atomic_fetch_add(&p.ctl->stat_help, t_help, __ATOMIC_RELAXED, __HIP_MEMORY_SCOPE_AGENT);
		__hip_atomic_fetch_add(&p.ctl->stat_t_wait, rt_wait, __ATOMIC_RELAXED, __HIP_MEMORY_SCOPE_AGENT);
	}
}
__global__ void __launch_bounds__(64 * SVC_MAX_WAVES) __attribute__((amdgpu_waves_per_eu(4, 4))) k_lsd_service(Geom g, SvcParams p) { svc_kernel_body<false>(g, p); }
__global__ void __launch_bounds__(64 * SVC_MAX_WAVES) __attribute__((amdgpu_waves_per_eu(3, 3))) k_lsd_service_c(Geom g, SvcParams p) { svc_kernel_body<true>(g, p); }
#pragma clang diagnostic pop

__global__ void k_svc_probe(SvcHost *host, unsigned long long expect, unsigned long long desired, uint32_t *ok) {
	unsigned long long *w = (unsigned long long *)&host->pad[0];
	unsigned long long e = expect;
	const bool swapped = __hip_atomic_compare_exchange_strong(w, &e, desired, __ATOMIC_ACQ_REL, __ATOMIC_RELAXED, __HIP_MEMORY_SCOPE_SYSTEM);
	__hip_atomic_store(&host->pad[2], swapped ? 0x600Du : 0xBADu, __ATOMIC_RELEASE, __HIP_MEMORY_SCOPE_SYSTEM);
	*ok = swapped ? 1u : 0u;
}

__global__ void __launch_bounds__(256) k_svc_publish(SvcCtl *ctl, unsigned long long *ring, SvcSlot *slots, uint32_t slot, Buffers b, uint32_t n, uint32_t seq, uint32_t ring_log2) {
	__shared__ uint32_t s_base;
	if (threadIdx.x == 0) {
		SvcSlot *sl = slots + slot;
		sl->b = b;
		__hip_atomic_store(&sl->n, n, __ATOMIC_RELAXED, __HIP_MEMORY_SCOPE_AGENT);
		__hip_atomic_store(&sl->seq, seq, __ATOMIC_RELAXED, __HIP_MEMORY_SCOPE_AGENT);
		__hip_atomic_store(&sl->done, 0u, __ATOMIC_RELAXED, __HIP_MEMORY_SCOPE_AGENT);
		__hip_atomic_store(&sl->t_pub, (unsigned long long)__builtin_amdgcn_s_memrealtime(), __ATOMIC_RELAXED, __HIP_MEMORY_SCOPE_AGENT);
		s_base = __hip_atomic_fetch_add(&ctl->reserve, n, __ATOMIC_RELAXED, __HIP_MEMORY_SCOPE_AGENT);
	}
	__syncthreads();
	const uint32_t base = s_base, mask = (1u << ring_log2) - 1u;
	__builtin_amdgcn_fence(__ATOMIC_RELEASE, "agent");
	for (uint32_t i = threadIdx.x; i < n; i += blockDim.x) {
		const uint32_t t = base + i;
		__hip_atomic_store(ring + (t & mask), ((unsigned long long)((t >> ring_log2) + 1u) << 32) | (slot << 24) | i, __ATOMIC_RELAXED, __HIP_MEMORY_SCOPE_AGENT);
	}
	__builtin_amdgcn_fence(__ATOMIC_RELEASE, "agent");
	__syncthreads();
	if (threadIdx.x == 0) __hip_atomic_fetch_add(&ctl->avail, (int32_t)n, __ATOMIC_RELEASE, __HIP_MEMORY_SCOPE_AGENT);
}
```

Measured before the change: 561,500.

## Compute scale ratios in parallel publish kernel and keep LSD results in LDS

In non-compact service mode, the publish kernel now launches one workgroup per frame and computes scale ratios in parallel before the last-arriving block publishes the batch to the ring. The persistent service wave then no longer scans scales serially. The LSD search keeps its lines, rounds and steps in LDS, and the record tail writes final results directly instead of a global write followed by a re-read. The cost is a wider publish launch and a last-arriver counter. The scale work is removed from the per-frame service critical path.

```diff
diff --git a/squad-mortar-helper_amd/batch.py b/squad-mortar-helper_amd/batch.py
--- a/squad-mortar-helper_amd/batch.py
+++ b/squad-mortar-helper_amd/batch.py
@@ -269,6 +269,7 @@
         d["adaptive"] = bool(int(out[13]) & 2)
         d["settled"] = bool(int(out[13]) & 4) or not d["adaptive"]
         d["mode"] = "frame-granular" if int(out[13]) & 1 else "batch-granular"
+        d["service_kernel"] = "k_lsd_service_c" if int(out[30]) else "k_lsd_service"
         d["measured_frames_per_s"] = {"frame-granular": int(out[14]), "batch-granular": int(out[15])}
         return d
 
diff --git a/squad-mortar-helper_amd/csrc/smh_kernels.h b/squad-mortar-helper_amd/csrc/smh_kernels.h
--- a/squad-mortar-helper_amd/csrc/smh_kernels.h
+++ b/squad-mortar-helper_amd/csrc/smh_kernels.h
@@ -69,6 +69,8 @@
 
 #define SMH_FARM_RING 4u
 #define SMH_REC_ON 0x80000000u
+#define SMH_REC_SCANNED 0x40000000u
+#define SMH_REC_FLAGS (SMH_REC_ON | SMH_REC_SCANNED)
 #define SMH_LSD_LATE_HELP 1u
 struct FarmEntry {
 	unsigned long long post;
@@ -206,7 +208,7 @@
 	uint32_t n;
 	uint32_t seq;
 	uint32_t done;
-	uint32_t pad;
+	uint32_t arrived;
 	unsigned long long t_pub;
 };
 #define SVC_REMOTE_RING 12u
@@ -277,7 +279,7 @@
 uint32_t svc_waves_for(const Geom &g, uint32_t tile_limit, uint32_t *part_words, uint32_t *tile_cap, uint32_t *list_cap, uint32_t *lds_bytes, uint32_t *compact = nullptr);
 uint32_t svc_store_words_for(const Geom &g, uint32_t tile_cap, uint32_t compact);
 hipError_t svc_probe_host_atomics(SvcHost *h, SvcHost *d_h, bool *ok);
-hipError_t launch_svc_publish(SvcCtl *ctl, unsigned long long *ring, SvcSlot *slots, uint32_t slot, const Buffers &b, uint32_t n, uint32_t seq, uint32_t ring_log2, hipStream_t s);
+hipError_t launch_svc_publish(const Geom &g, SvcCtl *ctl, unsigned long long *ring, SvcSlot *slots, uint32_t slot, const Buffers &b, uint32_t n, uint32_t seq, uint32_t ring_log2, hipStream_t s);
 hipError_t launch_lsd_service(const Geom &g, const SvcParams &p, uint32_t workgroups, uint32_t waves, uint32_t lds_bytes, hipStream_t s);
 
 enum : uint32_t { MAP_UI = 1u, MAP_MASK = 2u, MAP_PRIO = 0x100u, MAP_BAND_MAJOR = 0x200u };
diff --git a/squad-mortar-helper_amd/csrc/smh_lsd.hip b/squad-mortar-helper_amd/csrc/smh_lsd.hip
--- a/squad-mortar-helper_amd/csrc/smh_lsd.hip
+++ b/squad-mortar-helper_amd/csrc/smh_lsd.hip
@@ -1302,8 +1302,11 @@
 	return hipSuccess;
 }
 
-hipError_t launch_svc_publish(SvcCtl *ctl, unsigned long long *ring, SvcSlot *slots, uint32_t slot, const Buffers &b, uint32_t n, uint32_t seq, uint32_t ring_log2, hipStream_t s) {
-	hipLaunchKernelGGL(k_svc_publish, dim3(1), dim3(256), 0, s, ctl, ring, slots, slot, b, n, seq, ring_log2);
+hipError_t launch_svc_publish(const Geom &g, SvcCtl *ctl, unsigned long long *ring, SvcSlot *slots, uint32_t slot, const Buffers &b, uint32_t n, uint32_t seq, uint32_t ring_log2, hipStream_t s) {
+	if (!(b.rec_stages & SMH_REC_ON)) return hipErrorInvalidValue;
+	const SvcPublishArgs a{g, ctl, ring, slots, b, slot, n, seq, ring_log2};
+	const bool scan = (b.rec_stages & SMH_REC_SCANNED) != 0u;
+	hipLaunchKernelGGL(k_svc_publish, dim3(scan ? n : 1u), dim3(scan ? 64u * SMHV_MAX_SCALES : 256u), 0, s, a);
 	return hipGetLastError();
 }
 
diff --git a/squad-mortar-helper_amd/csrc/smh_lsd_seq.inc b/squad-mortar-helper_amd/csrc/smh_lsd_seq.inc
--- a/squad-mortar-helper_amd/csrc/smh_lsd_seq.inc
+++ b/squad-mortar-helper_amd/csrc/smh_lsd_seq.inc
@@ -472,7 +472,7 @@
 	}
 }
 
-template <int MODE, bool WAVE = false, bool TEAM = false>
+template <int MODE, bool WAVE = false, bool TEAM = false, bool KEEP = false>
 __device__ void lsd_frame_seq(const Geom &g, const Buffers &b, uint32_t f, float max_gap, const FrameAux &aux, uint32_t *smem, WShared &ws, const uint32_t *cull_tab, const RayDir *dirs,
                               uint32_t win_cap, uint32_t list_cap, const FrameView *tile_view = nullptr) {
 	static_assert(!TEAM || (WAVE && (MODE == LSD_MODE_TILE || MODE == LSD_MODE_TILEC)), "helpers read the owner's tile store in LDS");
@@ -624,11 +624,16 @@
 		while (uniform_u32(W_LD_ACQ(&ws.late)) != 0u) __builtin_amdgcn_s_sleep(2);
 	}
 	smhv_frame_result *res = &b.results[f];
-	if (lane < n_lines) {
-		res->lines[lane].x0 = ws.lines[lane][0]; res->lines[lane].y0 = ws.lines[lane][1];
-		res->lines[lane].x1 = ws.lines[lane][2]; res->lines[lane].y1 = ws.lines[lane][3];
-	}
-	if (lane == 0) { res->n_lines = n_lines; res->rounds = rounds; res->ray_steps = ws.steps; res->status = SMHV_FRAME_OK; }
+	if constexpr (KEEP) {
+		if (lane == 0) ws.rounds = rounds;
+		(void)res;
+	} else {
+		if (lane < n_lines) {
+			res->lines[lane].x0 = ws.lines[lane][0]; res->lines[lane].y0 = ws.lines[lane][1];
+			res->lines[lane].x1 = ws.lines[lane][2]; res->lines[lane].y1 = ws.lines[lane][3];
+		}
+		if (lane == 0) { res->n_lines = n_lines; res->rounds = rounds; res->ray_steps = ws.steps; res->status = SMHV_FRAME_OK; }
+	}
 #ifdef SMH_LSD_WDEBUG
 	if (lane == 0) {
 		for (int k = 0; k < 5; ++k) res->meters[20 + k] = (double)sprof[k];
diff --git a/squad-mortar-helper_amd/csrc/smh_lsd_wave.inc b/squad-mortar-helper_amd/csrc/smh_lsd_wave.inc
--- a/squad-mortar-helper_amd/csrc/smh_lsd_wave.inc
+++ b/squad-mortar-helper_amd/csrc/smh_lsd_wave.inc
@@ -66,13 +66,17 @@
 	uint32_t win_free;
 	uint32_t farm_on, farm_posted, farm_retired, pad0;
 	uint32_t late, want_set, want_tick, pick;
-	unsigned long long t0, late_cycles;
+	unsigned long long t0;
+	union {
+		unsigned long long late_cycles;
+		double rec_mpx;
+	};
 	unsigned long long rem_r, rem_store, rem_ctl;
 	uint32_t rem_after, rem_tickets, rem_owner, rem_cap;
 	uint32_t rem_open, rem_gen, rem_k, rem_nr;
 	unsigned long long rem_done;
 	uint32_t rem_n, rem_last_div;
-	uint32_t rem_flags, rem_pad;
+	uint32_t rem_flags, rec_has_mpx;
 #ifdef SMH_LSD_WDEBUG
 	uint32_t dbg[8];
 	unsigned long long rdbg[10];
diff --git a/squad-mortar-helper_amd/csrc/smh_record.inc b/squad-mortar-helper_amd/csrc/smh_record.inc
--- a/squad-mortar-helper_amd/csrc/smh_record.inc
+++ b/squad-mortar-helper_amd/csrc/smh_record.inc
@@ -4,6 +4,7 @@
 
 namespace smh {
 
+template <uint32_t CHUNKS = 4u>
 __device__ inline bool find_scale_width(const uint8_t *img, size_t pitch, uint32_t w, uint32_t h, uint32_t meters, uint32_t x, uint32_t y, double *ratio,
                                  uint32_t bar[3]) {
 	const uint32_t lane = threadIdx.x & 63u;
@@ -12,16 +13,16 @@
 	const uint32_t max_off = (uint32_t)floor(t + 0.5);
 	const uint32_t y_end = min(h, y + max_off);
 	auto first_tick = [&](uint32_t yy, uint32_t count, auto col) -> uint32_t {
-		for (uint32_t base = 0; base < count; base += 256u) {
-			uint8_t v[4][SMH_MIN_SCALE_VERTICAL_BAR_HEIGHT];
+		for (uint32_t base = 0; base < count; base += 64u * CHUNKS) {
+			uint8_t v[CHUNKS][SMH_MIN_SCALE_VERTICAL_BAR_HEIGHT];
 #pragma unroll
-			for (uint32_t c = 0; c < 4u; ++c) {
+			for (uint32_t c = 0; c < CHUNKS; ++c) {
 				const uint32_t i = base + c * 64u + lane, xx = col(min(i, count - 1u));
 #pragma unroll
 				for (uint32_t k = 0; k < SMH_MIN_SCALE_VERTICAL_BAR_HEIGHT; ++k) v[c][k] = img[(size_t)min(yy + k, h - 1u) * pitch + xx];
 			}
 #pragma unroll
-			for (uint32_t c = 0; c < 4u; ++c) {
+			for (uint32_t c = 0; c < CHUNKS; ++c) {
 				const uint32_t i = base + c * 64u + lane;
 				uint32_t bad = 0;
 #pragma unroll
@@ -56,28 +57,38 @@
 	return false;
 }
 
+__device__ __forceinline__ void rec_st_wt(uint32_t *p, uint32_t v) { __hip_atomic_store(p, v, __ATOMIC_RELAXED, __HIP_MEMORY_SCOPE_AGENT); }
+__device__ __forceinline__ void rec_st_wt(double *p, double v) {
+	__hip_atomic_store((unsigned long long *)p, (unsigned long long)__double_as_longlong(v), __ATOMIC_RELAXED, __HIP_MEMORY_SCOPE_AGENT);
+}
+
+template <bool PUBLISH = false>
 __device__ __forceinline__ void scale_ratio_body(const Geom &g, const Buffers &b, uint32_t f, uint32_t *bars) {
 	const uint32_t wave = threadIdx.x >> 6, lane = threadIdx.x & 63u, nwaves = blockDim.x >> 6;
 	__shared__ double s_ratio[SMHV_MAX_SCALES];
 	__shared__ uint32_t s_ok[SMHV_MAX_SCALES];
 	smhv_frame_result *res = &b.results[f];
 	const bool open = b.aux[f].open != 0;
-	const smhv_anchors an = b.anchors[f];
+	const smhv_anchors *ap = b.anchors + f;
+	smhv_anchors an;
+	if constexpr (PUBLISH) { an.n = ap->n; an.scales_start_y = ap->scales_start_y; } else an = *ap;
 	const uint32_t n = open ? min(an.n, (uint32_t)SMHV_MAX_SCALES) : 0u;
 	const bool valid = an.scales_start_y <= g.qh;
 	for (uint32_t k = wave; k < SMHV_MAX_SCALES; k += nwaves) {
 		double r = 0.0;
 		uint32_t bar[3] = {0, 0, 0};
 		bool ok = false;
+		const uint32_t *sc = PUBLISH ? ap->scales[k] : an.scales[k];
 		if (k < n && valid) {
 			const uint8_t *img = b.scales + (size_t)f * g.ocr_stride + g.q_xoff;
-			ok = find_scale_width(img, g.ocr_pitch, g.qw, g.qh, an.scales[k][0], an.scales[k][1], an.scales[k][2], &r, bar);
+			ok = find_scale_width<PUBLISH ? 1u : 4u>(img, g.ocr_pitch, g.qw, g.qh, sc[0], sc[1], sc[2], &r, bar);
 		}
 		if (lane == 0) {
 			s_ratio[k] = r; s_ok[k] = ok ? 1u : 0u;
 			if (bars) {
 				uint32_t *o = bars + ((size_t)f * SMHV_MAX_SCALES + k) * 4;
-				o[0] = bar[0]; o[1] = bar[1]; o[2] = bar[2]; o[3] = ok ? 1u : 0u;
+				if constexpr (PUBLISH) { rec_st_wt(o, bar[0]); rec_st_wt(o + 1, bar[1]); rec_st_wt(o + 2, bar[2]); rec_st_wt(o + 3, ok ? 1u : 0u); }
+				else { o[0] = bar[0]; o[1] = bar[1]; o[2] = bar[2]; o[3] = ok ? 1u : 0u; }
 			}
 		}
 	}
@@ -86,25 +97,24 @@
 		double sum = 0.0; uint32_t k = 0;
 		for (uint32_t i = 0; i < SMHV_MAX_SCALES; ++i)
 			if (s_ok[i]) { sum = k ? sum + s_ratio[i] : s_ratio[i]; ++k; }
-		res->has_mpx = k ? 1u : 0u;
-		res->mpx = k == 0 ? 0.0 : (k == 1 ? sum : sum / (double)k);
+		const double mpx = k == 0 ? 0.0 : (k == 1 ? sum : sum / (double)k);
+		if constexpr (PUBLISH) { rec_st_wt(&res->has_mpx, k ? 1u : 0u); rec_st_wt(&res->mpx, mpx); }
+		else { res->has_mpx = k ? 1u : 0u; res->mpx = mpx; }
 	}
 }
 
-__device__ __forceinline__ void finalize_body(const Geom &g, const Buffers &b, uint32_t f, uint32_t stages, uint32_t l) {
+template <bool OWN_SEARCH, typename LineAt>
+__device__ __forceinline__ void finalize_write(const Buffers &b, uint32_t f, uint32_t stages, uint32_t l, const FrameAux &aux, uint32_t n, bool has_mpx, double mpx, LineAt line_at,
+                                               uint32_t rounds, unsigned long long ray_steps) {
 	smhv_frame_result *res = &b.results[f];
-	const FrameAux aux = b.aux[f];
 	const bool open = aux.open != 0;
 	const bool markers = (stages & SMHV_STAGE_MARKERS) != 0;
-	const uint32_t n = (open && markers) ? res->n_lines : 0u;
-	const bool has_mpx = open && (stages & SMHV_STAGE_SCALES) && res->has_mpx;
-	const double mpx = has_mpx ? res->mpx : 0.0;
 	if (l < SMHV_MAX_LINES) {
 		double len = 0.0, met = 0.0;
 		float ang = 0.0f;
 		smhv_line ln = {0.0f, 0.0f, 0.0f, 0.0f};
 		if (l < n) {
-			ln = res->lines[l];
+			ln = line_at(l);
 			const double ax = (double)ln.x0 - (double)ln.x1, ay = (double)ln.y0 - (double)ln.y1;
 			len = sqrt(ax * ax + ay * ay);
 			met = has_mpx ? len * mpx : 0.0;
@@ -130,10 +140,24 @@
 		res->mpx = mpx; res->has_mpx = has_mpx ? 1u : 0u;
 		res->n_mask_px = (open && markers) ? aux.n_mask_px : 0u;
 		res->red_pixels = aux.red;
-		if (!(open && markers)) { res->rounds = 0; res->ray_steps = 0; }
+		if constexpr (OWN_SEARCH) {
+			res->rounds = (open && markers) ? rounds : 0u; res->ray_steps = (open && markers) ? ray_steps : 0ull;
+			res->status = SMHV_FRAME_OK;
+		} else if (!(open && markers)) { res->rounds = 0; res->ray_steps = 0; }
 		if (!(stages & SMHV_STAGE_MINIMAP)) { res->has_minimap = 0; res->minimap[0] = 0; res->minimap[1] = 0; res->minimap[2] = 0; res->minimap[3] = 0; }
-		if (!(open && markers)) res->status = SMHV_FRAME_OK;
+		if constexpr (!OWN_SEARCH) if (!(open && markers)) res->status = SMHV_FRAME_OK;
 	}
+}
+
+__device__ __forceinline__ void finalize_body(const Geom &g, const Buffers &b, uint32_t f, uint32_t stages, uint32_t l) {
+	smhv_frame_result *res = &b.results[f];
+	const FrameAux aux = b.aux[f];
+	const bool open = aux.open != 0;
+	const bool markers = (stages & SMHV_STAGE_MARKERS) != 0;
+	const uint32_t n = (open && markers) ? res->n_lines : 0u;
+	const bool has_mpx = open && (stages & SMHV_STAGE_SCALES) && res->has_mpx;
+	const double mpx = has_mpx ? res->mpx : 0.0;
+	finalize_write<false>(b, f, stages, l, aux, n, has_mpx, mpx, [&](uint32_t i) { return res->lines[i]; }, 0u, 0ull);
 }
 
 __device__ __forceinline__ void finalize_body(const Geom &g, const Buffers &b, uint32_t f, uint32_t stages) { finalize_body(g, b, f, stages, threadIdx.x); }
@@ -148,7 +172,7 @@
 __device__ __attribute__((noinline)) void frame_record_tail(const Geom *gp, const Buffers *bp, uint32_t f) {
 	const Geom &g = *gp;
 	const Buffers &b = *bp;
-	const uint32_t stages = b.rec_stages & ~SMH_REC_ON;
+	const uint32_t stages = b.rec_stages & ~SMH_REC_FLAGS;
 	if (stages & SMHV_STAGE_SCALES) {
 		scale_ratio_body(g, b, f, b.rec_bars);
 		__syncthreads();
@@ -159,43 +183,5 @@
 	}
 }
 
-__device__ __attribute__((noinline)) void frame_record_tail_wave(const Geom *gp, const Buffers *bp, uint32_t f) {
-	const Geom &g = *gp;
-	const Buffers &b = *bp;
-	const uint32_t stages = b.rec_stages & ~SMH_REC_ON;
-	const uint32_t lane = threadIdx.x & 63u;
-	smhv_frame_result *res = &b.results[f];
-	if (stages & SMHV_STAGE_SCALES) {
-		const bool open = b.aux[f].open != 0;
-		const smhv_anchors an = b.anchors[f];
-		const uint32_t n = open ? min(an.n, (uint32_t)SMHV_MAX_SCALES) : 0u;
-		const bool valid = an.scales_start_y <= g.qh;
-		double sum = 0.0;
-		uint32_t cnt = 0;
-		for (uint32_t k = 0; k < SMHV_MAX_SCALES; ++k) {
-			double r = 0.0;
-			uint32_t bar[3] = {0, 0, 0};
-			bool ok = false;
-			if (k < n && valid) {
-				const uint8_t *img = b.scales + (size_t)f * g.ocr_stride + g.q_xoff;
-				ok = find_scale_width(img, g.ocr_pitch, g.qw, g.qh, an.scales[k][0], an.scales[k][1], an.scales[k][2], &r, bar);
-			}
-			if (lane == 0 && b.rec_bars) {
-				uint32_t *o = b.rec_bars + ((size_t)f * SMHV_MAX_SCALES + k) * 4;
-				o[0] = bar[0]; o[1] = bar[1]; o[2] = bar[2]; o[3] = ok ? 1u : 0u;
-			}
-			if (ok) { sum = cnt ? sum + r : r; ++cnt; }
-		}
-		if (lane == 0) {
-			res->has_mpx = cnt ? 1u : 0u;
-			res->mpx = cnt == 0 ? 0.0 : (cnt == 1 ? sum : sum / (double)cnt);
-		}
-	}
-	__builtin_amdgcn_fence(__ATOMIC_RELEASE, "workgroup");
-	__builtin_amdgcn_wave_barrier();
-	__builtin_amdgcn_fence(__ATOMIC_ACQUIRE, "workgroup");
-	finalize_body(g, b, f, stages, lane);
-	if (stages & SMHV_STAGE_FIRING) firing_after_finalize(bp, f, lane);
-}
 
 }
diff --git a/squad-mortar-helper_amd/csrc/smh_runtime.cpp b/squad-mortar-helper_amd/csrc/smh_runtime.cpp
--- a/squad-mortar-helper_amd/csrc/smh_runtime.cpp
+++ b/squad-mortar-helper_amd/csrc/smh_runtime.cpp
@@ -775,7 +775,8 @@
 }
 
 struct SvcPublish { SvcCtl *ctl; unsigned long long *ring; SvcSlot *slots; uint32_t slot, seq, ring_log2; const uint32_t *cull_tab; bool have_cull; hipStream_t s_pro; hipEvent_t ev_pro;
-                    bool *published; };
+                    bool *published;
+                    bool scan; };
 static int batch_run_impl(smhv_batch *b, const void *d_frames, uint32_t n, uint32_t stages, int grayscale, uint32_t max_gap,
                           const smhv_anchors *anchors, hipStream_t s, hipStream_t sl, const SvcPublish *svc = nullptr) {
 	if (!b || !d_frames || n == 0 || n > b->max_frames) return fail(SMHV_E_INVALID, "bad arguments (n=%u, capacity %u)", n, b ? b->max_frames : 0);
@@ -857,10 +858,10 @@
 	if (svc) {
 		if (stages & SMHV_STAGE_MINIMAP) HIPCHK(launch_find_minimap(g, bf, n, s));
 		if (stages & SMHV_STAGE_HEIGHTMAP_OVERLAY) HIPCHK(launch_hm_overlay(g, orun, n, s));
-		bf.rec_stages = SMH_REC_ON | (scales ? stages : (stages & ~SMHV_STAGE_SCALES));
+		bf.rec_stages = SMH_REC_ON | (scales ? (stages | (svc->scan ? SMH_REC_SCANNED : 0u)) : (stages & ~SMHV_STAGE_SCALES));
 		bf.rec_bars = b->d_bars;
 		STAGE_BEGIN(3, s);
-		HIPCHK(launch_svc_publish(svc->ctl, svc->ring, svc->slots, svc->slot, bf, n, svc->seq, svc->ring_log2, s));
+		HIPCHK(launch_svc_publish(g, svc->ctl, svc->ring, svc->slots, svc->slot, bf, n, svc->seq, svc->ring_log2, s));
 		if (svc->published) *svc->published = true;
 		STAGE_END(3, s);
 		STAGE_BEGIN(4, s);
@@ -1395,7 +1396,7 @@
 	uint32_t seq = ++p->seq_counter;
 	if (seq == 0u) seq = ++p->seq_counter;
 	bool published = false;
-	SvcPublish pub{p->d_svc_ctl, p->d_svc_ring, p->d_svc_slots, slot, seq, p->svc_ring_log2, probe.cull_tab, true, p->s_pro, p->ev_pro[slot], &published};
+	SvcPublish pub{p->d_svc_ctl, p->d_svc_ring, p->d_svc_slots, slot, seq, p->svc_ring_log2, probe.cull_tab, true, p->s_pro, p->ev_pro[slot], &published, !p->svc_compact};
 	__atomic_fetch_add(&p->h_svc->state, 1ull << 32, __ATOMIC_ACQ_REL);
 	rc = batch_run_impl(b, d_frames, n, stages, grayscale, max_gap, anchors, st, st, &pub);
 	if (rc && !published) {
@@ -1593,6 +1594,7 @@
 	out[16] = c.stat_requests; out[17] = c.stat_attached; out[18] = c.stat_remote; out[19] = (uint64_t)(int64_t)c.help_avail;
 	out[20] = c.stat_t_wait; out[21] = c.stat_t_sub; out[22] = c.stat_t_last;
 	out[23] = c.stat_h_polls; out[24] = c.stat_h_empty; out[25] = c.stat_h_lost; out[26] = c.stat_h_idle_exit; out[27] = c.stat_h_closed_exit; out[28] = c.stat_h_cycles; out[29] = c.stat_h_cast_cycles;
+	out[30] = p->svc_compact;
 	out[13] = (p->adaptive ? 2u : 0u) | (p->mode_frame ? 1u : 0u) | (p->mc.phase == 4u ? 4u : 0u); out[14] = (uint64_t)p->mc.rate[1]; out[15] = (uint64_t)p->mc.rate[0];
 	return SMHV_OK;
 }
diff --git a/squad-mortar-helper_amd/csrc/smh_service.inc b/squad-mortar-helper_amd/csrc/smh_service.inc
--- a/squad-mortar-helper_amd/csrc/smh_service.inc
+++ b/squad-mortar-helper_amd/csrc/smh_service.inc
@@ -22,6 +22,52 @@
 __device__ __forceinline__ uint32_t *lds_ptr(uint32_t byte_off) { return (uint32_t *)(LdsWord *)(uintptr_t)uniform_u32(byte_off); }
 __device__ __forceinline__ uint32_t lds_off(const void *p) { return (uint32_t)(uintptr_t)(const LdsByte *)p; }
 
+__device__ __attribute__((noinline)) void frame_record_tail_wave(const Geom *gp, const Buffers *bp, uint32_t f, uint32_t ws_off, uint32_t aux_open, uint32_t aux_n_mask_px, uint32_t aux_red) {
+	const Geom &g = *gp;
+	const Buffers &b = *bp;
+	const uint32_t stages = b.rec_stages & ~SMH_REC_FLAGS;
+	const uint32_t lane = threadIdx.x & 63u;
+	const WShared &ws = *(const WShared *)lds_ptr(ws_off);
+	FrameAux aux{};
+	aux.open = aux_open; aux.n_mask_px = aux_n_mask_px; aux.red = aux_red;
+	const bool open = aux_open != 0;
+	uint32_t rec_has = 0;
+	double rec_mpx = 0.0;
+	if (stages & SMHV_STAGE_SCALES) {
+		if (b.rec_stages & SMH_REC_SCANNED) { rec_has = ws.rec_has_mpx; rec_mpx = ws.rec_mpx; }
+		else {
+			const smhv_anchors an = b.anchors[f];
+			const uint32_t n = open ? min(an.n, (uint32_t)SMHV_MAX_SCALES) : 0u;
+			const bool valid = an.scales_start_y <= g.qh;
+			double sum = 0.0;
+			uint32_t cnt = 0;
+			for (uint32_t k = 0; k < SMHV_MAX_SCALES; ++k) {
+				double r = 0.0;
+				uint32_t bar[3] = {0, 0, 0};
+				bool ok = false;
+				if (k < n && valid) {
+					const uint8_t *img = b.scales + (size_t)f * g.ocr_stride + g.q_xoff;
+					ok = find_scale_width(img, g.ocr_pitch, g.qw, g.qh, an.scales[k][0], an.scales[k][1], an.scales[k][2], &r, bar);
+				}
+				if (lane == 0 && b.rec_bars) {
+					uint32_t *o = b.rec_bars + ((size_t)f * SMHV_MAX_SCALES + k) * 4;
+					o[0] = bar[0]; o[1] = bar[1]; o[2] = bar[2]; o[3] = ok ? 1u : 0u;
+				}
+				if (ok) { sum = cnt ? sum + r : r; ++cnt; }
+			}
+			rec_has = cnt ? 1u : 0u;
+			rec_mpx = cnt == 0 ? 0.0 : (cnt == 1 ? sum : sum / (double)cnt);
+		}
+	}
+	const bool markers = (stages & SMHV_STAGE_MARKERS) != 0;
+	const uint32_t n = (open && markers) ? ws.n_lines : 0u;
+	const bool has_mpx = open && (stages & SMHV_STAGE_SCALES) && rec_has;
+	const double mpx = has_mpx ? rec_mpx : 0.0;
+	finalize_write<true>(b, f, stages, lane, aux, n, has_mpx, mpx, [&](uint32_t i) { return smhv_line{ws.lines[i][0], ws.lines[i][1], ws.lines[i][2], ws.lines[i][3]}; },
+	                     ws.rounds, ws.steps);
+	if (stages & SMHV_STAGE_FIRING) firing_after_finalize(bp, f, lane);
+}
+
 template <bool COMPACT>
 __device__ __attribute__((noinline)) void svc_frame_global(const void *kargs, uint32_t slot, uint32_t f, uint32_t part_off, uint32_t cull_off, uint32_t dirs_off) {
 	SvcKernelArgsPtr ka = svc_args(kargs);
@@ -30,7 +76,7 @@
 	const Geom g = ka->g;
 	const Buffers b = ((SvcSlotPtr)(ka->p.slots + slot))->b;
 	const FrameAux aux = b.aux[f];
-	lsd_frame_seq<LSD_MODE_GLOBAL, true>(g, b, f, ka->p.max_gap, aux, part + SVC_WS_WORDS, *(WShared *)part, lds_ptr(cull_off), (const RayDir *)lds_ptr(dirs_off), 0u, ka->p.list_cap);
+	lsd_frame_seq<LSD_MODE_GLOBAL, true, false, true>(g, b, f, ka->p.max_gap, aux, part + SVC_WS_WORDS, *(WShared *)part, lds_ptr(cull_off), (const RayDir *)lds_ptr(dirs_off), 0u, ka->p.list_cap);
 }
 
 template <bool COMPACT>
@@ -43,8 +89,10 @@
 	const FrameAux aux = b.aux[f];
 	WShared &ws = *(WShared *)part;
 	uint32_t *smem = part + SVC_WS_WORDS;
+	if ((b.rec_stages & SMH_REC_SCANNED) && (threadIdx.x & 63u) == 0) { ws.rec_has_mpx = b.results[f].has_mpx; ws.rec_mpx = b.results[f].mpx; }
 	if (!aux.open || aux.n_mask_px == 0) {
-		if ((threadIdx.x & 63u) == 0) { b.results[f].n_lines = 0; b.results[f].rounds = 0; b.results[f].ray_steps = 0; b.results[f].status = SMHV_FRAME_OK; }
+		if ((threadIdx.x & 63u) == 0) { ws.n_lines = 0u; ws.rounds = 0u; ws.steps = 0ull; }
+		wave_lds_sync();
 	} else {
 		const uint32_t tile_cap = ka->p.tile_cap;
 		if ((threadIdx.x & 63u) == 0) {
@@ -64,12 +112,12 @@
 			fits = rc == 2u ? frame_setup_tile<true>(g, b, f, aux, smem, tile_cap, &ws.ntiles, v) : rc == 0u;
 		}
 		if (fits) {
-			if constexpr (COMPACT) lsd_frame_seq<LSD_MODE_TILEC, true, true>(g, b, f, ka->p.max_gap, aux, smem, ws, lds_ptr(cull_off), (const RayDir *)lds_ptr(dirs_off), tilec_mask_words(g.rw, g.rh, tile_cap), ka->p.list_cap, &v);
-			else lsd_frame_seq<LSD_MODE_TILE, true, true>(g, b, f, ka->p.max_gap, aux, smem, ws, lds_ptr(cull_off), (const RayDir *)lds_ptr(dirs_off), tile_mask_words(g.rw, g.rh, tile_cap), ka->p.list_cap, &v);
+			if constexpr (COMPACT) lsd_frame_seq<LSD_MODE_TILEC, true, true, true>(g, b, f, ka->p.max_gap, aux, smem, ws, lds_ptr(cull_off), (const RayDir *)lds_ptr(dirs_off), tilec_mask_words(g.rw, g.rh, tile_cap), ka->p.list_cap, &v);
+			else lsd_frame_seq<LSD_MODE_TILE, true, true, true>(g, b, f, ka->p.max_gap, aux, smem, ws, lds_ptr(cull_off), (const RayDir *)lds_ptr(dirs_off), tile_mask_words(g.rw, g.rh, tile_cap), ka->p.list_cap, &v);
 		} else svc_frame_global<COMPACT>(kargs, slot, f, part_off, cull_off, dirs_off);
 	}
 	const unsigned long long t_search_end = __builtin_amdgcn_s_memtime();
-	if (b.rec_stages & SMH_REC_ON) frame_record_tail_wave(&((const SvcKernelArgs *)kargs)->g, &((const SvcSlot *)(ka->p.slots + slot))->b, f);
+	frame_record_tail_wave(&((const SvcKernelArgs *)kargs)->g, &((const SvcSlot *)(ka->p.slots + slot))->b, f, part_off, aux.open, aux.n_mask_px, aux.red);
 	return t_search_end;
 }
 
@@ -418,13 +466,35 @@
 	*ok = swapped ? 1u : 0u;
 }
 
-__global__ void __launch_bounds__(256) k_svc_publish(SvcCtl *ctl, unsigned long long *ring, SvcSlot *slots, uint32_t slot, Buffers b, uint32_t n, uint32_t seq, uint32_t ring_log2) {
+struct SvcPublishArgs { Geom g; SvcCtl *ctl; unsigned long long *ring; SvcSlot *slots; Buffers b; uint32_t slot, n, seq, ring_log2; };
+__global__ void __launch_bounds__(256) k_svc_publish(SvcPublishArgs) {
+#ifdef __HIP_DEVICE_COMPILE__
+	const SvcPublishArgs &a = *(const SvcPublishArgs *)(const __attribute__((address_space(4))) SvcPublishArgs *)__builtin_amdgcn_kernarg_segment_ptr();
+#else
+	const SvcPublishArgs a{};
+#endif
+	SvcCtl *ctl = a.ctl;
+	unsigned long long *ring = a.ring;
+	SvcSlot *sl = a.slots + a.slot;
+	const uint32_t slot = a.slot, n = a.n, ring_log2 = a.ring_log2;
 	__shared__ uint32_t s_base;
+	if (a.b.rec_stages & SMH_REC_SCANNED) {
+		__shared__ uint32_t s_last;
+		scale_ratio_body<true>(a.g, a.b, blockIdx.x, a.b.rec_bars);
+		asm volatile("s_waitcnt vmcnt(0)" ::: "memory");
+		__syncthreads();
+		if (threadIdx.x == 0) {
+			const uint32_t last = __hip_atomic_fetch_add(&sl->arrived, 1u, __ATOMIC_RELAXED, __HIP_MEMORY_SCOPE_AGENT) + 1u == gridDim.x ? 1u : 0u;
+			if (last) __hip_atomic_store(&sl->arrived, 0u, __ATOMIC_RELAXED, __HIP_MEMORY_SCOPE_AGENT);
+			s_last = last;
+		}
+		__syncthreads();
+		if (!s_last) return;
+	}
 	if (threadIdx.x == 0) {
-		SvcSlot *sl = slots + slot;
-		sl->b = b;
+		sl->b = a.b;
 		__hip_atomic_store(&sl->n, n, __ATOMIC_RELAXED, __HIP_MEMORY_SCOPE_AGENT);
-		__hip_atomic_store(&sl->seq, seq, __ATOMIC_RELAXED, __HIP_MEMORY_SCOPE_AGENT);
+		__hip_atomic_store(&sl->seq, a.seq, __ATOMIC_RELAXED, __HIP_MEMORY_SCOPE_AGENT);
 		__hip_atomic_store(&sl->done, 0u, __ATOMIC_RELAXED, __HIP_MEMORY_SCOPE_AGENT);
 		__hip_atomic_store(&sl->t_pub, (unsigned long long)__builtin_amdgcn_s_memrealtime(), __ATOMIC_RELAXED, __HIP_MEMORY_SCOPE_AGENT);
 		s_base = __hip_atomic_fetch_add(&ctl->reserve, n, __ATOMIC_RELAXED, __HIP_MEMORY_SCOPE_AGENT);
```

Measured after the change: 568,600, median of 6. 1.01x the previous value.
